# andreaskoepf/faster-rcnn.torch

Hardware: AMD Instinct MI355X
Metric: images/sec (vgg_small 800x450 fwd+bwd) (higher is better)
Workload: dtype f32 (conv / Linear(13824,1024) operands as 2 x fp16 split planes: 22 significand bits, 3 MFMA partial products; fp32 accumulate)

## Files before the change

faster-rcnn.torch_amd/_lib.py:

```python
import ctypes as C
import os

_HERE = os.path.dirname(os.path.abspath(__file__))
SO_PATH = os.environ.get("FRCNN_LIB_PATH") or os.path.join(_HERE, "libfrcnn_hip.so")

KC_NAMES = ["conv_igemm_k3", "conv_igemm_other", "conv_wgrad_k3", "conv_wgrad_other", "gemm", "elemwise",
            "roi", "rpn", "nms", "optim", "image", "conv_x3", "conv_wgradx", "topk"]


class FrcnnError(RuntimeError):
    pass


class ModelDesc(C.Structure):
    _fields_ = [
        ("nblocks", C.c_int),
        ("filters", C.c_int * 8), ("ksize", C.c_int * 8), ("pad", C.c_int * 8), ("conv_steps", C.c_int * 8),
        ("dropout", C.c_float * 8),
        ("nheads", C.c_int),
        ("head_k", C.c_int * 8), ("head_n", C.c_int * 8), ("head_input", C.c_int * 8),
        ("ncls", C.c_int),
        ("cls_n", C.c_int * 8), ("cls_bn", C.c_int * 8),
        ("cls_dropout", C.c_float * 8),
        ("class_count", C.c_int),
        ("kh", C.c_int), ("kw", C.c_int),
    ]


vp = C.c_void_p
_SIGS = {
    "frcnn_version": ([], C.c_int),
    "frcnn_set_option": ([C.c_char_p, C.c_int], C.c_int),
    "frcnn_get_option": ([C.c_char_p, C.POINTER(C.c_int)], C.c_int),
    "frcnn_last_error": ([], C.c_char_p),
    "frcnn_device_count": ([C.POINTER(C.c_int)], C.c_int),
    "frcnn_set_device": ([C.c_int], C.c_int),
    "frcnn_device_name": ([C.c_char_p, C.c_int], C.c_int),
    "frcnn_malloc": ([C.POINTER(vp), C.c_size_t], C.c_int),
    "frcnn_free": ([vp], C.c_int),
    "frcnn_host_alloc": ([C.POINTER(vp), C.c_size_t], C.c_int),
    "frcnn_host_free": ([vp], C.c_int),
    "frcnn_memcpy_h2d": ([vp, vp, C.c_size_t, vp], C.c_int),
    "frcnn_memcpy_d2h": ([vp, vp, C.c_size_t, vp], C.c_int),
    "frcnn_memcpy_d2d": ([vp, vp, C.c_size_t, vp], C.c_int),
    "frcnn_stream_sync": ([vp], C.c_int),
    "frcnn_zero": ([vp, C.c_size_t, vp], C.c_int),
    "frcnn_scale": ([vp, C.c_longlong, C.c_float, vp], C.c_int),
    "frcnn_add": ([vp, vp, C.c_longlong, vp], C.c_int),
    "frcnn_prof_enable": ([C.c_int], C.c_int),
    "frcnn_prof_collect": ([vp, vp, vp, vp], C.c_int),
    "frcnn_nms_workspace_bytes": ([C.c_int], C.c_size_t),
    "frcnn_nms_device": ([vp, C.c_int, C.c_int, C.c_float, C.c_int, C.c_int, vp, vp, vp, C.c_size_t, vp], C.c_int),
    "frcnn_nms_device_classes": ([vp, C.c_int, C.c_int, C.c_float, C.c_int, C.c_int, vp, vp, vp, vp, C.c_size_t, vp], C.c_int),
    "frcnn_nms_device_n": ([vp, C.c_int, vp, C.c_int, C.c_float, C.c_int, C.c_int, vp, vp, vp, vp, C.c_size_t, vp], C.c_int),
    "frcnn_nms_batch_workspace_bytes": ([C.c_int, C.c_int], C.c_size_t),
    "frcnn_nms_device_batch": ([vp, C.c_int, C.c_longlong, C.c_int, vp, C.c_int, C.c_float, C.c_int, C.c_int, vp, vp, vp, vp, C.c_size_t,
                               vp], C.c_int),
    "frcnn_topk_select_workspace_bytes": ([C.c_int, C.c_int], C.c_size_t),
    "frcnn_topk_select": ([vp, C.c_int, C.c_longlong, C.c_int, vp, C.c_int, vp, C.c_longlong, vp, vp, C.c_size_t, vp], C.c_int),
    "frcnn_rpn_gather_rows": ([vp, vp, vp, vp, C.c_int, C.c_longlong, C.c_int, vp, C.c_longlong, vp, C.c_int, vp, vp, vp, vp, vp, vp,
                              C.c_longlong, vp], C.c_int),
    "frcnn_detect_gather_batch": ([vp, vp, C.c_int, C.c_int, vp, vp, vp, vp, vp, C.c_longlong, vp, vp, vp, vp, vp], C.c_int),
    "frcnn_roi_windows": ([vp, vp, C.c_int, vp, C.c_int, C.c_int, C.c_int, vp, vp], C.c_int),
    "frcnn_detect_post": ([vp, vp, vp, vp, vp, C.c_int, C.c_int, C.c_double, vp, vp, vp, vp, vp, vp], C.c_int),
    "frcnn_detect_gather": ([vp, vp, C.c_int, vp, vp, vp, vp, vp, vp, vp, vp, vp, vp], C.c_int),
    "frcnn_nms_host": ([vp, C.c_int, C.c_int, C.c_float, C.c_int, C.c_int, vp, vp], C.c_int),
    "frcnn_conv2d_forward": ([vp, C.c_int, C.c_int, C.c_int, vp, vp, vp, vp, C.c_int, C.c_int, C.c_int, vp, vp], C.c_int),
    "frcnn_conv2d_backward_input": ([vp, C.c_int, C.c_int, C.c_int, vp, C.c_int, C.c_int, C.c_int, vp, C.c_int, vp], C.c_int),
    "frcnn_conv2d_backward_weight": ([vp, C.c_int, C.c_int, C.c_int, vp, vp, vp, C.c_int, C.c_int, C.c_int, vp, vp, vp], C.c_int),
    "frcnn_maxpool_act_forward": ([vp, C.c_int, C.c_int, C.c_int, vp, vp, vp, vp, vp], C.c_int),
    "frcnn_maxpool_act_backward": ([vp, vp, vp, C.c_int, C.c_int, C.c_int, vp, vp, vp, vp, vp, vp], C.c_int),
    "frcnn_act_forward": ([vp, C.c_int, C.c_longlong, vp, vp, vp, vp], C.c_int),
    "frcnn_act_backward": ([vp, vp, C.c_int, C.c_longlong, vp, vp, vp, vp, vp, vp], C.c_int),
    "frcnn_roi_pool_forward": ([vp, C.c_int, C.c_int, C.c_int, vp, C.c_int, C.c_int, C.c_int, vp, vp, vp], C.c_int),
    "frcnn_roi_pool_backward": ([vp, C.c_int, C.c_int, C.c_int, vp, vp, C.c_int, C.c_int, C.c_int, vp], C.c_int),
    "frcnn_roi_align_forward": ([vp, C.c_int, C.c_int, C.c_int, vp, vp, C.c_int, C.c_double, C.c_double, C.c_int, C.c_int, C.c_int, vp,
                                 vp], C.c_int),
    "frcnn_roi_align_backward": ([vp, C.c_int, C.c_int, C.c_int, vp, vp, vp, C.c_int, C.c_double, C.c_double, C.c_int, C.c_int, C.c_int,
                                  vp], C.c_int),
    "frcnn_rpn_scan_workspace_bytes": ([vp, vp], C.c_size_t),
    "frcnn_rpn_scan": ([vp, vp, vp, vp, vp, C.c_double, C.c_double, C.c_double, C.c_int, vp, vp, vp, vp, vp, vp, C.c_size_t, vp], C.c_int),
    "frcnn_rpn_scan_batch_workspace_bytes": ([vp, vp, C.c_int], C.c_size_t),
    "frcnn_rpn_scan_batch": ([vp, vp, vp, C.c_int, C.c_longlong, vp, vp, C.c_double, C.c_double, C.c_double, C.c_int, vp, vp, vp, vp, vp,
                             vp, C.c_size_t, vp], C.c_int),
    "frcnn_rpn_loss": ([vp, vp, vp, vp, vp, vp, vp, vp, C.c_int, C.c_int, C.c_int, vp, vp, vp, vp], C.c_int),
    "frcnn_loss_accumulate": ([vp, C.c_int, vp, vp], C.c_int),
    "frcnn_linear_forward": ([vp, C.c_int, C.c_int, vp, vp, C.c_int, vp, vp], C.c_int),
    "frcnn_linear_backward": ([vp, vp, C.c_int, C.c_int, vp, C.c_int, vp, vp, vp, vp], C.c_int),
    "frcnn_rmsprop": ([vp, vp, vp, C.c_longlong, C.c_float, C.c_float, C.c_float, vp], C.c_int),
    "frcnn_scale_rmsprop": ([vp, vp, C.c_float, vp, C.c_longlong, C.c_float, C.c_float, C.c_float, vp], C.c_int),
    "frcnn_scale_rmsprop_dev": ([vp, vp, vp, vp, C.c_longlong, C.c_float, C.c_float, C.c_float, vp], C.c_int),
    "frcnn_scale_rmsprop_slice": ([vp, vp, C.c_float, vp, C.c_longlong, C.c_longlong, C.c_float, C.c_float, C.c_float, vp], C.c_int),
    "frcnn_sgd": ([vp, vp, vp, C.c_longlong, C.c_float, vp, C.c_float, C.c_float, C.c_float, C.c_float, C.c_int, C.c_int, vp], C.c_int),
    "frcnn_sgd_slice": ([vp, vp, vp, C.c_longlong, C.c_longlong, C.c_float, C.c_float, C.c_float, C.c_float, C.c_float, C.c_int, C.c_int,
                         vp], C.c_int),
    "frcnn_nag": ([vp, vp, vp, C.c_longlong, C.c_float, vp, C.c_float, C.c_float, C.c_float, C.c_int, vp], C.c_int),
    "frcnn_nag_slice": ([vp, vp, vp, C.c_longlong, C.c_longlong, C.c_float, C.c_float, C.c_float, C.c_float, C.c_int, vp], C.c_int),
    "frcnn_scale_rmsprop_slice_dev": ([vp, vp, vp, vp, C.c_longlong, C.c_longlong, C.c_float, C.c_float, C.c_float, vp], C.c_int),
    "frcnn_sgd_slice_dev": ([vp, vp, vp, C.c_longlong, C.c_longlong, vp, C.c_float, C.c_float, C.c_float, C.c_float, C.c_int, C.c_int,
                            vp], C.c_int),
    "frcnn_nag_slice_dev": ([vp, vp, vp, C.c_longlong, C.c_longlong, vp, C.c_float, C.c_float, C.c_float, C.c_int, vp], C.c_int),
    "frcnn_grad_clip_workspace_bytes": ([C.c_longlong], C.c_size_t),
    "frcnn_grad_clip": ([vp, C.c_longlong, vp, C.c_int, C.c_double, vp, C.c_double, vp, vp, C.c_size_t, vp], C.c_int),
    "frcnn_nag_lookahead": ([vp, vp, C.c_longlong, C.c_float, vp], C.c_int),
    "frcnn_nag_lookahead_slice": ([vp, vp, C.c_longlong, C.c_longlong, C.c_float, vp], C.c_int),
    "frcnn_model_update_stream": ([vp, C.POINTER(vp)], C.c_int),
    "frcnn_model_update_fork": ([vp, vp], C.c_int),
    "frcnn_model_update_join": ([vp, vp], C.c_int),
    "frcnn_pnet_wait_backward_begun": ([vp, vp], C.c_int),
    "frcnn_pnet_wait_heads_done": ([vp, vp], C.c_int),
    "frcnn_pnet_wait_block_done": ([vp, C.c_int, vp], C.c_int),
    "frcnn_pnet_refresh_packs": ([vp, vp, C.c_int, vp], C.c_int),
    "frcnn_pnet_invalidate_packs": ([vp], C.c_int),
    "frcnn_model_create": ([C.POINTER(ModelDesc), C.POINTER(vp)], C.c_int),
    "frcnn_model_destroy": ([vp], C.c_int),
    "frcnn_model_param_count": ([vp, C.POINTER(C.c_longlong), C.POINTER(C.c_longlong)], C.c_int),
    "frcnn_model_param_table": ([vp, vp, C.c_int, C.POINTER(C.c_int)], C.c_int),
    "frcnn_model_localizer_layers": ([vp, C.c_int, vp, C.c_int, C.POINTER(C.c_int)], C.c_int),
    "frcnn_model_set_trainable": ([vp, C.c_int, C.c_int, C.c_int], C.c_int),
    "frcnn_model_get_trainable": ([vp, C.POINTER(C.c_int), C.POINTER(C.c_int), C.POINTER(C.c_int)], C.c_int),
    "frcnn_model_debug_buffer": ([vp, C.c_int, C.c_int, C.POINTER(vp), C.POINTER(C.c_longlong)], C.c_int),
    "frcnn_pnet_forward": ([vp, vp, vp, C.c_int, C.c_int, C.c_int, vp, C.c_ulonglong, vp], C.c_int),
    "frcnn_pnet_forward_async_heads": ([vp, vp, vp, C.c_int, C.c_int, vp, C.c_ulonglong, vp], C.c_int),
    "frcnn_pnet_output": ([vp, C.c_int, C.POINTER(vp), C.POINTER(C.c_int), C.POINTER(C.c_int), C.POINTER(C.c_int)], C.c_int),
    "frcnn_pnet_delta": ([vp, C.c_int, C.POINTER(vp)], C.c_int),
    "frcnn_pnet_set_sparse_deltas": ([vp, C.c_int, vp, C.c_int], C.c_int),
    "frcnn_pnet_zero_deltas": ([vp, vp], C.c_int),
    "frcnn_pnet_backward_heads_begin": ([vp, vp, vp, vp], C.c_int),
    "frcnn_pnet_anchor_loss_begin": ([vp, vp, vp, vp, vp, vp, vp, C.c_int, C.c_int, C.c_int, vp, vp, vp, vp, vp], C.c_int),
    "frcnn_pnet_anchor_loss_wait": ([vp, vp], C.c_int),
    "frcnn_pnet_backward_heads_join": ([vp, vp, C.POINTER(C.c_int)], C.c_int),
    "frcnn_pnet_backward": ([vp, vp, vp, vp], C.c_int),
    "frcnn_pnet_wait_block_gradients": ([vp, C.c_int, vp], C.c_int),
    "frcnn_cnet_forward": ([vp, vp, vp, C.c_int, C.c_int, vp, C.c_ulonglong, vp, vp, vp, vp], C.c_int),
    "frcnn_cnet_backward": ([vp, vp, vp, vp, vp, vp, vp], C.c_int),
    "frcnn_cnet_backward_join": ([vp, vp], C.c_int),
    "frcnn_cnet_losses": ([vp, vp, vp, vp, C.c_int, C.c_int, C.c_int, vp, vp, vp, vp], C.c_int),
    "frcnn_cnet_decode": ([vp, C.c_int, C.c_int, vp, vp, vp], C.c_int),
    "frcnn_anchors_create": ([vp, vp, vp, vp, C.c_int, C.c_int, C.POINTER(vp)], C.c_int),
    "frcnn_anchors_destroy": ([vp], C.c_int),
    "frcnn_anchors_assemble": ([vp, vp, C.c_int, C.c_double, C.c_double, C.c_double, C.c_double, C.c_int, C.c_int, C.c_int, vp,
                               C.POINTER(C.c_int), vp, vp, C.c_int, C.POINTER(C.c_int), C.POINTER(C.c_int)], C.c_int),
    "frcnn_comm_get_unique_id": ([vp], C.c_int),
    "frcnn_comm_exchange_id_file": ([C.c_char_p, C.c_int, vp, C.c_int], C.c_int),
    "frcnn_comm_init_rank": ([C.POINTER(vp), C.c_int, C.c_int, vp], C.c_int),
    "frcnn_comm_init_rank_timeout": ([C.POINTER(vp), C.c_int, C.c_int, vp, C.c_int], C.c_int),
    "frcnn_comm_init_rank_file": ([C.POINTER(vp), C.c_int, C.c_int, C.c_char_p, C.c_int], C.c_int),
    "frcnn_comm_destroy": ([vp], C.c_int),
    "frcnn_comm_info": ([vp, C.POINTER(C.c_int), C.POINTER(C.c_int)], C.c_int),
    "frcnn_comm_query": ([vp, C.POINTER(C.c_int), C.POINTER(C.c_int), C.POINTER(C.c_int)], C.c_int),
    "frcnn_allreduce_f32": ([vp, vp, C.c_longlong, vp], C.c_int),
    "frcnn_allreduce_f64": ([vp, vp, C.c_longlong, vp], C.c_int),
    "frcnn_broadcast_f32": ([vp, vp, C.c_longlong, C.c_int, vp], C.c_int),
    "frcnn_image_rgb2yuv": ([vp, vp, C.c_int, C.c_int, vp], C.c_int),
    "frcnn_image_rgb2hsv": ([vp, vp, C.c_int, C.c_int, vp], C.c_int),
    "frcnn_image_rgb2lab": ([vp, vp, C.c_int, C.c_int, vp], C.c_int),
    "frcnn_image_scale": ([vp, C.c_int, C.c_int, C.c_int, vp, C.c_int, C.c_int, vp, C.c_int, vp], C.c_int),
    "frcnn_image_scale_u8": ([vp, C.c_int, C.c_int, vp, C.c_int, C.c_int, vp, C.c_int, vp], C.c_int),
    "frcnn_image_crop_flip": ([vp, C.c_int, C.c_int, C.c_int, C.c_int, C.c_int, C.c_int, C.c_int, C.c_int, C.c_int, vp, vp], C.c_int),
    "frcnn_image_normalize_workspace_bytes": ([C.c_int], C.c_size_t),
    "frcnn_image_normalize": ([vp, C.c_int, C.c_int, C.c_int, C.c_int, C.c_int, vp, C.c_size_t, vp], C.c_int),
    "frcnn_image_contrastive_norm": ([vp, C.c_int, C.c_int, vp, C.c_int, C.c_float, vp, vp, vp], C.c_int),
}

_lib = None


def exported_symbols():
    return sorted(_SIGS.keys())


def load():
    global _lib
    if _lib is not None:
        return _lib
    if not os.path.exists(SO_PATH):
        raise FrcnnError(
            "libfrcnn_hip.so not found at %s -- build it with `python -c 'import __graft_entry__ as g; g.build()'` "
            "(there is no CPU fallback for the product path)" % SO_PATH)
    try:
        import torch
    except ImportError:
        pass
    L = C.CDLL(SO_PATH)
    for name, (args, res) in _SIGS.items():
        fn = getattr(L, name)
        fn.argtypes = args
        fn.restype = res
    _lib = L
    return L


def check(rc):
    if rc != 0:
        raise FrcnnError("libfrcnn_hip: %s (code %d)" % (load().frcnn_last_error().decode("utf-8", "replace"), rc))


def call(name, *args):
    check(getattr(load(), name)(*args))
```

faster-rcnn.torch_amd/csrc/amax.h:

```cpp
#pragma once
#include <hip/hip_runtime.h>

#include "kernels.h"

namespace frcnn {

__device__ __forceinline__ void amax_store_block(float m, float* rec) {
  __shared__ float amax_part[16];
#pragma unroll
  for (int o = 32; o > 0; o >>= 1) m = fmaxf(m, __shfl_xor(m, o));
  if ((threadIdx.x & 63) == 0) amax_part[threadIdx.x >> 6] = m;
  __syncthreads();
  if (threadIdx.x == 0) {
    const int nw = (blockDim.x + 63) >> 6;
    for (int i = 1; i < nw; ++i) m = fmaxf(m, amax_part[i]);
    rec[1 + blockIdx.x] = m;
    if (blockIdx.x == 0) rec[0] = __builtin_bit_cast(float, (int)gridDim.x);
  }
}

__device__ __forceinline__ float amax_load_block(const float* __restrict__ rec) {
  __shared__ float amax_all[16];
  const int n = __builtin_bit_cast(int, rec[0]);
  float m = 0.f;
  for (int i = threadIdx.x; i < n; i += blockDim.x) m = fmaxf(m, rec[1 + i]);
#pragma unroll
  for (int o = 32; o > 0; o >>= 1) m = fmaxf(m, __shfl_xor(m, o));
  if ((threadIdx.x & 63) == 0) amax_all[threadIdx.x >> 6] = m;
  __syncthreads();
  const int nw = (blockDim.x + 63) >> 6;
  m = amax_all[0];
  for (int i = 1; i < nw; ++i) m = fmaxf(m, amax_all[i]);
  __syncthreads();
  return m;
}

}
```

faster-rcnn.torch_amd/csrc/cnet.hip:

```cpp
#include "kernels.h"

namespace frcnn {

#define BN_EPS 1e-5
#define BN_MOM 0.1

#define BN_CB 16
#define BN_RG 64
template <int CB = BN_CB, int RG = BN_RG>
__device__ __forceinline__ double bn_reduce(double v, double* sh, int tx, int ty) {
  sh[ty * CB + tx] = v;
  __syncthreads();
  for (int stride = RG / 2; stride > 0; stride >>= 1) {
    if (ty < stride) sh[ty * CB + tx] += sh[(ty + stride) * CB + tx];
    __syncthreads();
  }
  const double s = sh[tx];
  __syncthreads();
  return s;
}
template <int NV>
__device__ __forceinline__ void fb_reduce(double (&v)[NV], double* sh, int tx, int ty) {
  const int tid = ty * 4 + tx, lane = tid & 63, wave = tid >> 6;
#pragma unroll
  for (int k = 0; k < NV; ++k) {
#pragma unroll
    for (int o = 4; o < 64; o <<= 1) v[k] += __shfl_xor(v[k], o, 64);
    if (lane < 4) sh[(k * 16 + wave) * 4 + lane] = v[k];
  }
  __syncthreads();
#pragma unroll
  for (int k = 0; k < NV; ++k) {
    double t = 0.0;
#pragma unroll
    for (int w = 0; w < 16; ++w) t += sh[(k * 16 + w) * 4 + tx];
    v[k] = t;
  }
  __syncthreads();
}
#define FB_CB 4
#define FB_RG 256
#define FB_KEEP 4

__global__ __launch_bounds__(1024) void bn_forward_kernel(const float* __restrict__ x, int R, int n,
                                                          const float* __restrict__ gamma, const float* __restrict__ beta,
                                                          float* running, int training, float* __restrict__ xhat,
                                                          float* __restrict__ invstd, float* __restrict__ y) {
  __shared__ double sh[BN_RG * BN_CB];
  const int tx = threadIdx.x, ty = threadIdx.y;
  const int j = blockIdx.x * BN_CB + tx;
  const bool ok = j < n;
  double mean, var;
  if (training) {
    double s = 0.0;
    if (ok) for (int r = ty; r < R; r += BN_RG) s += x[(size_t)r * n + j];
    mean = bn_reduce(s, sh, tx, ty) / R;
    double q = 0.0;
    if (ok) for (int r = ty; r < R; r += BN_RG) { double d = x[(size_t)r * n + j] - mean; q += d * d; }
    var = bn_reduce(q, sh, tx, ty);
    const double unb = R > 1 ? var / (R - 1) : var / R;
    var /= R;
    if (running && ok && ty == 0) {
      running[j] = (float)((1.0 - BN_MOM) * running[j] + BN_MOM * mean);
      running[n + j] = (float)((1.0 - BN_MOM) * running[n + j] + BN_MOM * unb);
    }
  } else {
    mean = ok ? running[j] : 0.0;
    var = ok ? running[n + j] : 1.0;
  }
  if (!ok) return;
  const double is = 1.0 / sqrt(var + BN_EPS);
  if (ty == 0) invstd[j] = (float)is;
  const double g = gamma[j], b = beta[j];
  for (int r = ty; r < R; r += BN_RG) {
    const double xh = (x[(size_t)r * n + j] - mean) * is;
    xhat[(size_t)r * n + j] = (float)xh;
    y[(size_t)r * n + j] = (float)(xh * g + b);
  }
}
int bn_forward(const float* x, int R, int n, const float* gamma, const float* beta, float* running,
               int training, float* xhat, float* invstd, float* y, hipStream_t s) {
  FR_CHECK(training || running, "bn_forward: evaluate mode needs running statistics");
  FR_LAUNCH(KC_ELEMWISE, 0, (double)R * n * 16.0, s, bn_forward_kernel, dim3(cdiv(n, BN_CB)), dim3(BN_CB, BN_RG), 0, x, R, n,
            gamma, beta, running, training, xhat, invstd, y);
  FR_LAUNCH_CHECK();
  return FRCNN_OK;
}

__global__ __launch_bounds__(1024) void bn_backward_kernel(const float* __restrict__ gy, const float* __restrict__ xhat,
                                                           const float* __restrict__ invstd, const float* __restrict__ gamma,
                                                           int R, int n, int training, float* __restrict__ gx, float* ggamma,
                                                           float* gbeta) {
  __shared__ double sh[BN_RG * BN_CB];
  const int tx = threadIdx.x, ty = threadIdx.y;
  const int j = blockIdx.x * BN_CB + tx;
  const bool ok = j < n;
  double sg = 0.0, sgx = 0.0;
  if (ok)
    for (int r = ty; r < R; r += BN_RG) {
      const double g = gy[(size_t)r * n + j];
      sg += g;
      sgx += g * xhat[(size_t)r * n + j];
    }
  sg = bn_reduce(sg, sh, tx, ty);
  sgx = bn_reduce(sgx, sh, tx, ty);
  if (!ok) return;
  if (ty == 0) {
    ggamma[j] = (float)((double)ggamma[j] + sgx);
    gbeta[j] = (float)((double)gbeta[j] + sg);
  }
  const double is = invstd[j], gm = gamma[j];
  for (int r = ty; r < R; r += BN_RG) {
    const double g = gy[(size_t)r * n + j];
    const double xh = xhat[(size_t)r * n + j];
    const double v = training ? (g - sg / R - xh * sgx / R) * gm * is : g * gm * is;
    gx[(size_t)r * n + j] = (float)v;
  }
}
int bn_backward(const float* gy, const float* xhat, const float* invstd, const float* gamma, int R,
                int n, int training, float* gx, float* ggamma, float* gbeta, hipStream_t s) {
  FR_LAUNCH(KC_ELEMWISE, 0, (double)R * n * 16.0, s, bn_backward_kernel, dim3(cdiv(n, BN_CB)), dim3(BN_CB, BN_RG), 0, gy,
            xhat, invstd, gamma, R, n, training, gx, ggamma, gbeta);
  FR_LAUNCH_CHECK();
  return FRCNN_OK;
}

__device__ __forceinline__ float fold_value(const float* __restrict__ x, const GemmFold& src, size_t total, size_t idx, int j) {
  if (src.nSplit == 0) return x[idx];
  float v = src.bias ? src.bias[j] : 0.f;
  for (int sI = 0; sI < src.nSplit; ++sI) v += src.slab[(size_t)sI * total + idx];
  return v;
}

template <bool GEN>
__global__ __launch_bounds__(1024) void cnet_act_forward_kernel(const float* __restrict__ x, GemmFold src, int R, int n,
                                                                const float* __restrict__ gamma, const float* __restrict__ beta,
                                                                float* running, int training, float* __restrict__ lin,
                                                                float* __restrict__ xhat, float* __restrict__ invstd,
                                                                float* __restrict__ pre, const float* slope, float* __restrict__ mask,
                                                                float inv_keep, float p, unsigned long long seed,
                                                                float* __restrict__ post) {
  __shared__ double sh[FB_RG * FB_CB];
  const int tx = threadIdx.x, ty = threadIdx.y;
  const int j = blockIdx.x * FB_CB + tx;
  const bool ok = j < n;
  const size_t total = (size_t)R * n;
  const bool bn = gamma != nullptr;
  const float* v = src.nSplit ? lin : x;
  const bool keep = R <= FB_RG * FB_KEEP;
  float xv[FB_KEEP];
  double s0 = 0.0;
  if (ok) {
#pragma unroll
    for (int i = 0; i < FB_KEEP; ++i) {
      const int r = ty + i * FB_RG;
      xv[i] = 0.f;
      if (keep && r < R) {
        const size_t idx = (size_t)r * n + j;
        xv[i] = fold_value(x, src, total, idx, j);
        if (src.nSplit) lin[idx] = xv[i];
        s0 += xv[i];
      }
    }
    if (!keep && (src.nSplit || (bn && training)))
      for (int r = ty; r < R; r += FB_RG) {
        const size_t idx = (size_t)r * n + j;
        const float t = fold_value(x, src, total, idx, j);
        if (src.nSplit) lin[idx] = t;
        s0 += t;
      }
  }
  double mean = 0.0, is = 1.0, g = 1.0, b = 0.0;
  if (bn) {
    double var;
    if (training) {
      { double t[1] = {s0}; fb_reduce(t, sh, tx, ty); mean = t[0] / R; }
      double q = 0.0;
      if (ok && keep) {
#pragma unroll
        for (int i = 0; i < FB_KEEP; ++i)
          if (ty + i * FB_RG < R) { double d = xv[i] - mean; q += d * d; }
      } else if (ok) {
        for (int r = ty; r < R; r += FB_RG) { double d = v[(size_t)r * n + j] - mean; q += d * d; }
      }
      { double t[1] = {q}; fb_reduce(t, sh, tx, ty); var = t[0]; }
      const double unb = R > 1 ? var / (R - 1) : var / R;
      var /= R;
      if (running && ok && ty == 0) {
        running[j] = (float)((1.0 - BN_MOM) * running[j] + BN_MOM * mean);
        running[n + j] = (float)((1.0 - BN_MOM) * running[n + j] + BN_MOM * unb);
      }
    } else {
      mean = ok ? running[j] : 0.0;
      var = ok ? running[n + j] : 1.0;
    }
    if (!ok) return;
    is = 1.0 / sqrt(var + BN_EPS);
    if (ty == 0) invstd[j] = (float)is;
    g = gamma[j]; b = beta[j];
  }
  if (!ok) return;
  const float a = *slope;
  auto emit = [&](size_t idx, float y) {
    if (bn) {
      const double xh = ((double)y - mean) * is;
      xhat[idx] = (float)xh;
      y = (float)(xh * g + b);
      pre[idx] = y;
    }
    y = y > 0.f ? y : a * y;
    if (GEN) {
      const float mk = frcnn_keep_mask(seed, (unsigned long long)idx, p);
      mask[idx] = mk;
      y = y * (mk * inv_keep);
    } else if (mask) {
      y = y * (mask[idx] * inv_keep);
    }
    post[idx] = y;
  };
  if (keep) {
#pragma unroll
    for (int i = 0; i < FB_KEEP; ++i)
      if (ty + i * FB_RG < R) emit((size_t)(ty + i * FB_RG) * n + j, xv[i]);
  } else {
    for (int r = ty; r < R; r += FB_RG) emit((size_t)r * n + j, v[(size_t)r * n + j]);
  }
}
template <bool GEN>
__global__ void cnet_act_forward_flat_kernel(const float* __restrict__ x, GemmFold src, long total, int n, float* __restrict__ lin,
                                             const float* slope, float* __restrict__ mask, float inv_keep, float p,
                                             unsigned long long seed, float* __restrict__ post) {
  const float a = *slope;
  for (long i = (long)blockIdx.x * blockDim.x + threadIdx.x; i < total; i += (long)gridDim.x * blockDim.x) {
    float y = fold_value(x, src, (size_t)total, (size_t)i, (int)(i % n));
    if (src.nSplit) lin[i] = y;
    y = y > 0.f ? y : a * y;
    if (GEN) {
      const float mk = frcnn_keep_mask(seed, (unsigned long long)i, p);
      mask[i] = mk;
      y = y * (mk * inv_keep);
    } else if (mask) {
      y = y * (mask[i] * inv_keep);
    }
    post[i] = y;
  }
}
int cnet_act_forward(const float* x, GemmFold src, int R, int n, const float* gamma, const float* beta, float* running,
                     int training, float* lin, float* xhat, float* invstd, float* pre, const float* slope, float* mask, bool gen,
                     float inv_keep, float p, unsigned long long seed, float* post, hipStream_t s) {
  FR_CHECK(!gamma || training || running, "cnet_act_forward: evaluate mode needs running statistics");
  if (!gamma) {
    const long total = (long)R * n;
    const int grid = (int)std::min<long>(std::max<long>(1, cdivl(total, 256)), 2048);
    if (gen)
      FR_LAUNCH(KC_ELEMWISE, 0, total * 16.0, s, cnet_act_forward_flat_kernel<true>, dim3(grid), dim3(256), 0, x, src, total, n, lin, slope,
                mask, inv_keep, p, seed, post);
    else
      FR_LAUNCH(KC_ELEMWISE, 0, total * 16.0, s, cnet_act_forward_flat_kernel<false>, dim3(grid), dim3(256), 0, x, src, total, n, lin, slope,
                mask, inv_keep, p, seed, post);
    FR_LAUNCH_CHECK();
    return FRCNN_OK;
  }
  if (gen)
    FR_LAUNCH(KC_ELEMWISE, 0, (double)R * n * 20.0, s, cnet_act_forward_kernel<true>, dim3(cdiv(n, FB_CB)), dim3(FB_CB, FB_RG), 0, x,
              src, R, n, gamma, beta, running, training, lin, xhat, invstd, pre, slope, mask, inv_keep, p, seed, post);
  else
    FR_LAUNCH(KC_ELEMWISE, 0, (double)R * n * 20.0, s, cnet_act_forward_kernel<false>, dim3(cdiv(n, FB_CB)), dim3(FB_CB, FB_RG), 0, x,
              src, R, n, gamma, beta, running, training, lin, xhat, invstd, pre, slope, mask, inv_keep, p, seed, post);
  FR_LAUNCH_CHECK();
  return FRCNN_OK;
}

__global__ __launch_bounds__(1024) void cnet_act_bn_backward_kernel(const float* __restrict__ gy, GemmFold src,
                                                                    const float* __restrict__ pre, const float* __restrict__ xhat,
                                                                    const float* __restrict__ invstd, const float* __restrict__ gamma,
                                                                    const float* slope, const float* __restrict__ mask, float inv_keep,
                                                                    int R, int n, int training, float* __restrict__ gx, float* ggamma,
                                                                    float* gbeta, float* gslope, float* part) {
  __shared__ double sh[FB_RG * FB_CB];
  __shared__ float shs[16];
  const int tx = threadIdx.x, ty = threadIdx.y;
  const int j = blockIdx.x * FB_CB + tx;
  const bool ok = j < n;
  const size_t total = (size_t)R * n;
  const float a = *slope;
  double sg = 0.0, sgx = 0.0;
  float sa = 0.f;
  const bool keep = R <= FB_RG * FB_KEEP;
  float tv[FB_KEEP], xh[FB_KEEP];
  auto first = [&](size_t idx, float& t, float& xhv) {
    float g = fold_value(gy, src, total, idx, j);
    if (mask) g = g * (mask[idx] * inv_keep);
    const float xv = pre[idx];
    t = g;
    if (!(xv > 0.f)) { t = a * g; sa += xv * g; }
    xhv = xhat[idx];
    sg += t;
    sgx += (double)t * xhv;
  };
  if (ok && keep) {
#pragma unroll
    for (int i = 0; i < FB_KEEP; ++i) {
      tv[i] = 0.f; xh[i] = 0.f;
      if (ty + i * FB_RG < R) first((size_t)(ty + i * FB_RG) * n + j, tv[i], xh[i]);
    }
  } else if (ok) {
    for (int r = ty; r < R; r += FB_RG) {
      const size_t idx = (size_t)r * n + j;
      float t, xhv;
      first(idx, t, xhv);
      gx[idx] = t;
    }
  }
  { double t[2] = {sg, sgx}; fb_reduce(t, sh, tx, ty); sg = t[0]; sgx = t[1]; }
  {
    const int tid = ty * FB_CB + tx;
#pragma unroll
    for (int o = 32; o > 0; o >>= 1) sa += __shfl_down(sa, o, 64);
    if ((tid & 63) == 0) shs[tid >> 6] = sa;
    __syncthreads();
    if (tid == 0) {
      float t = 0.f;
      for (int i = 0; i < 16; ++i) t += shs[i];
      if (part) part[blockIdx.x] = t; else unsafeAtomicAdd(gslope, t);
    }
  }
  if (!ok) return;
  if (ty == 0) {
    ggamma[j] = (float)((double)ggamma[j] + sgx);
    gbeta[j] = (float)((double)gbeta[j] + sg);
  }
  const double is = invstd[j], gm = gamma[j];
  auto second = [&](size_t idx, double g, double xhv) {
    const double v = training ? (g - sg / R - xhv * sgx / R) * gm * is : g * gm * is;
    gx[idx] = (float)v;
  };
  if (keep) {
#pragma unroll
    for (int i = 0; i < FB_KEEP; ++i)
      if (ty + i * FB_RG < R) second((size_t)(ty + i * FB_RG) * n + j, tv[i], xh[i]);
  } else {
    for (int r = ty; r < R; r += FB_RG) {
      const size_t idx = (size_t)r * n + j;
      second(idx, gx[idx], xhat[idx]);
    }
  }
}
__global__ void slope_fold_kernel(const float* __restrict__ part, int n, float* gslope);
int cnet_act_bn_backward(const float* gy, GemmFold src, const float* pre, const float* xhat, const float* invstd,
                         const float* gamma, const float* slope, const float* mask, float inv_keep, int R, int n, int training,
                         float* gx, float* ggamma, float* gbeta, float* gslope, hipStream_t s) {
  const int grid = cdiv(n, FB_CB);
  float* part = nullptr;
  if (deterministic()) FR_TRY(det_workspace(s, (size_t)grid, &part));
  FR_LAUNCH(KC_ELEMWISE, 0, (double)R * n * 28.0, s, cnet_act_bn_backward_kernel, dim3(grid), dim3(FB_CB, FB_RG), 0, gy, src, pre, xhat,
            invstd, gamma, slope, mask, inv_keep, R, n, training, gx, ggamma, gbeta, gslope, part);
  if (part) FR_LAUNCH(KC_ELEMWISE, 0, grid * 4.0, s, slope_fold_kernel, dim3(1), dim3(1), 0, (const float*)part, grid, gslope);
  FR_LAUNCH_CHECK();
  return FRCNN_OK;
}

template <bool GEN>
__global__ void prelu_dropout_forward_kernel(const float* __restrict__ x, long n, const float* slope,
                                             float* __restrict__ mask, float inv_keep, float p,
                                             unsigned long long seed, float* __restrict__ y) {
  const float a = *slope;
  for (long i = (long)blockIdx.x * blockDim.x + threadIdx.x; i < n; i += (long)gridDim.x * blockDim.x) {
    float v = x[i];
    v = v > 0.f ? v : a * v;
    if (GEN) {
      const float mk = frcnn_keep_mask(seed, (unsigned long long)i, p);
      mask[i] = mk;
      v = v * (mk * inv_keep);
    } else if (mask) {
      v = v * (mask[i] * inv_keep);
    }
    y[i] = v;
  }
}
int prelu_dropout_forward(const float* x, long n, const float* slope, const float* mask, float inv_keep,
                          float* y, hipStream_t s) {
  int grid = (int)std::min<long>(std::max<long>(1, cdivl(n, 256)), 1024);
  FR_LAUNCH(KC_ELEMWISE, 0, n * 12.0, s, prelu_dropout_forward_kernel<false>, dim3(grid), dim3(256), 0, x, n, slope,
            const_cast<float*>(mask), inv_keep, 0.f, 0ull, y);
  FR_LAUNCH_CHECK();
  return FRCNN_OK;
}
int prelu_dropout_forward_gen(const float* x, long n, const float* slope, float* mask_out, float p,
                              unsigned long long seed, float* y, hipStream_t s) {
  int grid = (int)std::min<long>(std::max<long>(1, cdivl(n, 256)), 1024);
  FR_LAUNCH(KC_ELEMWISE, 0, n * 12.0, s, prelu_dropout_forward_kernel<true>, dim3(grid), dim3(256), 0, x, n, slope,
            mask_out, 1.0f / (1.0f - p), p, seed, y);
  FR_LAUNCH_CHECK();
  return FRCNN_OK;
}

__global__ void prelu_dropout_backward_kernel(const float* __restrict__ gy, const float* __restrict__ x, long n,
                                              const float* slope, const float* __restrict__ mask,
                                              float inv_keep, float* __restrict__ gx, float* gslope, float* part) {
  __shared__ float sh[4];
  const float a = *slope;
  float sa = 0.f;
  for (long i = (long)blockIdx.x * blockDim.x + threadIdx.x; i < n; i += (long)gridDim.x * blockDim.x) {
    float g = gy[i];
    if (mask) g = g * (mask[i] * inv_keep);
    const float xv = x[i];
    float r = g;
    if (!(xv > 0.f)) { r = a * g; sa += xv * g; }
    gx[i] = r;
  }
#pragma unroll
  for (int o = 32; o > 0; o >>= 1) sa += __shfl_down(sa, o, 64);
  if ((threadIdx.x & 63) == 0) sh[threadIdx.x >> 6] = sa;
  __syncthreads();
  if (threadIdx.x == 0) {
    const float t = sh[0] + sh[1] + sh[2] + sh[3];
    if (part) part[blockIdx.x] = t;
    else unsafeAtomicAdd(gslope, t);
  }
}
__global__ void slope_fold_kernel(const float* __restrict__ part, int n, float* gslope) {
  float v = 0.f;
  for (int i = 0; i < n; ++i) v += part[i];
  *gslope += v;
}
int prelu_dropout_backward(const float* gy, const float* x, long n, const float* slope,
                           const float* mask, float inv_keep, float* gx, float* gslope, hipStream_t s) {
  int grid = (int)std::min<long>(std::max<long>(1, cdivl(n, 256)), 256);
  float* part = nullptr;
  if (deterministic()) FR_TRY(det_workspace(s, (size_t)grid, &part));
  FR_LAUNCH(KC_ELEMWISE, 0, n * 16.0, s, prelu_dropout_backward_kernel, dim3(grid), dim3(256), 0, gy, x, n,
            slope, mask, inv_keep, gx, gslope, part);
  if (part) FR_LAUNCH(KC_ELEMWISE, 0, grid * 4.0, s, slope_fold_kernel, dim3(1), dim3(1), 0, (const float*)part, grid, gslope);
  FR_LAUNCH_CHECK();
  return FRCNN_OK;
}

__device__ __forceinline__ double wave_sum_f64(double v) {
#pragma unroll
  for (int o = 32; o > 0; o >>= 1) v += __shfl_xor(v, o, 64);
  return v;
}
__device__ __forceinline__ double wave_max_f64(double v) {
#pragma unroll
  for (int o = 32; o > 0; o >>= 1) { const double w = __shfl_xor(v, o, 64); v = w > v ? w : v; }
  return v;
}
__global__ void log_softmax_rows_fold_kernel(float* __restrict__ x, GemmFold src, int R, int n, float* __restrict__ y,
                                             float* __restrict__ y2) {
  const int r = blockIdx.x * (blockDim.x >> 6) + (threadIdx.x >> 6), lane = threadIdx.x & 63;
  if (r >= R) return;
  float* xr = x + (size_t)r * n;
  const size_t total = (size_t)R * n;
  if (src.nSplit)
    for (int i = lane; i < n; i += 64) xr[i] = fold_value(x, src, total, (size_t)r * n + i, i);
  double m = -1.0e300;
  for (int i = lane; i < n; i += 64) m = xr[i] > m ? (double)xr[i] : m;
  m = wave_max_f64(m);
  double s = 0.0;
  for (int i = lane; i < n; i += 64) s += exp((double)xr[i] - m);
  s = wave_sum_f64(s);
  const double lse = m + log(s);
  for (int i = lane; i < n; i += 64) {
    const float v = (float)((double)xr[i] - lse);
    y[(size_t)r * n + i] = v;
    if (y2) y2[(size_t)r * n + i] = v;
  }
}
int log_softmax_rows_fold(const float* x, GemmFold src, int R, int n, float* y, float* y2, hipStream_t s) {
  if (R <= 0) return FRCNN_OK;
  FR_LAUNCH(KC_ELEMWISE, 0, (double)R * n * 8.0, s, log_softmax_rows_fold_kernel, dim3(cdiv(R, 4)), dim3(256), 0, const_cast<float*>(x),
            src, R, n, y, y2);
  FR_LAUNCH_CHECK();
  return FRCNN_OK;
}

__global__ void log_softmax_rows_kernel(const float* __restrict__ x, int R, int n, float* __restrict__ y) {
  const int r = blockIdx.x * (blockDim.x >> 6) + (threadIdx.x >> 6), lane = threadIdx.x & 63;
  if (r >= R) return;
  const float* xr = x + (size_t)r * n;
  double m = -1.0e300;
  for (int i = lane; i < n; i += 64) m = xr[i] > m ? (double)xr[i] : m;
  m = wave_max_f64(m);
  double s = 0.0;
  for (int i = lane; i < n; i += 64) s += exp((double)xr[i] - m);
  s = wave_sum_f64(s);
  const double lse = m + log(s);
  for (int i = lane; i < n; i += 64) y[(size_t)r * n + i] = (float)((double)xr[i] - lse);
}
int log_softmax_rows(const float* x, int R, int n, float* y, hipStream_t s) {
  if (R <= 0) return FRCNN_OK;
  FR_LAUNCH(KC_ELEMWISE, 0, (double)R * n * 8.0, s, log_softmax_rows_kernel, dim3(cdiv(R, 4)), dim3(256), 0, x, R,
            n, y);
  FR_LAUNCH_CHECK();
  return FRCNN_OK;
}

#define HEADS_PITCH 33
__global__ __launch_bounds__(256) void cnet_heads_forward_kernel(const float* __restrict__ x, int R, int nf, const float* __restrict__ Wb,
                                                                 const float* __restrict__ bb, const float* __restrict__ Wc,
                                                                 const float* __restrict__ bc, int nc, float* __restrict__ bbox_out,
                                                                 float* __restrict__ logits, float* __restrict__ lsm,
                                                                 float* __restrict__ cls_out) {
  extern __shared__ float wt[];
  float* xs = wt + (size_t)nf * HEADS_PITCH + (threadIdx.x >> 6) * nf;
  const int no = 4 + nc;
  for (int k = threadIdx.x; k < nf; k += 256) {
    float* d = wt + k * HEADS_PITCH;
#pragma unroll
    for (int n = 0; n < 4; ++n) d[n] = Wb[(size_t)n * nf + k];
#pragma unroll 8
// ... 208 lines not shown
```

faster-rcnn.torch_amd/csrc/kernels.h:

```cpp
#pragma once
#include <algorithm>

#include "common.h"

namespace frcnn {

int conv_cc(int k);
int conv_mpad(int M);
size_t conv_pack_floats(int Kchan, int M, int k);
int conv_pack_weights(const float* w, int O, int C, int k, float* wf, float* wd, hipStream_t s);
struct PackJob { long w_off; long total; float* dst; int O, C, k, mode, Mpad, blk_begin, nblk; };
PackJob conv_pack_job(long w_off, int O, int C, int k, int mode, float* dst);
int conv_pack_assign_blocks(PackJob* jobs, int njobs, int total_blocks);
int conv_pack_weights_multi(const float* weights, const PackJob* jobs_dev, int njobs, int grid, hipStream_t s);

enum { OUT_STORE = 0, OUT_ADD = 1 };
struct IgemmPool { float* out; unsigned char* idx; const float* slope; const float* scale; float* amax = nullptr; };
int conv_igemm(const float* in, int Cin, int H, int W, const float* in_slope, const float* in_scale,
               const float* wp, const float* bias, int M, int k, int pad, float* out, int out_mode,
               double algo_flops, hipStream_t s, int ws_slot = 0,
               const IgemmPool* pool = nullptr, bool* pool_fused = nullptr);

void set_split_bf16(int on);
int get_split_bf16();
bool conv_x3_eligible(int Cin, int M, int k);
size_t conv_x3_pack_bytes(int Kchan, int M, int k);
struct PackXJob {
  long w_off; long total; void* dst; const float* amax; float* amax_w; int O, C, k, mode, bm, blk_begin, nblk;
  const int* oidx = nullptr; const int* cidx = nullptr; int Cs = 0; long bias_off = 0; float* bias_dst = nullptr;
};
PackXJob conv_x3_pack_job(long w_off, int O, int C, int k, int mode, void* dst, int Ho, int Wo);
int conv_x3_pack_assign_blocks(PackXJob* jobs, int njobs);
int conv_x3_pack_multi(const float* weights, const PackXJob* jobs_dev, int njobs, int grid, hipStream_t s);
int conv_x3_pack(const float* w, int O, int C, int k, int mode, void* dst, hipStream_t s, int Ho, int Wo,
                 const float* amax_rec_w = nullptr, float* amax_w = nullptr);
#define AMAX_REC 16400
#define AMAX_MAX_BLOCKS 16384
int tensor_absmax(const float* x, long n, float* rec, hipStream_t s);
struct AmaxJob { long off; long n; float* out; int blk_begin; };
int tensor_absmax_assign_blocks(AmaxJob* jobs, int njobs);
long tensor_absmax_record_floats(long n);
int tensor_absmax_multi(const float* w, const AmaxJob* jobs_dev, int njobs, int grid, hipStream_t s);
void set_x3_f16(int on);
int get_x3_f16();
int conv_x3(const float* in, int Cin, int H, int W, const float* in_slope, const float* in_scale, const void* wp,
            const float* bias, int M, int k, int pad, float* out, int out_mode, double algo_flops, hipStream_t s, int ws_slot = 0,
            const struct X3PostAct* post = nullptr, const float* amax_in = nullptr, const float* amax_w = nullptr,
            float* amax_out = nullptr);
struct X3PostAct {
  const float* x;
  const float* slope;
  const float* scale;
  float* gslope;
};

bool conv_wgradx_eligible(int Cin, int O, int k);
size_t conv_wgradx_workspace_bytes(int Cin, int H, int W, int O, int pad);
struct WgradMap { const int* omap = nullptr; const int* cmap = nullptr; int Cfull = 0; };
int conv_wgradx(const float* in, int Cin, int H, int W, const float* in_slope, const float* in_scale, const float* g, int O,
                int pad, float* gw, void* ws, size_t ws_bytes, hipStream_t s, float* gbias = nullptr,
                const float* amax_in = nullptr, const float* amax_g = nullptr,
                const WgradMap* map = nullptr);
int wgrad_reduce(const float* slab, int nSplit, int taps, int OC, float* gw, hipStream_t s);
int wgrad_reduce_map(const float* slab, int nSplit, int taps, int O, int C, float* gw, const WgradMap& map, hipStream_t s);
bool conv_wgrad_first_pooled_eligible(int Cin, int O, int k, int Wo);
int conv_wgrad_first_pooled(const float* in, int Cin, int H, int W, const float* gpool, const unsigned char* pidx, const float* x,
                            const float* slope, int O, int pad, float* gw, float* gbias, float* gslope, void* ws, size_t ws_bytes,
                            hipStream_t s);

size_t conv_wgrad_workspace_bytes(int Cin, int H, int W, int O, int k, int pad);
int conv_wgrad(const float* in, int Cin, int H, int W, const float* in_slope, const float* in_scale,
               const float* g, int O, int k, int pad, float* gw, void* ws, size_t ws_bytes, hipStream_t s,
               float* gbias = nullptr,
               const float* amax_in = nullptr, const float* amax_g = nullptr,
               const WgradMap* map = nullptr);

bool deterministic();
void set_deterministic(bool on);
int det_workspace(hipStream_t s, size_t floats, float** out);

int fill_zero(void* p, size_t bytes, hipStream_t s);
int scale_inplace(float* x, long n, float sc, hipStream_t s);
int add_inplace(float* y, const float* x, long n, hipStream_t s);
int act_forward(const float* x, int C, long hw, const float* slope, const float* scale, float* y,
                hipStream_t s);
int maxpool_act_forward(const float* x, int C, int H, int W, const float* slope, const float* scale,
                        float* out, unsigned char* idx, hipStream_t s, float* amax = nullptr);
int maxpool_act_backward(const float* gpool, const unsigned char* idx, const float* x, int C, int H,
                         int W, const float* slope, const float* scale, float* gx, float* gbias,
                         float* gslope, hipStream_t s, float* amax = nullptr);
int act_backward(const float* gy, const float* x, int C, long hw, const float* slope,
                 const float* scale, float* gx, float* gbias, float* gslope, hipStream_t s, float* amax = nullptr);
int channel_sum(const float* g, int C, long hw, float* gbias, hipStream_t s);
int channel_sum_cols(const float* g, int R, int O, float* gb, hipStream_t s);
int gather_positions(const float* src, int C, long hw, const int* pos, int P, float* dst, const float* slope,
                     float* dst_act, hipStream_t s);
int im2col_positions(const float* X, int C, int H, int W, int k, int Wo, const int* pos, int P, float* col, hipStream_t s);
int col2im_positions_add(const float* col, int C, int H, int W, int k, int Wo, const int* pos, int P, float* gX,
                         hipStream_t s);
int dropout_channel_mask(float* scale, int C, float p, unsigned long long seed, hipStream_t s);
int fill_value(float* x, long n, float v, hipStream_t s);
int rmsprop_step(float* x, float* g, float* m, long n, float lr, float alpha, float eps, float gscale,
                 bool scale_first, hipStream_t s, const double* gcount_dev = nullptr);
int rmsprop_slice(float* x, float* g, float* m, long lo, long hi, float lr, float alpha, float eps, float gscale, bool scale_first,
                  hipStream_t s, const double* gcount_dev = nullptr);
int sgd_update(float* x, float* g, float* v, long lo, long hi, bool slice, float gscale, const double* gcount_dev, float clr,
               float wd, float mom, float one_minus_damp, bool nesterov, bool first, hipStream_t s);
int nag_update(float* x, float* g, float* v, long lo, long hi, bool slice, float gscale, const double* gcount_dev, float clr,
               float wd, float mom, bool first, hipStream_t s);
int nag_lookahead(float* x, const float* v, long n, float mom, hipStream_t s);
constexpr int GRAD_CLIP_MAX_RANGES = 16;
size_t grad_clip_workspace_bytes(long n);
int grad_clip(float* g, long n, const long long* ranges_host, int nranges, double divisor, const double* divisor_dev, double clip_norm,
              double* record, void* workspace, size_t workspace_bytes, hipStream_t s);
int nag_lookahead_slice(float* x, const float* v, long lo, long hi, float mom, hipStream_t s);

#define FRCNN_HEAD_OUT 18
struct HeadJob {
  int Cin, H, W, k, Ho, Wo, n;
  int P; const int* pos;
  const float* in; float* gin;
  const float *bias3, *slope, *bias1;
  float *gbias3, *gslope, *gbias1;
  float* out; const float* delta;
  float *COL, *HX, *HY, *OUT, *D, *GH, *DX;
  const float* hx_slab; int hx_splits;
};
struct HeadJobs { HeadJob j[4]; int n; };
int heads_im2col(const HeadJobs& g, hipStream_t s);
int heads_bias_act(const HeadJobs& g, hipStream_t s);
int heads_scatter(const HeadJobs& g, hipStream_t s);
int heads_gather_delta(const HeadJobs& g, hipStream_t s);
int heads_act_backward(const HeadJobs& g, hipStream_t s);
int heads_col2im(const HeadJobs& g, hipStream_t s);

struct GemmFold;
#define GEMM_GROUP_MAX 4
struct GemmJob {
  const float* A; long sAm, sAk; const float* B; long sBk, sBn; float* C; long ldc;
  int M, N, K, out_mode;
  int splits = 1;
  int kPerSplit = 0;
};
int gemm_f32_group(GemmJob* jobs, int n, hipStream_t s);
int gemm_f32(const float* A, long sAm, long sAk, const float* B, long sBk, long sBn, float* C,
             long ldc, int M, int N, int K, int out_mode, const float* bias_n, hipStream_t s, int ws_slot = 0,
             GemmFold* defer = nullptr);
int gemm_workspace_get(size_t need, float** out, int slot);
struct GemmFold {
  const float* slab = nullptr;
  int nSplit = 0;
  const float* bias = nullptr;
};
int gemm_reduce_slabs(const float* slab, int nSplit, int M, int N, const float* bias, float* C, long ldc, bool accumulate,
                      hipStream_t s);
void set_gemm_x_roles(int mask);
int get_gemm_x_roles();
bool linear_x_eligible(int role, int R, int I, int O);
int linear_x_rows_padded(int R);
int split_planes(const float* src, int R, int C, void* P , void* PT ,
                 hipStream_t s, const float* amax = nullptr);
int linear_x_forward(const void* Xp, int R, int I, const float* W, const float* bias, int O, float* y, hipStream_t s, int ws_slot = 0,
                     GemmFold* defer = nullptr, const float* amax_x = nullptr, const float* amax_w = nullptr);
int linear_x_dgrad(const void* Gp, int R, int O, const float* W, int I, float* gx, int out_mode, hipStream_t s, int ws_slot = 0,
                   GemmFold* defer = nullptr, const float* amax_g = nullptr, const float* amax_w = nullptr);
int linear_x_wgrad(const void* GpT, const void* XpT, int R, int O, int I, float* gw, hipStream_t s, int ws_slot = 0,
                   const float* amax_g = nullptr, const float* amax_x = nullptr);


int roi_pool_forward(const float* fmap, int C, int H, int W, const int* wins, int R, int kh, int kw,
                     float* out, int* idx, hipStream_t s);
int roi_pool_backward(float* gmap, int C, int H, int W, const float* gout, const int* idx, int R,
                      int kh, int kw, hipStream_t s);

int roi_align_forward(const float* fmap, int C, int H, int W, const double* rect, const long long* pick, int R, double inv_sx,
                      double inv_sy, int kh, int kw, int g, float* out, hipStream_t s);
int roi_align_backward(float* gmap, int C, int H, int W, const float* gout, const double* rect, const long long* pick, int R,
                       double inv_sx, double inv_sy, int kh, int kw, int g, hipStream_t s);

struct RpnLayers {
  const float* map[4];
  int H[4], W[4];
};
int rpn_scan(const RpnLayers& L, const float* anchor_w, const float* anchor_h, double img_w,
             double img_h, double p_threshold, int cap, float* match_p, int* match_idx,
             double* match_rect, float* match_box, int* count, void* ws, size_t ws_bytes,
             hipStream_t s);
size_t rpn_scan_workspace_bytes(const RpnLayers& L);
int rpn_scan_batch(const RpnLayers& L, int B, long slot_stride, const float* anchor_w, const float* anchor_h, double img_w,
                   double img_h, double p_threshold, int cap, float* match_p, int* match_idx, double* match_rect,
                   float* match_box, int* count, void* ws, size_t ws_bytes, hipStream_t s);
size_t rpn_scan_batch_workspace_bytes(const RpnLayers& L, int B);
int rpn_loss(const RpnLayers& L, float* const* delta, const int* ex_idx, const double* ex_anchor,
             const double* ex_roi, const int* ex_class, int npos, int nneg, int bgclass,
             double* ex_loss, float* crtarget, float* cctarget, hipStream_t s);

int loss_accumulate(const double* ex_loss, int E, double* acc, hipStream_t s);

size_t nms_workspace_bytes(int n);
int nms_device(const float* boxes, int n, int ncols, float overlap, int key_mode, int key_col,
               long long* pick, int* count, void* ws, size_t ws_bytes, hipStream_t s, const int* cls = nullptr,
               const int* n_dev = nullptr);
size_t nms_batch_workspace_bytes(int B, int n);
int nms_device_batch(const float* boxes, int B, long row_stride, int n, const int* n_dev, int ncols, float overlap, int key_mode,
                     int key_col, const int* cls, long long* pick, int* count, void* ws, size_t ws_bytes, hipStream_t s);
size_t topk_select_workspace_bytes(int B, int n_cap);
int topk_select(const float* score, int B, long stride, int n_cap, const int* n_dev, int K, int* sel_row, long sel_stride,
                int* k_dev, void* ws, size_t ws_bytes, hipStream_t s);
int rpn_gather_rows(const float* p, const int* idx, const double* rect, const float* box, int B, long src_stride, int src_rows,
                    const int* sel_row, long sel_stride, const int* k_dev, int k_cap, float* dst_p, int* dst_idx,
                    double* dst_rect, float* dst_box, float* box5, int* row, long dst_stride, hipStream_t s);
int roi_windows(const double* rect, const long long* pick, int k, const int* layers, int nlayers, int fmH, int fmW, int* wins,
                hipStream_t s);
int detect_post(const int* cls, const float* conf, const float* bbox, const double* rect, const long long* pick, int R,
                int bgclass, double min_conf, float* bb, int* kc, int* keep_row, double* r2, int* K_dev, hipStream_t s);
int detect_gather(const long long* wpick, const int* nwin_dev, int cap, const int* keep_row, const int* kc, const float* bb,
                  const double* r2, const long long* pick, const float* mp, const double* rect, const int* midx, double* rec,
                  hipStream_t s);
int detect_gather_batch(const long long* wpick, const int* counts, int B, int row_stride, const int* keep_row, const int* kc,
                        const float* bb, const double* r2, const long long* pick, long match_stride, const float* mp,
                        const double* rect, const int* midx, double* rec, hipStream_t s);

int bn_forward(const float* x, int R, int n, const float* gamma, const float* beta, float* running,
               int training, float* xhat, float* invstd, float* y, hipStream_t s);
int bn_backward(const float* gy, const float* xhat, const float* invstd, const float* gamma, int R,
                int n, int training, float* gx, float* ggamma, float* gbeta, hipStream_t s);
int prelu_dropout_forward(const float* x, long n, const float* slope, const float* mask, float inv_keep,
                          float* y, hipStream_t s);
int prelu_dropout_forward_gen(const float* x, long n, const float* slope, float* mask_out, float p,
                              unsigned long long seed, float* y, hipStream_t s);
int prelu_dropout_backward(const float* gy, const float* x, long n, const float* slope,
                           const float* mask, float inv_keep, float* gx, float* gslope, hipStream_t s);
int cnet_act_forward(const float* x, GemmFold src, int R, int n, const float* gamma, const float* beta, float* running,
                     int training, float* lin, float* xhat, float* invstd, float* pre, const float* slope, float* mask, bool gen,
                     float inv_keep, float p, unsigned long long seed, float* post, hipStream_t s);
int cnet_act_bn_backward(const float* gy, GemmFold src, const float* pre, const float* xhat, const float* invstd,
                         const float* gamma, const float* slope, const float* mask, float inv_keep, int R, int n, int training,
                         float* gx, float* ggamma, float* gbeta, float* gslope, hipStream_t s);
bool cnet_heads_fused_eligible(int nf, int nc);
int cnet_heads_forward(const float* x, int R, int nf, const float* Wb, const float* bb, const float* Wc, const float* bc, int nc,
                       float* bbox_out, float* logits, float* lsm, float* cls_out, hipStream_t s);
struct HeadsPostAct {
  const float* pre = nullptr;
  const float* mask = nullptr;
  float inv_keep = 1.f;
  const float* slope = nullptr;
  float* gslope = nullptr;
};
int cnet_heads_backward(const float* g_bbox, const float* g_cls, const float* lsm, int R, int nf, const float* Wb, const float* Wc,
                        int nc, float* glog, float* gfeat, hipStream_t s, const HeadsPostAct* post = nullptr);
int log_softmax_rows_fold(const float* x, GemmFold src, int R, int n, float* y, float* y2, hipStream_t s);
int dropout_mask(float* mask, long n, float p, unsigned long long seed, hipStream_t s);
struct DropoutJobs { float* ptr[8]; int C[8]; float p[8]; unsigned long long seed[8]; int n; };
int dropout_channel_masks(const DropoutJobs& j, hipStream_t s);
int log_softmax_rows(const float* x, int R, int n, float* y, hipStream_t s);
int cnet_losses(float* crout, const float* crtarget, const float* ccout, const float* cctarget, int R,
                int npos, int ncls, float* crdelta, float* ccdelta, double* loss2, hipStream_t s);
int log_softmax_backward(const float* gy, const float* lsm, int R, int n, float* gx, hipStream_t s);
int cnet_decode(const float* cls_lsm, int R, int ncls, int* cls_out, float* conf_out, hipStream_t s);

int image_rgb2yuv(const float* rgb, float* yuv, int H, int W, hipStream_t s);
int image_rgb2hsv(const float* rgb, float* hsv, int H, int W, hipStream_t s);
int image_rgb2lab(const float* rgb, float* lab, int H, int W, hipStream_t s);
int image_scale(const float* src, int C, int H, int W, float* dst, int dH, int dW, float* tmp, int rgb2yuv,
                hipStream_t s);
int image_scale_u8(const unsigned char* src_hwc, int H, int W, float* dst, int dH, int dW, float* tmp, int rgb2yuv,
                   hipStream_t s);
int image_crop_flip(const float* src, int C, int H, int W, int x0, int y0, int w, int h, int hflip, int vflip,
                    float* dst, hipStream_t s);
size_t image_normalize_workspace_bytes(int C);
int image_normalize(float* img, int C, int H, int W, int centering, int scaling, void* ws, size_t ws_bytes,
                    hipStream_t s);
int image_contrastive_norm(const float* in, int H, int W, const float* kernel_host, int K, float threshold, float* out,
                           float* tmp, hipStream_t s);

}
```

faster-rcnn.torch_amd/csrc/net.cpp:

```cpp
#include <array>
#include <vector>
#include <cmath>
#include <cstring>

#include "kernels.h"

namespace frcnn {

static const int HEAD_OUT = 18;
static const int SPARSE_MAX_POS = 512;

struct DevBuf {
  void* p = nullptr;
  size_t bytes = 0;
  bool owned = true;
  void view(void* ptr, size_t n) { p = ptr; bytes = n; owned = false; }
  int ensure(size_t need) {
    if (need <= bytes) return FRCNN_OK;
    if (p && owned) (void)hipFree(p);
    owned = true;
    p = nullptr; bytes = 0;
    FR_HIP(hipMalloc(&p, need + 64));
    bytes = need;
    return FRCNN_OK;
  }
  void release() { if (p && owned) (void)hipFree(p); p = nullptr; bytes = 0; owned = true; }
  float* f() const { return (float*)p; }
};

struct Conv {
  int Cin, Cout, k, pad;
  int H, W, Ho, Wo;
  long w_off, b_off, a_off;
  int block, step;
  DevBuf wf, wd;
  DevBuf wx, wxd;
  bool x_f = false, x_d = false;
  DevBuf x, gx;
  int am = -1;
};

struct Block {
  int first_conv, nconv;
  bool has_drop;
  float p_drop;
  DevBuf scale;
  DevBuf pooled, gpooled;
  DevBuf pidx;
  int Hp, Wp;
  int am = -1;
  bool dc_on = false;
  int nk = 0, nkM = 0, nkK = 0;
  const int* dc_idx = nullptr;
  DevBuf dc_bias;
};

struct Head {
  Conv c3;
  Conv c1;
  int input;
  DevBuf delta;
  const int* sp_pos = nullptr;
  int sp_count = -1;
  DevBuf spD, spHX, spHY, spGH, spCol, spDX;
  DevBuf spOut, spSlab;
  hipStream_t stream = nullptr;
  hipEvent_t done = nullptr;
  hipEvent_t gin_done = nullptr;
  bool gin_recorded = false;
};

struct ClsLayer {
  int in, n;
  bool bn;
  float p_drop;
  long w_off, b_off, bnw_off, bnb_off, a_off;
  DevBuf lin, pre, post, xhat, invstd, mask, g;
  DevBuf gin;
  DevBuf xp, xpT, gp, gpT;
  int x_form = 0;
  DevBuf am;
  const float* am_w_of = nullptr;
  long am_w_gen = -1;
};

}

using namespace frcnn;

static int g_drop_compact = -1;
static int drop_compact_on() {
  if (g_drop_compact < 0) g_drop_compact = getenv("FRCNN_DROP_COMPACT") ? (atoi(getenv("FRCNN_DROP_COMPACT")) != 0) : 1;
  return g_drop_compact;
}
static int pool_stream(int slot, hipStream_t* out) {
  static hipStream_t pool[8] = {};
  if (!pool[slot]) FR_HIP(hipStreamCreateWithFlags(&pool[slot], hipStreamNonBlocking));
  *out = pool[slot];
  return FRCNN_OK;
}

static int g_sparse_heads = -1;
static int sparse_heads_on() {
  if (g_sparse_heads < 0) g_sparse_heads = getenv("FRCNN_SPARSE_HEADS") ? (atoi(getenv("FRCNN_SPARSE_HEADS")) != 0) : 1;
  return g_sparse_heads;
}
static int g_static_weights = 0;
static long g_static_gen = 0;

struct frcnn_model {
  frcnn_model_desc d;
  std::vector<Conv> convs;
  std::vector<Block> blocks;
  std::vector<Head> heads;
  std::vector<ClsLayer> cls;
  long pnet_params = 0, total_params = 0;
  long bbox_w_off = 0, bbox_b_off = 0, clsw_off = 0, clsb_off = 0;
  int H = 0, W = 0;
  int training = 0;
  DevBuf delta_last;
  DevBuf zero_arena;
  size_t delta_bytes = 0, gpool_bytes = 0;
  DevBuf pack_jobs;
  DevBuf x3_jobs;
  DevBuf amax, amax_ws, amax_jobs;
  int n_amax = 0, n_amax_jobs = 0, amax_grid = 0;
  float* rec(int id) const { return (float*)amax.p + (size_t)id * AMAX_REC; }
  bool f16_packed = false;
  long eval_packs_gen = -1;
  const float* eval_packs_w = nullptr;
  int n_x3_all = 0, n_x3_fwd = 0, x3_grid_all = 0, x3_grid_fwd = 0;
  int n_pack_fwd = 0, n_pack_all = 0, n_pack_heads = 0, pack_grid_fwd = 0, pack_grid_all = 0, pack_grid_heads = 0;
  bool head_packs_fresh = false;
  struct PackGroup { int pk_off = 0, pk_n = 0, pk_grid = 0, am_off = 0, am_n = 0, am_grid = 0, x3_off = 0, x3_off16 = 0, x3_n = 0, x3_grid = 0; };
  std::vector<PackGroup> groups;
  unsigned fresh_mask = 0;
  const float* fresh_w = nullptr;
  bool fresh_f16 = false;
  static const int DC_RING = 4;
  char* dc_pin = nullptr; DevBuf dc_dev; size_t dc_slot_bytes = 0, dc_idx_off = 0; unsigned dc_step = 0;
  hipEvent_t dc_ev[DC_RING] = {};
  std::vector<PackXJob> x3_host, x3_host16;
  std::vector<int> x3_conv;
  DevBuf dbg_expand;
  std::vector<hipEvent_t> block_rd_ev;
  hipStream_t side = nullptr;
  hipStream_t cw = nullptr;
  hipEvent_t cw_fork = nullptr, cw_done = nullptr;
  bool cw_pending = false;
  std::vector<hipEvent_t> cw_ev;
  std::vector<hipEvent_t> fork_ev;
  hipEvent_t join_ev = nullptr;
  bool update_armed = false;
  hipEvent_t bwd_ev = nullptr;
  hipEvent_t upd_ev = nullptr, upd_join_ev = nullptr;
  bool head_x3_fresh = true;
  int am_bb_off = 0, am_bb_n = 0, am_bb_grid = 0;
  int pk_bb_off = 0, pk_bb_n = 0, pk_bb_grid = 0;
  bool heads_deferred = false;
  bool heads_sparse_fwd = false;
  const float* last_w = nullptr;
  hipEvent_t heads_gin_ev = nullptr;
  bool heads_gin = false;
  bool heads_begun = false;
  bool heads_joined = false;
  bool side_busy = false;
  hipEvent_t loss_ev = nullptr;
  hipEvent_t chain_ev = nullptr;
  std::vector<hipEvent_t> block_ev;
  bool block_ev_valid = false;
  bool loss_pending = false;
  DevBuf wg_ws;
  DevBuf wg_ws_first;
  DevBuf img;
  int frozen_blocks = 0;
  int train_heads = 1, train_cnet = 1;
  int R = 0, D = 0;
  const float* cnet_x = nullptr;
  DevBuf feat_g, logits, lsm, glog, gtmp;
  std::vector<std::array<long long, 4>> table;
};

static int pool_out(int n) { return (n - 2 + 1) / 2 + 1; }
static int refresh_group(frcnn_model* m, const float* w, int group, hipStream_t s);

static void build_layout(frcnn_model* m) {
  const frcnn_model_desc& d = m->d;
  long off = 0;
  int cin = 3;
  for (int b = 0; b < d.nblocks; ++b) {
    Block blk;
    blk.first_conv = (int)m->convs.size();
    blk.nconv = d.conv_steps[b];
    blk.has_drop = d.dropout[b] > 0.f;
    blk.p_drop = d.dropout[b];
    for (int s = 0; s < d.conv_steps[b]; ++s) {
      Conv c;
      c.Cin = cin; c.Cout = d.filters[b]; c.k = d.ksize[b]; c.pad = d.pad[b];
      c.block = b; c.step = s;
      long wsz = (long)c.Cout * c.Cin * c.k * c.k;
      c.w_off = off; c.b_off = off + wsz; c.a_off = off + wsz + c.Cout;
      m->table.push_back({c.w_off, wsz, 0, (long long)c.k * c.k * c.Cout});
      m->table.push_back({c.b_off, c.Cout, 1, 0});
      m->table.push_back({c.a_off, 1, 2, 0});
      off += wsz + c.Cout + 1;
      cin = c.Cout;
      m->convs.push_back(std::move(c));
    }
    m->blocks.push_back(std::move(blk));
  }
  for (int h = 0; h < d.nheads; ++h) {
    Head hd;
    hd.input = d.head_input[h] - 1;
    Conv& a = hd.c3;
    a.Cin = d.filters[hd.input]; a.Cout = d.head_n[h]; a.k = d.head_k[h]; a.pad = 0;
    a.block = -1; a.step = 0;
    long wsz = (long)a.Cout * a.Cin * a.k * a.k;
    a.w_off = off; a.b_off = off + wsz; a.a_off = off + wsz + a.Cout;
    m->table.push_back({a.w_off, wsz, 0, (long long)a.k * a.k * a.Cout});
    m->table.push_back({a.b_off, a.Cout, 1, 0});
    m->table.push_back({a.a_off, 1, 2, 0});
    off += wsz + a.Cout + 1;
    Conv& c = hd.c1;
    c.Cin = a.Cout; c.Cout = HEAD_OUT; c.k = 1; c.pad = 0; c.block = -1; c.step = 1;
    long w1 = (long)HEAD_OUT * c.Cin;
    c.w_off = off; c.b_off = off + w1; c.a_off = -1;
    m->table.push_back({c.w_off, w1, 0, (long long)HEAD_OUT});
    m->table.push_back({c.b_off, HEAD_OUT, 1, 0});
    off += w1 + HEAD_OUT;
    m->heads.push_back(std::move(hd));
  }
  m->pnet_params = off;
  int in = d.kh * d.kw * d.filters[d.nblocks - 1];
  m->D = in;
  for (int l = 0; l < d.ncls; ++l) {
    ClsLayer L;
    L.in = in; L.n = d.cls_n[l]; L.bn = d.cls_bn[l] != 0; L.p_drop = d.cls_dropout[l];
    L.w_off = off; L.b_off = off + (long)in * L.n;
    m->table.push_back({L.w_off, (long long)in * L.n, 3, in});
    m->table.push_back({L.b_off, L.n, 4, in});
    off += (long)in * L.n + L.n;
    L.bnw_off = L.bnb_off = -1;
    if (L.bn) {
      L.bnw_off = off; L.bnb_off = off + L.n;
      m->table.push_back({L.bnw_off, L.n, 5, 0});
      m->table.push_back({L.bnb_off, L.n, 6, 0});
      off += 2L * L.n;
    }
    L.a_off = off;
    m->table.push_back({L.a_off, 1, 2, 0});
    off += 1;
    in = L.n;
    m->cls.push_back(std::move(L));
  }
  m->bbox_w_off = off; m->bbox_b_off = off + (long)in * 4;
  m->table.push_back({m->bbox_w_off, (long long)in * 4, 3, in});
  m->table.push_back({m->bbox_b_off, 4, 4, in});
  off += (long)in * 4 + 4;
  int nc = d.class_count + 1;
  m->clsw_off = off; m->clsb_off = off + (long)in * nc;
  m->table.push_back({m->clsw_off, (long long)in * nc, 3, in});
  m->table.push_back({m->clsb_off, nc, 4, in});
  off += (long)in * nc + nc;
  m->total_params = off;
}

static int ensure_conv(Conv& c, int H, int W, bool need_dgrad) {
  c.H = H; c.W = W;
  c.Ho = H + 2 * c.pad - c.k + 1; c.Wo = W + 2 * c.pad - c.k + 1;
  FR_CHECK(c.Ho > 0 && c.Wo > 0, "image too small: a %dx%d map reaches a %dx%d convolution", H, W, c.k, c.k);
  size_t n = (size_t)c.Cout * c.Ho * c.Wo * 4;
  FR_TRY(c.x.ensure(n));
  FR_TRY(c.gx.ensure(n));
  if (c.wf.bytes < conv_pack_floats(c.Cin, c.Cout, c.k) * 4) {
    FR_TRY(c.wf.ensure(conv_pack_floats(c.Cin, c.Cout, c.k) * 4));
    FR_HIP(hipMemset(c.wf.p, 0, c.wf.bytes));
  }
  if (need_dgrad && c.wd.bytes < conv_pack_floats(c.Cout, c.Cin, c.k) * 4) {
    FR_TRY(c.wd.ensure(conv_pack_floats(c.Cout, c.Cin, c.k) * 4));
    FR_HIP(hipMemset(c.wd.p, 0, c.wd.bytes));
  }
  c.x_f = (c.k == 3 || c.block < 0) && conv_x3_eligible(c.Cin, c.Cout, c.k);
  c.x_d = c.block >= 0 && need_dgrad && conv_x3_eligible(c.Cout, c.Cin, c.k);
  if (c.x_f) FR_TRY(c.wx.ensure(conv_x3_pack_bytes(c.Cin, c.Cout, c.k)));
  if (c.x_d) FR_TRY(c.wxd.ensure(conv_x3_pack_bytes(c.Cout, c.Cin, c.k)));
  return FRCNN_OK;
}

static int ensure_shapes(frcnn_model* m, int H, int W) {
  int h = H, w = W;
  for (size_t b = 0; b < m->blocks.size(); ++b) {
    Block& blk = m->blocks[b];
    for (int s = 0; s < blk.nconv; ++s) {
      Conv& c = m->convs[blk.first_conv + s];
      FR_TRY(ensure_conv(c, h, w, !(b == 0 && s == 0)));
      h = c.Ho; w = c.Wo;
    }
    FR_CHECK(h >= 2 && w >= 2, "image too small for block %zu pooling", b + 1);
    blk.Hp = pool_out(h); blk.Wp = pool_out(w);
    int C = m->d.filters[b];
    FR_TRY(blk.pooled.ensure((size_t)C * blk.Hp * blk.Wp * 4));
    FR_TRY(blk.pidx.ensure((size_t)C * blk.Hp * blk.Wp));
    if (blk.has_drop) FR_TRY(blk.scale.ensure((size_t)C * 4));
    h = blk.Hp; w = blk.Wp;
  }
  for (auto& hd : m->heads) {
    const Block& in = m->blocks[hd.input];
    FR_TRY(ensure_conv(hd.c3, in.Hp, in.Wp, true));
    FR_TRY(ensure_conv(hd.c1, hd.c3.Ho, hd.c3.Wo, true));
  }
  const Block& last = m->blocks.back();
  {
    auto al = [](size_t b) { return (b + 255) / 256 * 256; };
    size_t db = 0, gb = 0;
    for (auto& hd : m->heads) db += al((size_t)HEAD_OUT * hd.c1.Ho * hd.c1.Wo * 4);
    db += al((size_t)m->d.filters[m->d.nblocks - 1] * last.Hp * last.Wp * 4);
    for (size_t b = 0; b < m->blocks.size(); ++b) gb += al((size_t)m->d.filters[b] * m->blocks[b].Hp * m->blocks[b].Wp * 4);
    m->zero_arena.release();
    FR_TRY(m->zero_arena.ensure(db + gb));
    char* q = (char*)m->zero_arena.p;
    for (auto& hd : m->heads) { size_t n = (size_t)HEAD_OUT * hd.c1.Ho * hd.c1.Wo * 4; hd.delta.view(q, n); q += al(n); }
    { size_t n = (size_t)m->d.filters[m->d.nblocks - 1] * last.Hp * last.Wp * 4; m->delta_last.view(q, n); q += al(n); }
    for (size_t b = 0; b < m->blocks.size(); ++b) {
      size_t n = (size_t)m->d.filters[b] * m->blocks[b].Hp * m->blocks[b].Wp * 4;
      m->blocks[b].gpooled.view(q, n); q += al(n);
    }
    m->delta_bytes = db; m->gpool_bytes = gb;
  }
  size_t wsb = 0;
  for (auto& c : m->convs) wsb = std::max(wsb, conv_wgrad_workspace_bytes(c.Cin, c.H, c.W, c.Cout, c.k, c.pad));
  for (auto& hd : m->heads) {
// ... 606 lines not shown
    else
      FR_TRY(conv_pack_weights_multi(w, (const PackJob*)m->pack_jobs.p + m->n_pack_all, m->n_pack_fwd, m->pack_grid_fwd, s));
    const PackXJob* xjobs = (const PackXJob*)m->x3_jobs.p + (f16 ? m->n_x3_all + m->n_x3_fwd : 0);
    if (f16 && skip_heads)
      FR_TRY(tensor_absmax_multi(w, (const AmaxJob*)m->amax_jobs.p + m->am_bb_off, m->am_bb_n, m->am_bb_grid, s));
    else if (f16)
      FR_TRY(tensor_absmax_multi(w, (const AmaxJob*)m->amax_jobs.p, m->n_amax_jobs, m->amax_grid, s));
    if (training && any_compact(m))
      FR_TRY(pack_compact(m, w, f16, s));
    else if (training)
      FR_TRY(conv_x3_pack_multi(w, xjobs, m->n_x3_all, m->x3_grid_all, s));
    else
      FR_TRY(conv_x3_pack_multi(w, xjobs + m->n_x3_all, m->n_x3_fwd, m->x3_grid_fwd, s));
  }
  m->eval_packs_gen = training ? -1 : g_static_gen;
  m->eval_packs_w = w;
  FR_TRY(m->img.ensure((size_t)3 * H * W * 4));
  FR_HIP(hipMemcpyAsync(m->img.p, img, (size_t)3 * H * W * 4, hipMemcpyDeviceToDevice, s));
  const float* cur = m->img.f();
  const float* cur_slope = nullptr;
  const float* cur_scale = nullptr;
  const float* cur_am = nullptr;
  for (size_t b = 0; b < m->blocks.size(); ++b) {
    Block& blk = m->blocks[b];
    bool pooled_in_conv = false;
    for (int st = 0; st < blk.nconv; ++st) {
      Conv& c = m->convs[blk.first_conv + st];
      const bool last = st == blk.nconv - 1;
      IgemmPool pl = {blk.pooled.f(), (unsigned char*)blk.pidx.p, w + c.a_off,
                      (st == 0 && blk.has_drop) ? blk.scale.f() : nullptr, f16 ? m->rec(blk.am) : nullptr};
      const bool want_am = f16 && !last && m->convs[blk.first_conv + st + 1].x_f;
      if (c.x_f && blk.dc_on && st <= 1) {
        const int cin = st == 0 ? c.Cin : blk.nkK, mo = st == 0 ? blk.nkM : c.Cout;
        FR_TRY(conv_x3(cur, cin, c.H, c.W, cur_slope, nullptr, c.wx.p, st == 0 ? blk.dc_bias.f() : w + c.b_off, mo, c.k, c.pad, c.x.f(),
                       OUT_STORE, 0, s, 0, nullptr, f16 ? cur_am : nullptr, f16 ? m->amax_ws.f() + c.am : nullptr,
                       want_am ? m->rec(c.am) : nullptr));
      } else if (c.x_f)
        FR_TRY(conv_x3(cur, c.Cin, c.H, c.W, cur_slope, cur_scale, c.wx.p, w + c.b_off, c.Cout, c.k, c.pad, c.x.f(), OUT_STORE, 0, s, 0,
                       nullptr, f16 ? cur_am : nullptr, f16 ? m->amax_ws.f() + c.am : nullptr, want_am ? m->rec(c.am) : nullptr));
      else
        FR_TRY(conv_igemm(cur, c.Cin, c.H, c.W, cur_slope, cur_scale, c.wf.f(), w + c.b_off, c.Cout, c.k, c.pad,
                          c.x.f(), OUT_STORE, 0, s, 0, last ? &pl : nullptr, last ? &pooled_in_conv : nullptr));
      if (want_am) {
        if (!c.x_f) FR_TRY(tensor_absmax(c.x.f(), (long)c.Cout * c.Ho * c.Wo, m->rec(c.am), s));
        cur_am = m->rec(c.am);
      }
      cur = c.x.f();
      cur_slope = w + c.a_off;
      cur_scale = (st == 0 && blk.has_drop) ? blk.scale.f() : nullptr;
    }
    const Conv& lc = m->convs[blk.first_conv + blk.nconv - 1];
    if (!pooled_in_conv)
      FR_TRY(maxpool_act_forward(cur, lc.Cout, lc.Ho, lc.Wo, cur_slope, cur_scale, blk.pooled.f(),
                                 (unsigned char*)blk.pidx.p, s, f16 ? m->rec(blk.am) : nullptr));
    cur = blk.pooled.f();
    cur_slope = nullptr;
    cur_scale = nullptr;
    cur_am = f16 ? m->rec(blk.am) : nullptr;
    if (use_side && b + 1 < m->blocks.size() && !m->heads_deferred) {
      FR_TRY(ensure_side(m));
      for (size_t i = 0; i < m->heads.size(); ++i) {
        Head& h = m->heads[i];
        if (h.input != (int)b) continue;
        FR_TRY(fork_to(m, s, head_stream(m, i), 16 + i));
        FR_TRY(head_forward(m, h, w, head_stream(m, i), head_slot(m, i)));
      }
    }
  }
  if (!m->heads_deferred) {
    const int last = (int)m->blocks.size() - 1;
    int heavy = -1;
    for (size_t i = 0; i < m->heads.size(); ++i)
      if ((!use_side || m->heads[i].input == last) && (heavy < 0 || m->heads[i].c3.k > m->heads[heavy].c3.k)) heavy = (int)i;
    if (async_heads) heavy = -1;
    if (use_side) FR_TRY(ensure_side(m));
    for (size_t i = 0; use_side && i < m->heads.size(); ++i) {
      if (m->heads[i].input != last || (int)i == heavy) continue;
      FR_TRY(fork_to(m, s, head_stream(m, i), 16 + i));
      FR_TRY(head_forward(m, m->heads[i], w, head_stream(m, i), head_slot(m, i)));
    }
    for (size_t i = 0; i < m->heads.size(); ++i)
      if ((int)i == heavy || (!use_side)) FR_TRY(head_forward(m, m->heads[i], w, s, 0));
  }
  if (use_side && !async_heads) FR_TRY(join_side(m, s));
  return FRCNN_OK;
}

int frcnn_pnet_forward(frcnn_model* m, const float* w, const float* img, int H, int W, int training,
                       const float* const* drop_masks, unsigned long long seed, void* stream) {
  return pnet_forward_impl(m, w, img, H, W, training, drop_masks, seed, stream, false);
}

int frcnn_pnet_forward_async_heads(frcnn_model* m, const float* w, const float* img, int H, int W,
                                   const float* const* drop_masks, unsigned long long seed, void* stream) {
  return pnet_forward_impl(m, w, img, H, W, 1, drop_masks, seed, stream, true);
}

int frcnn_pnet_output(frcnn_model* m, int i, float** ptr, int* C, int* H, int* W) {
  FR_CHECK(m->H > 0, "pnet_output: call frcnn_pnet_forward first");
  FR_CHECK(i >= 1 && i <= (int)m->heads.size() + 1, "pnet_output: index %d out of range", i);
  if (i <= (int)m->heads.size()) {
    Head& h = m->heads[i - 1];
    *ptr = h.c1.x.f(); *C = HEAD_OUT; *H = h.c1.Ho; *W = h.c1.Wo;
  } else {
    Block& b = m->blocks.back();
    *ptr = b.pooled.f(); *C = m->d.filters[m->d.nblocks - 1]; *H = b.Hp; *W = b.Wp;
  }
  return FRCNN_OK;
}

int frcnn_model_debug_buffer(frcnn_model* m, int kind, int index, void** ptr, long long* bytes) {
  FR_CHECK(m && ptr && bytes, "frcnn_model_debug_buffer: NULL argument");
  const DevBuf* b = nullptr;
  size_t n = 0;
  switch (kind) {
    case 0: {
      FR_CHECK(index >= 0 && index < (int)m->convs.size() && m->H > 0, "debug_buffer: backbone convolution %d (after a forward pass)", index);
      const Conv& c = m->convs[index]; b = &c.x; n = (size_t)c.Cout * c.Ho * c.Wo * 4;
      const Block& k = m->blocks[c.block];
      if (k.dc_on && c.step == 0) {
        FR_HIP(hipDeviceSynchronize());
        FR_TRY(m->dbg_expand.ensure(n));
        FR_HIP(hipMemset(m->dbg_expand.p, 0, n));
        std::vector<int> idx(c.Cout);
        FR_HIP(hipMemcpy(idx.data(), k.dc_idx, (size_t)c.Cout * 4, hipMemcpyDeviceToHost));
        const size_t row = (size_t)c.Ho * c.Wo * 4;
        for (int i = 0; i < k.nk; ++i)
          FR_HIP(hipMemcpy((char*)m->dbg_expand.p + (size_t)idx[i] * row, (const char*)c.x.p + (size_t)i * row, row, hipMemcpyDeviceToDevice));
        b = &m->dbg_expand;
      }
    } break;
    case 4: {
      FR_CHECK(index >= 0 && index < (int)m->blocks.size() && m->H > 0 && m->blocks[index].has_drop, "debug_buffer: block %d has no dropout", index);
      const Block& k = m->blocks[index]; b = &k.scale; n = (size_t)m->d.filters[index] * 4;
    } break;
    case 1: {
      FR_CHECK(index >= 0 && index < (int)m->blocks.size() && m->H > 0, "debug_buffer: block %d (after a forward pass)", index);
      const Block& k = m->blocks[index]; b = &k.pidx; n = (size_t)m->d.filters[index] * k.Hp * k.Wp;
    } break;
    case 2: {
      FR_CHECK(index >= 0 && index < (int)m->heads.size() && m->H > 0, "debug_buffer: anchor net %d (after a forward pass)", index);
      const Conv& c = m->heads[index].c3; b = &c.x; n = (size_t)c.Cout * c.Ho * c.Wo * 4;
      if ((m->heads_sparse_fwd || m->heads_deferred) && m->last_w) {
        FR_HIP(hipDeviceSynchronize());
        if (!m->head_x3_fresh) { FR_TRY(refresh_group(m, m->last_w, (int)m->blocks.size(), nullptr)); m->head_x3_fresh = true; }
        FR_TRY(head_forward(m, m->heads[index], m->last_w, nullptr, 0));
        FR_HIP(hipDeviceSynchronize());
      }
    } break;
    case 3: {
      FR_CHECK(index >= 0 && index < (int)m->cls.size() && m->R > 0, "debug_buffer: classification layer %d (after frcnn_cnet_forward)", index);
      const ClsLayer& L = m->cls[index]; b = L.bn ? &L.pre : &L.lin; n = (size_t)m->R * L.n * 4;
    } break;
    default: FR_CHECK(false, "debug_buffer: unknown kind %d", kind);
  }
  FR_CHECK(b->p && b->bytes >= n, "debug_buffer: buffer not allocated yet");
  *ptr = b->p; *bytes = (long long)n;
  return FRCNN_OK;
}

int frcnn_pnet_delta(frcnn_model* m, int i, float** ptr) {
  FR_CHECK(m->H > 0, "pnet_delta: call frcnn_pnet_forward first");
  FR_CHECK(i >= 1 && i <= (int)m->heads.size() + 1, "pnet_delta: index %d out of range", i);
  *ptr = i <= (int)m->heads.size() ? m->heads[i - 1].delta.f() : m->delta_last.f();
  return FRCNN_OK;
}

int frcnn_pnet_set_sparse_deltas(frcnn_model* m, int head, const int* positions, int count) {
  FR_CHECK(head >= 1 && head <= (int)m->heads.size(), "pnet_set_sparse_deltas: head %d out of range", head);
  m->heads[head - 1].sp_pos = positions;
  m->heads[head - 1].sp_count = count;
  return FRCNN_OK;
}

int frcnn_pnet_zero_deltas(frcnn_model* m, void* stream) {
  FR_CHECK(m->H > 0, "pnet_zero_deltas: call frcnn_pnet_forward first");
  FR_TRY(fill_zero(m->zero_arena.p, m->delta_bytes, S(stream)));
  return FRCNN_OK;
}

static bool head_is_sparse(const Head& h) { return h.sp_count >= 0 && h.sp_count <= SPARSE_MAX_POS; }
static bool head_needs_gin(const frcnn_model* m, const Head& h) { return h.input >= m->frozen_blocks; }
static bool backbone_trained(const frcnn_model* m) { return m->frozen_blocks < (int)m->blocks.size(); }

static int backward_head(frcnn_model* m, Head& h, const float* w, float* grad, hipStream_t s, int ws_slot) {
  Block& in = m->blocks[h.input];
  Conv &a = h.c3, &c = h.c1;
  const long hw1 = (long)c.Ho * c.Wo;
  if (head_is_sparse(h)) {
    const int P = h.sp_count;
    const int* pos = h.sp_pos;
    h.sp_count = -1; h.sp_pos = nullptr;
    if (P == 0) return FRCNN_OK;
    const int n = a.Cout, ckk = a.Cin * a.k * a.k;
    FR_TRY(h.spD.ensure((size_t)HEAD_OUT * SPARSE_MAX_POS * 4));
    FR_TRY(h.spHX.ensure((size_t)n * SPARSE_MAX_POS * 4));
    FR_TRY(h.spHY.ensure((size_t)n * SPARSE_MAX_POS * 4));
    FR_TRY(h.spGH.ensure((size_t)n * SPARSE_MAX_POS * 4));
    FR_TRY(h.spCol.ensure((size_t)ckk * SPARSE_MAX_POS * 4));
    FR_TRY(h.spDX.ensure((size_t)ckk * SPARSE_MAX_POS * 4));
    float *D = h.spD.f(), *HX = h.spHX.f(), *HY = h.spHY.f(), *GH = h.spGH.f(), *COL = h.spCol.f(), *DX = h.spDX.f();
    FR_TRY(gather_positions(h.delta.f(), HEAD_OUT, hw1, pos, P, D, nullptr, nullptr, s));
    FR_TRY(gather_positions(a.x.f(), n, hw1, pos, P, HX, w + a.a_off, HY, s));
    FR_TRY(gemm_f32(w + c.w_off, 1, n, D, P, 1, GH, P, n, P, HEAD_OUT, OUT_STORE, nullptr, s, ws_slot));
    FR_TRY(act_backward(GH, HX, n, P, w + a.a_off, nullptr, GH, grad + a.b_off, grad + a.a_off, s));
    if (head_needs_gin(m, h)) {
      FR_TRY(gemm_f32(GH, 1, P, w + a.w_off, ckk, 1, DX, ckk, P, ckk, n, OUT_STORE, nullptr, s, ws_slot));
      FR_TRY(col2im_positions_add(DX, a.Cin, a.H, a.W, a.k, a.Wo, pos, P, in.gpooled.f(), s));
    }
    if (h.stream && s == h.stream) {
      if (!h.gin_done) FR_HIP(hipEventCreateWithFlags(&h.gin_done, hipEventDisableTiming));
      FR_HIP(hipEventRecord(h.gin_done, s));
      h.gin_recorded = true;
    }
    FR_TRY(gemm_f32(D, P, 1, HY, 1, P, grad + c.w_off, n, HEAD_OUT, n, P, OUT_ADD, nullptr, s, ws_slot));
    FR_TRY(channel_sum(D, HEAD_OUT, P, grad + c.b_off, s));
    FR_TRY(im2col_positions(in.pooled.f(), a.Cin, a.H, a.W, a.k, a.Wo, pos, P, COL, s));
    FR_TRY(gemm_f32(GH, P, 1, COL, ckk, 1, grad + a.w_off, ckk, n, ckk, P, OUT_ADD, nullptr, s, ws_slot));
    return FRCNN_OK;
  }
  h.sp_count = -1; h.sp_pos = nullptr;
  if (!m->head_packs_fresh) {
    FR_TRY(conv_pack_weights_multi(w, (const PackJob*)m->pack_jobs.p + m->n_pack_all + m->n_pack_fwd, m->n_pack_heads,
                                   m->pack_grid_heads, s));
    m->head_packs_fresh = true;
  }
  FR_TRY(conv_wgrad(a.x.f(), c.Cin, c.H, c.W, w + a.a_off, nullptr, h.delta.f(), HEAD_OUT, 1, 0, grad + c.w_off, m->wg_ws.p, m->wg_ws.bytes, s));
  FR_TRY(channel_sum(h.delta.f(), HEAD_OUT, hw1, grad + c.b_off, s));
  double f1 = 2.0 * HEAD_OUT * c.Cin * (double)hw1;
  FR_TRY(conv_igemm(h.delta.f(), HEAD_OUT, c.Ho, c.Wo, nullptr, nullptr, c.wd.f(), nullptr, c.Cin, 1, 0, a.gx.f(),
                    OUT_STORE, f1, s, ws_slot));
  FR_TRY(act_backward(a.gx.f(), a.x.f(), a.Cout, (long)a.Ho * a.Wo, w + a.a_off, nullptr, a.gx.f(),
                      grad + a.b_off, grad + a.a_off, s));
  FR_TRY(conv_wgrad(in.pooled.f(), a.Cin, a.H, a.W, nullptr, nullptr, a.gx.f(), a.Cout, a.k, 0, grad + a.w_off, m->wg_ws.p, m->wg_ws.bytes, s));
  if (!head_needs_gin(m, h)) return FRCNN_OK;
  double f3 = 2.0 * a.Cout * a.Cin * a.k * a.k * (double)a.Ho * a.Wo;
  FR_TRY(conv_igemm(a.gx.f(), a.Cout, a.Ho, a.Wo, nullptr, nullptr, a.wd.f(), nullptr, a.Cin, a.k, a.k - 1,
                    in.gpooled.f(), OUT_ADD, f3, s, ws_slot));
  return FRCNN_OK;
}

static int backward_heads(frcnn_model* m, const float* w, float* grad, hipStream_t s, int ws_slot) {
  for (auto& h : m->heads) FR_TRY(backward_head(m, h, w, grad, s, ws_slot));
  return FRCNN_OK;
}

static int backward_heads_fanout(frcnn_model* m, const float* w, float* grad) {
  FR_TRY(ensure_head_streams(m));
  if (backbone_trained(m)) FR_TRY(fill_zero((char*)m->zero_arena.p + m->delta_bytes, m->gpool_bytes, m->side));
  FR_HIP(hipEventRecord(m->chain_ev, m->side));
  for (auto& h : m->heads) h.gin_recorded = false;
  std::vector<char> own(m->heads.size(), 0);
  for (size_t i = 0; i < m->heads.size(); ++i) own[i] = m->heads[i].stream && head_is_sparse(m->heads[i]);
  bool any_dense = false;
  for (size_t i = 0; i < m->heads.size(); ++i) any_dense = any_dense || !head_is_sparse(m->heads[i]);
  if (any_dense || deterministic()) std::fill(own.begin(), own.end(), 0);
  for (size_t i = 0; i < m->heads.size(); ++i) {
    Head& h = m->heads[i];
    if (!own[i]) continue;
    FR_HIP(hipStreamWaitEvent(h.stream, m->chain_ev, 0));
    FR_TRY(backward_head(m, h, w, grad, h.stream, head_slot(m, i)));
  }
  for (size_t i = 0; i < m->heads.size(); ++i)
    if (!own[i]) FR_TRY(backward_head(m, m->heads[i], w, grad, m->side, 1));
  return FRCNN_OK;
}

static int heads_forward_dense(frcnn_model* m, const float* w, hipStream_t s) {
  FR_TRY(ensure_side(m));
  FR_TRY(ensure_head_streams(m));
  if (!m->head_x3_fresh) {
    FR_TRY(refresh_group(m, w, (int)m->blocks.size(), s));
    m->head_x3_fresh = true;
  }
  for (size_t i = 0; i < m->heads.size(); ++i) {
    FR_TRY(fork_to(m, s, head_stream(m, i), 16 + i));
    FR_TRY(head_forward(m, m->heads[i], w, head_stream(m, i), head_slot(m, i)));
  }
  m->heads_deferred = false;
  return FRCNN_OK;
}

static bool heads_all_sparse(const frcnn_model* m) {
  for (auto& h : m->heads) if (!head_is_sparse(h)) return false;
  return !m->heads.empty() && m->heads.size() <= 4;
}

static int heads_jobs(frcnn_model* m, const float* w, float* grad, HeadJobs& g) {
  g.n = 0;
  for (auto& h : m->heads) {
    const int P = h.sp_count;
    if (P <= 0) continue;
    Block& in = m->blocks[h.input];
    Conv &a = h.c3, &c = h.c1;
    const size_t n = (size_t)a.Cout, ckk = (size_t)a.Cin * a.k * a.k, cap = SPARSE_MAX_POS;
    FR_TRY(h.spD.ensure((size_t)HEAD_OUT * cap * 4)); FR_TRY(h.spOut.ensure((size_t)HEAD_OUT * cap * 4));
    FR_TRY(h.spHX.ensure(n * cap * 4)); FR_TRY(h.spHY.ensure(n * cap * 4)); FR_TRY(h.spGH.ensure(n * cap * 4));
    FR_TRY(h.spCol.ensure(ckk * cap * 4)); FR_TRY(h.spDX.ensure(ckk * cap * 4));
    HeadJob& j = g.j[g.n++];
    j.Cin = a.Cin; j.H = a.H; j.W = a.W; j.k = a.k; j.Ho = a.Ho; j.Wo = a.Wo; j.n = a.Cout;
    j.P = P; j.pos = h.sp_pos;
    j.in = in.pooled.f(); j.gin = in.gpooled.f();
    j.bias3 = w + a.b_off; j.slope = w + a.a_off; j.bias1 = w + c.b_off;
    j.gbias3 = grad ? grad + a.b_off : nullptr; j.gslope = grad ? grad + a.a_off : nullptr; j.gbias1 = grad ? grad + c.b_off : nullptr;
    j.out = c.x.f(); j.delta = h.delta.f();
    j.COL = h.spCol.f(); j.HX = h.spHX.f(); j.HY = h.spHY.f(); j.OUT = h.spOut.f(); j.D = h.spD.f(); j.GH = h.spGH.f(); j.DX = h.spDX.f();
// ... 269 lines not shown
    m->heads_begun = false; m->heads_joined = false; m->side_busy = false;
  } else if (!m->train_heads) {
    for (auto& h : m->heads) { h.sp_count = -1; h.sp_pos = nullptr; }
    m->heads_deferred = false;
    FR_TRY(join_side(m, s));
  } else {
    if (m->heads_deferred) {
      bool any = false;
      for (auto& h : m->heads) any = any || h.sp_count != 0;
      if (any) FR_TRY(heads_forward_dense(m, w, s));
      m->heads_deferred = false;
    }
    FR_TRY(join_side(m, s));
    if (backbone_trained(m)) FR_TRY(fill_zero((char*)m->zero_arena.p + m->delta_bytes, m->gpool_bytes, s));
    FR_TRY(backward_heads(m, w, grad, s, 0));
  }
  const int fb = m->frozen_blocks;
  if (fb < nb) {
    if (!m->train_heads) FR_TRY(fill_zero((char*)m->zero_arena.p + m->delta_bytes, m->gpool_bytes, s));
    Block& last = m->blocks.back();
    FR_TRY(add_inplace(last.gpooled.f(), m->delta_last.f(), (long)m->d.filters[nb - 1] * last.Hp * last.Wp, s));
  }
  if (m->update_armed) {
    if (!m->bwd_ev) FR_HIP(hipEventCreateWithFlags(&m->bwd_ev, hipEventDisableTiming));
    FR_HIP(hipEventRecord(m->bwd_ev, s));
  }
  for (int b = 0; b < fb; ++b) {
    while (m->block_ev.size() < (size_t)nb) {
      hipEvent_t e;
      FR_HIP(hipEventCreateWithFlags(&e, hipEventDisableTiming));
      m->block_ev.push_back(e);
    }
    FR_HIP(hipEventRecord(m->block_ev[b], s));
    FR_TRY(record_block_read(m, b, s));
  }
  const bool use_side = side_enabled();
  if (use_side) FR_TRY(ensure_side(m));
  hipStream_t ws = use_side ? m->side : s;
  size_t n_fork = 0;
  const bool fuse_act = !deterministic() && !(getenv("FRCNN_FUSE_ACT") && atoi(getenv("FRCNN_FUSE_ACT")) == 0);
  bool act_done = false;
  for (int b = nb - 1; b >= fb; --b) {
    Block& blk = m->blocks[b];
    for (int st = blk.nconv - 1; st >= 0; --st) {
      Conv& c = m->convs[blk.first_conv + st];
      const float* scale = (st == 0 && blk.has_drop) ? blk.scale.f() : nullptr;
      const bool fused_here = act_done;
      act_done = false;
      static const bool first_pooled_on = !(getenv("FRCNN_FIRST_POOLED") && atoi(getenv("FRCNN_FIRST_POOLED")) == 0);
      const bool first_pooled = fuse_act && first_pooled_on && b == 0 && st == 0 && blk.nconv == 1 && scale == nullptr &&
                                conv_wgrad_first_pooled_eligible(c.Cin, c.Cout, c.k, c.Wo);
      if (first_pooled) {
        FR_TRY(conv_wgrad_first_pooled(m->img.f(), c.Cin, c.H, c.W, blk.gpooled.f(), (const unsigned char*)blk.pidx.p, c.x.f(),
                                       w + c.a_off, c.Cout, c.pad, grad + c.w_off, grad + c.b_off, grad + c.a_off,
                                       m->wg_ws_first.p, m->wg_ws_first.bytes, s));
        while (m->block_ev.size() < (size_t)nb) {
          hipEvent_t e;
          FR_HIP(hipEventCreateWithFlags(&e, hipEventDisableTiming));
          m->block_ev.push_back(e);
        }
        FR_HIP(hipEventRecord(m->block_ev[b], s));
        FR_TRY(record_block_read(m, b, s));
        break;
      }
      if (fused_here) {
      } else if (st == blk.nconv - 1) {
        FR_TRY(maxpool_act_backward(blk.gpooled.f(), (const unsigned char*)blk.pidx.p, c.x.f(), c.Cout, c.Ho, c.Wo,
                                    w + c.a_off, scale, c.gx.f(), grad + c.b_off, grad + c.a_off, s,
                                    (c.x_d && m->f16_packed) ? m->rec(c.am + 1) : nullptr));
      } else {
        FR_TRY(act_backward(c.gx.f(), c.x.f(), c.Cout, (long)c.Ho * c.Wo, w + c.a_off, scale, c.gx.f(),
                            grad + c.b_off, grad + c.a_off, s, (c.x_d && m->f16_packed) ? m->rec(c.am + 1) : nullptr));
      }
      const float* in; const float* in_slope = nullptr; const float* in_scale = nullptr;
      if (st > 0) {
        Conv& pc = m->convs[blk.first_conv + st - 1];
        in = pc.x.f(); in_slope = w + pc.a_off;
        in_scale = (st - 1 == 0 && blk.has_drop) ? blk.scale.f() : nullptr;
      } else {
        in = b == 0 ? m->img.f() : m->blocks[b - 1].pooled.f();
      }
      const bool dc = blk.dc_on && st <= 1;
      int wg_cin = c.Cin, wg_o = c.Cout;
      WgradMap wmap;
      if (dc) {
        wmap.Cfull = c.Cin;
        if (st == 1) { wg_cin = blk.nkM; wmap.cmap = blk.dc_idx; in_scale = nullptr; }
        else { wg_o = blk.nkM; wmap.omap = blk.dc_idx; }
      }
      const float* wa_in = nullptr; const float* wa_g = nullptr;
      if (m->f16_packed && c.x_f && c.x_d && (st > 0 || b > 0)) {
        wa_in = st > 0 ? m->rec(m->convs[blk.first_conv + st - 1].am) : m->rec(m->blocks[b - 1].am);
        wa_g = m->rec(c.am + 1);
      }
      const bool on_caller = use_side && b == 0 && st == 0;
      if (use_side && !on_caller) FR_TRY(fork_side(m, s, n_fork++));
      if (on_caller) {
        FR_TRY(conv_wgrad(in, wg_cin, c.H, c.W, in_slope, in_scale, c.gx.f(), wg_o, c.k, c.pad, grad + c.w_off, m->wg_ws_first.p,
                          m->wg_ws_first.bytes, s, fused_here ? grad + c.b_off : nullptr, wa_in, wa_g, dc ? &wmap : nullptr));
        FR_HIP(hipEventRecord(m->join_ev, ws));
        FR_HIP(hipStreamWaitEvent(s, m->join_ev, 0));
      } else {
        FR_TRY(conv_wgrad(in, wg_cin, c.H, c.W, in_slope, in_scale, c.gx.f(), wg_o, c.k, c.pad, grad + c.w_off, m->wg_ws.p, m->wg_ws.bytes, ws,
                          fused_here ? grad + c.b_off : nullptr, wa_in, wa_g, dc ? &wmap : nullptr));
      }
      if (st == 0) {
        while (m->block_ev.size() < (size_t)nb) {
          hipEvent_t e;
          FR_HIP(hipEventCreateWithFlags(&e, hipEventDisableTiming));
          m->block_ev.push_back(e);
        }
        FR_HIP(hipEventRecord(m->block_ev[b], on_caller ? s : ws));
      }
      if (b == fb && st == 0) {
        FR_TRY(record_block_read(m, b, s));
        break;
      }
      float* gin = st > 0 ? m->convs[blk.first_conv + st - 1].gx.f() : m->blocks[b - 1].gpooled.f();
      const int gmode = st > 0 ? OUT_STORE : OUT_ADD;
      const float* ag = nullptr;
      const float* aw = nullptr;
      if (c.x_d && m->f16_packed) { ag = m->rec(c.am + 1); aw = m->amax_ws.f() + c.am; }
      const int dg_k = (dc && st == 0) ? blk.nkK : c.Cout, dg_m = (dc && st == 1) ? blk.nkM : c.Cin;
      const double fl = 2.0 * dg_k * dg_m * c.k * c.k * (double)c.Ho * c.Wo;
      if (c.x_d && st > 0 && fuse_act && c.k == 3) {
        Conv& pc = m->convs[blk.first_conv + st - 1];
        X3PostAct post{pc.x.f(), w + pc.a_off, (st - 1 == 0 && blk.has_drop && !dc) ? blk.scale.f() : nullptr, grad + pc.a_off};
        FR_TRY(conv_x3(c.gx.f(), dg_k, c.Ho, c.Wo, nullptr, nullptr, c.wxd.p, nullptr, dg_m, c.k, c.k - 1 - c.pad, gin, gmode, fl, s, 0, &post, ag, aw,
                       (pc.x_d && m->f16_packed) ? m->rec(pc.am + 1) : nullptr));
        act_done = true;
      } else if (c.x_d)
        FR_TRY(conv_x3(c.gx.f(), dg_k, c.Ho, c.Wo, nullptr, nullptr, c.wxd.p, nullptr, dg_m, c.k, c.k - 1 - c.pad, gin, gmode, fl, s, 0, nullptr, ag, aw));
      else
        FR_TRY(conv_igemm(c.gx.f(), c.Cout, c.Ho, c.Wo, nullptr, nullptr, c.wd.f(), nullptr, c.Cin, c.k,
                          c.k - 1 - c.pad, gin, gmode, fl, s));
      if (st == 0) FR_TRY(record_block_read(m, b, s));
    }
  }
  m->block_ev_valid = true;
  if (heads_tail && !m->heads_gin) FR_TRY(join_heads(m, s));
  FR_TRY(cw_join(m, s));
  if (use_side) {
    FR_HIP(hipEventRecord(m->join_ev, ws));
    FR_HIP(hipStreamWaitEvent(s, m->join_ev, 0));
    m->side_busy = false;
  }
  return FRCNN_OK;
}

static bool cnet_fuse() {
  const char* e = getenv("FRCNN_CNET_FUSE");
  return !(e && atoi(e) == 0);
}
static bool gemm_f16_on() {
  static const bool env_on = !(getenv("FRCNN_GEMM_F16") && atoi(getenv("FRCNN_GEMM_F16")) == 0);
  return env_on && get_x3_f16();
}
static int ensure_cnet(frcnn_model* m, int R) {
  for (auto& L : m->cls) {
    size_t n = (size_t)R * L.n * 4;
    FR_TRY(L.lin.ensure(n));
    if (L.bn) { FR_TRY(L.pre.ensure(n)); FR_TRY(L.xhat.ensure(n)); FR_TRY(L.invstd.ensure((size_t)L.n * 4)); }
    FR_TRY(L.post.ensure(n));
    FR_TRY(L.g.ensure(n));
    FR_TRY(L.gin.ensure((size_t)R * L.in * 4));
    if (L.p_drop > 0.f) FR_TRY(L.mask.ensure(n));
    L.x_form = 0;
    for (int role : {1, 2, 4}) if (linear_x_eligible(role, R, L.in, L.n)) L.x_form |= role;
    const size_t Rp = (size_t)linear_x_rows_padded(R);
    if (L.x_form & 1) FR_TRY(L.xp.ensure((size_t)3 * R * L.in * 2));
    if (L.x_form & 2) FR_TRY(L.gp.ensure((size_t)3 * R * L.n * 2));
    if (L.x_form & 4) { FR_TRY(L.xpT.ensure((size_t)3 * L.in * Rp * 2)); FR_TRY(L.gpT.ensure((size_t)3 * L.n * Rp * 2)); }
    if (L.x_form & 7) FR_TRY(L.am.ensure((size_t)5 * AMAX_REC * 4));
  }
  int nc = m->d.class_count + 1;
  int nf = m->cls.empty() ? m->D : m->cls.back().n;
  FR_TRY(m->feat_g.ensure((size_t)R * nf * 4));
  FR_TRY(m->logits.ensure((size_t)R * nc * 4));
  FR_TRY(m->lsm.ensure((size_t)R * nc * 4));
  FR_TRY(m->glog.ensure((size_t)R * nc * 4));
  return FRCNN_OK;
}

int frcnn_cnet_forward(frcnn_model* m, const float* weights, const float* x, int R, int training,
                       const float* const* drop_masks, unsigned long long seed, float* bn_running,
                       float* bbox_out, float* cls_out, void* stream) {
  hipStream_t s = S(stream);
  FR_CHECK(R > 0, "cnet_forward: empty batch");
  FR_TRY(cw_join(m, s));
  FR_TRY(ensure_cnet(m, R));
  m->R = R; m->cnet_x = x; m->training = training;
  const float* w = weights;
  const float* cur = x;
  float* bnr = bn_running;
  for (size_t l = 0; l < m->cls.size(); ++l) {
    ClsLayer& L = m->cls[l];
    GemmFold fold;
    GemmFold* defer = cnet_fuse() ? &fold : nullptr;
    if ((L.x_form & 3) && gemm_f16_on()) {
      float* rw = L.am.f() + 2 * AMAX_REC;
      const bool have = !training && g_static_weights && L.am_w_gen == g_static_gen && L.am_w_of == w;
      if (!have) FR_TRY(tensor_absmax(w + L.w_off, (long)L.n * L.in, rw, s));
      L.am_w_of = w; L.am_w_gen = training ? -1 : g_static_gen;
    } else {
      L.am_w_of = nullptr;
    }
    if ((L.x_form & 1) && gemm_f16_on()) {
      float* rx = L.am.f();
      FR_TRY(tensor_absmax(cur, (long)R * L.in, rx, s));
      FR_TRY(split_planes(cur, R, L.in, L.xp.p, nullptr, s, rx));
      FR_TRY(linear_x_forward(L.xp.p, R, L.in, w + L.w_off, w + L.b_off, L.n, L.lin.f(), s, 0, defer, rx, rx + 2 * AMAX_REC));
    } else if (L.x_form & 1) {
      FR_TRY(split_planes(cur, R, L.in, L.xp.p, nullptr, s));
      FR_TRY(linear_x_forward(L.xp.p, R, L.in, w + L.w_off, w + L.b_off, L.n, L.lin.f(), s, 0, defer));
    } else {
      FR_TRY(gemm_f32(cur, L.in, 1, w + L.w_off, 1, L.in, L.lin.f(), L.n, R, L.n, L.in, OUT_STORE, w + L.b_off, s, 0, defer));
    }
    if (L.bn) FR_CHECK(training || bnr, "cnet_forward: evaluate mode needs bn_running");
    const float* mask = nullptr;
    float inv_keep = 1.f;
    bool draw = false;
    if (training && L.p_drop > 0.f) {
      inv_keep = 1.0f / (1.0f - L.p_drop);
      if (drop_masks && drop_masks[l])
        FR_HIP(hipMemcpyAsync(L.mask.p, drop_masks[l], (size_t)R * L.n * 4, hipMemcpyDeviceToDevice, s));
      else
        draw = true;
      mask = L.mask.f();
    }
    if (defer) {
      FR_TRY(cnet_act_forward(L.lin.f(), fold, R, L.n, L.bn ? w + L.bnw_off : nullptr, L.bn ? w + L.bnb_off : nullptr, L.bn ? bnr : nullptr,
                              training, L.lin.f(), L.xhat.f(), L.invstd.f(), L.pre.f(), w + L.a_off, const_cast<float*>(mask), draw,
                              inv_keep, L.p_drop, seed * 977 + l + 17, L.post.f(), s));
      if (L.bn && bnr) bnr += 2 * L.n;
      cur = L.post.f();
      continue;
    }
    const float* pre = L.lin.f();
    if (L.bn) {
      FR_TRY(bn_forward(L.lin.f(), R, L.n, w + L.bnw_off, w + L.bnb_off, bnr, training, L.xhat.f(), L.invstd.f(),
                        L.pre.f(), s));
      if (bnr) bnr += 2 * L.n;
      pre = L.pre.f();
    }
    if (draw)
      FR_TRY(prelu_dropout_forward_gen(pre, (long)R * L.n, w + L.a_off, L.mask.f(), L.p_drop, seed * 977 + l + 17,
                                       L.post.f(), s));
    else
      FR_TRY(prelu_dropout_forward(pre, (long)R * L.n, w + L.a_off, mask, inv_keep, L.post.f(), s));
    cur = L.post.f();
  }
  const int nf = m->cls.empty() ? m->D : m->cls.back().n;
  const int nc = m->d.class_count + 1;
  if (cnet_fuse() && cnet_heads_fused_eligible(nf, nc)) {
    return cnet_heads_forward(cur, R, nf, w + m->bbox_w_off, w + m->bbox_b_off, w + m->clsw_off, w + m->clsb_off, nc, bbox_out,
                              m->logits.f(), m->lsm.f(), cls_out, s);
  }
  FR_TRY(gemm_f32(cur, nf, 1, w + m->bbox_w_off, 1, nf, bbox_out, 4, R, 4, nf, OUT_STORE, w + m->bbox_b_off, s));
  if (cnet_fuse()) {
    GemmFold fold;
    FR_TRY(gemm_f32(cur, nf, 1, w + m->clsw_off, 1, nf, m->logits.f(), nc, R, nc, nf, OUT_STORE, w + m->clsb_off, s, 0, &fold));
    FR_TRY(log_softmax_rows_fold(m->logits.f(), fold, R, nc, m->lsm.f(), cls_out, s));
    return FRCNN_OK;
  }
  FR_TRY(gemm_f32(cur, nf, 1, w + m->clsw_off, 1, nf, m->logits.f(), nc, R, nc, nf, OUT_STORE, w + m->clsb_off, s));
  FR_TRY(log_softmax_rows(m->logits.f(), R, nc, m->lsm.f(), s));
  FR_HIP(hipMemcpyAsync(cls_out, m->lsm.p, (size_t)R * nc * 4, hipMemcpyDeviceToDevice, s));
  return FRCNN_OK;
}

int frcnn_cnet_backward(frcnn_model* m, const float* weights, const float* g_bbox, const float* g_cls, float* gx,
                        float* grad, void* stream) {
  hipStream_t s = S(stream);
  FR_CHECK(m->R > 0, "cnet_backward: call frcnn_cnet_forward first");
  const int R = m->R;
  const float* w = weights;
  const int nf = m->cls.empty() ? m->D : m->cls.back().n;
  const int nc = m->d.class_count + 1;
  const float* feat = m->cls.empty() ? m->cnet_x : m->cls.back().post.f();
  if (m->frozen_blocks >= (int)m->blocks.size()) gx = nullptr;
  FR_TRY(cw_join(m, s));
  const bool async = g_cnet_wgrad_async && !deterministic();
  if (async && !m->cw) {
    FR_TRY(pool_stream(1, &m->cw));
    FR_HIP(hipEventCreateWithFlags(&m->cw_done, hipEventDisableTiming));
  }
  while (async && m->cw_ev.size() < m->cls.size() + 1) {
    hipEvent_t e;
    FR_HIP(hipEventCreateWithFlags(&e, hipEventDisableTiming));
    m->cw_ev.push_back(e);
  }
  hipStream_t ws = async ? m->cw : s;
  const int wslot = async ? 7 : 0;
  size_t nfork = 0;
  auto fork = [&]() -> int {
    if (!async) return FRCNN_OK;
    FR_HIP(hipEventRecord(m->cw_ev[nfork], s));
    FR_HIP(hipStreamWaitEvent(ws, m->cw_ev[nfork], 0));
    ++nfork;
    return FRCNN_OK;
  };
  bool top_act_done = false;
  if (cnet_fuse() && cnet_heads_fused_eligible(nf, nc)) {
    HeadsPostAct post;
    float* dst = m->feat_g.f();
    if (!m->cls.empty() && !m->cls.back().bn && !deterministic()) {
      ClsLayer& T = m->cls.back();
      const bool drop = m->training && T.p_drop > 0.f;
      post.pre = T.lin.f(); post.mask = drop ? T.mask.f() : nullptr; post.inv_keep = drop ? 1.0f / (1.0f - T.p_drop) : 1.f;
      post.slope = w + T.a_off; post.gslope = grad + T.a_off;
      dst = T.g.f();
      top_act_done = true;
    }
    FR_TRY(cnet_heads_backward(g_bbox, g_cls, m->lsm.f(), R, nf, w + m->bbox_w_off, w + m->clsw_off, nc, m->glog.f(), dst, s,
                               top_act_done ? &post : nullptr));
    FR_TRY(fork());
  } else {
    FR_TRY(log_softmax_backward(g_cls, m->lsm.f(), R, nc, m->glog.f(), s));
    FR_TRY(fork());
    FR_TRY(gemm_f32(g_bbox, 4, 1, w + m->bbox_w_off, nf, 1, m->feat_g.f(), nf, R, nf, 4, OUT_STORE, nullptr, s));
    FR_TRY(gemm_f32(m->glog.f(), nc, 1, w + m->clsw_off, nf, 1, m->feat_g.f(), nf, R, nf, nc, OUT_ADD, nullptr, s));
  }
  FR_TRY(gemm_f32(g_bbox, 1, 4, feat, nf, 1, grad + m->bbox_w_off, nf, 4, nf, R, OUT_ADD, nullptr, ws, wslot));
  FR_TRY(channel_sum_cols(g_bbox, R, 4, grad + m->bbox_b_off, ws));
  FR_TRY(gemm_f32(m->glog.f(), 1, nc, feat, nf, 1, grad + m->clsw_off, nf, nc, nf, R, OUT_ADD, nullptr, ws, wslot));
  FR_TRY(channel_sum_cols(m->glog.f(), R, nc, grad + m->clsb_off, ws));
  const float* g = m->feat_g.f();
  GemmFold gfold;
  for (int l = (int)m->cls.size() - 1; l >= 0; --l) {
    ClsLayer& L = m->cls[l];
    const float* pre = L.bn ? L.pre.f() : L.lin.f();
    const bool drop = m->training && L.p_drop > 0.f;
    if (top_act_done && l == (int)m->cls.size() - 1) {
    } else if (L.bn && cnet_fuse()) {
      FR_TRY(cnet_act_bn_backward(g, gfold, pre, L.xhat.f(), L.invstd.f(), w + L.bnw_off, w + L.a_off, drop ? L.mask.f() : nullptr,
                                  drop ? 1.0f / (1.0f - L.p_drop) : 1.f, R, L.n, m->training, L.g.f(), grad + L.bnw_off,
                                  grad + L.bnb_off, grad + L.a_off, s));
    } else {
      FR_TRY(prelu_dropout_backward(g, pre, (long)R * L.n, w + L.a_off, drop ? L.mask.f() : nullptr,
                                    drop ? 1.0f / (1.0f - L.p_drop) : 1.f, L.g.f(), grad + L.a_off, s));
      if (L.bn)
        FR_TRY(bn_backward(L.g.f(), L.xhat.f(), L.invstd.f(), w + L.bnw_off, R, L.n, m->training, L.g.f(),
                           grad + L.bnw_off, grad + L.bnb_off, s));
    }
    gfold = GemmFold{};
    GemmFold* gdefer = (cnet_fuse() && async && l > 0 && m->cls[l - 1].bn) ? &gfold : nullptr;
    FR_TRY(fork());
    const float* in = l == 0 ? m->cnet_x : m->cls[l - 1].post.f();
    float* gin = l == 0 ? gx : L.gin.f();
    const bool xw = (L.x_form & 4) != 0, xd = (L.x_form & 2) != 0 && gin;
    if (xd && gemm_f16_on() && L.am_w_of == w) {
      float* rg = L.am.f() + AMAX_REC;
      FR_TRY(tensor_absmax(L.g.f(), (long)R * L.n, rg, s));
      FR_TRY(split_planes(L.g.f(), R, L.n, L.gp.p, nullptr, s, rg));
      FR_TRY(linear_x_dgrad(L.gp.p, R, L.n, w + L.w_off, L.in, gin, OUT_STORE, s, 0, gdefer, rg, L.am.f() + 2 * AMAX_REC));
    } else if (xd) {
      FR_TRY(split_planes(L.g.f(), R, L.n, L.gp.p, nullptr, s));
      FR_TRY(linear_x_dgrad(L.gp.p, R, L.n, w + L.w_off, L.in, gin, OUT_STORE, s, 0, gdefer));
    } else if (gin) {
      FR_TRY(gemm_f32(L.g.f(), L.n, 1, w + L.w_off, L.in, 1, gin, L.in, R, L.in, L.n, OUT_STORE, nullptr, s, 0, gdefer));
    }
    static const bool wgrad_f16 = !(getenv("FRCNN_GEMM_WGRAD_F16") && atoi(getenv("FRCNN_GEMM_WGRAD_F16")) == 0);
    if (xw && wgrad_f16 && gemm_f16_on() && L.am.bytes >= (size_t)5 * AMAX_REC * 4) {
      float *rgT = L.am.f() + 3 * AMAX_REC, *rxT = L.am.f() + 4 * AMAX_REC;
      FR_TRY(tensor_absmax(L.g.f(), (long)R * L.n, rgT, ws));
      if ((L.x_form & 1) && L.am_w_of == w) rxT = L.am.f();
      else FR_TRY(tensor_absmax(in, (long)R * L.in, rxT, ws));
      FR_TRY(split_planes(L.g.f(), R, L.n, nullptr, L.gpT.p, ws, rgT));
      FR_TRY(split_planes(in, R, L.in, nullptr, L.xpT.p, ws, rxT));
      FR_TRY(linear_x_wgrad(L.gpT.p, L.xpT.p, R, L.n, L.in, grad + L.w_off, ws, wslot, rgT, rxT));
    } else if (xw) {
      FR_TRY(split_planes(L.g.f(), R, L.n, nullptr, L.gpT.p, ws));
      FR_TRY(split_planes(in, R, L.in, nullptr, L.xpT.p, ws));
      FR_TRY(linear_x_wgrad(L.gpT.p, L.xpT.p, R, L.n, L.in, grad + L.w_off, ws, wslot));
    } else {
      FR_TRY(gemm_f32(L.g.f(), 1, L.n, in, L.in, 1, grad + L.w_off, L.in, L.n, L.in, R, OUT_ADD, nullptr, ws, wslot));
    }
    FR_TRY(channel_sum_cols(L.g.f(), R, L.n, grad + L.b_off, ws));
    g = gin;
  }
  if (m->cls.empty() && gx) FR_HIP(hipMemcpyAsync(gx, g, (size_t)R * m->D * 4, hipMemcpyDeviceToDevice, s));
  if (async) {
    FR_HIP(hipEventRecord(m->cw_done, ws));
    m->cw_pending = true;
  }
  return FRCNN_OK;
}

}
```

faster-rcnn.torch_amd/csrc/roi.hip:

```cpp
#include "kernels.h"
#include "roi_fix.h"

namespace frcnn {

__global__ void roi_pool_forward_kernel(const float* __restrict__ fmap, int C, int H, int W,
                                        const int* __restrict__ wins, int R, int kh, int kw,
                                        float* __restrict__ out, int* __restrict__ idx) {
  const long total = (long)R * C * kh * kw;
  for (long t = (long)blockIdx.x * blockDim.x + threadIdx.x; t < total; t += (long)gridDim.x * blockDim.x) {
    int j = (int)(t % kw);
    long q = t / kw;
    int i = (int)(q % kh);
    q /= kh;
    int c = (int)(q % C);
    int r = (int)(q / C);
    const int* wn = wins + 4 * r;
    const int r0 = wn[0] - 1, c0 = wn[2] - 1;
    const int h = wn[1] - wn[0] + 1, w = wn[3] - wn[2] + 1;
    const int ys = (i * h) / kh, ye = ((i + 1) * h + kh - 1) / kh;
    const int xs = (j * w) / kw, xe = ((j + 1) * w + kw - 1) / kw;
    const float* ip = fmap + (size_t)c * H * W;
    float best = -3.402823466e+38f;
    int bi = -1;
    for (int y = ys; y < ye; ++y)
      for (int x = xs; x < xe; ++x) {
        float v = ip[(size_t)(r0 + y) * W + (c0 + x)];
        if (v > best) { best = v; bi = (r0 + y) * W + (c0 + x); }
      }
    out[t] = best;
    if (idx) idx[t] = bi;
  }
}

__global__ __launch_bounds__(256) void roi_pool_forward_cells_kernel(const float* __restrict__ fmap, int C, int H, int W,
                                                                     const int* __restrict__ wins, int kh, int kw,
                                                                     float* __restrict__ out, int* __restrict__ idx) {
  const int r = blockIdx.x, cells = kh * kw, groups = blockDim.x / cells;
  const int tid = threadIdx.x;
  if (tid >= groups * cells) return;
  const int cg = tid / cells, cell = tid - cg * cells;
  const int i = cell / kw, j = cell - i * kw;
  const int* wn = wins + 4 * r;
  const int r0 = wn[0] - 1, c0 = wn[2] - 1;
  const int h = wn[1] - wn[0] + 1, w = wn[3] - wn[2] + 1;
  const int ys = (i * h) / kh, ye = ((i + 1) * h + kh - 1) / kh;
  const int xs = (j * w) / kw, xe = ((j + 1) * w + kw - 1) / kw;
  const int HW = H * W;
  const int base = (r0 + ys) * W + c0 + xs, nx = xe - xs, ny = ye - ys;
  if (HW >= 4) {
    for (int c = blockIdx.y * groups + cg; c < C; c += gridDim.y * groups) {
      const float* ip = fmap + (size_t)c * HW;
      float best = -3.402823466e+38f;
      int bi = -1;
      for (int y = 0, o = base; y < ny; ++y, o += W)
        for (int x = 0; x < nx; x += 4) {
          const int q = min(o + x, HW - 4);
          float v[4];
          __builtin_memcpy(v, ip + q, 16);
#pragma unroll
          for (int e = 0; e < 4; ++e) {
            const int at = q + e;
            if (at >= o && at < o + nx && v[e] > best) { best = v[e]; bi = at; }
          }
        }
      const size_t t = ((size_t)r * C + c) * cells + cell;
      out[t] = best;
      if (idx) idx[t] = bi;
    }
    return;
  }
  for (int c = blockIdx.y * groups + cg; c < C; c += gridDim.y * groups) {
    const float* ip = fmap + (size_t)c * HW;
    float best = -3.402823466e+38f;
    int bi = -1;
    for (int y = 0, o = base; y < ny; ++y, o += W)
      for (int x = 0; x < nx; ++x) {
        const float v = ip[o + x];
        if (v > best) { best = v; bi = o + x; }
      }
    const size_t t = ((size_t)r * C + c) * cells + cell;
    out[t] = best;
    if (idx) idx[t] = bi;
  }
}

int roi_pool_forward(const float* fmap, int C, int H, int W, const int* wins, int R, int kh, int kw,
                     float* out, int* idx, hipStream_t s) {
  if (R <= 0) return FRCNN_OK;
  long total = (long)R * C * kh * kw;
  if (kh * kw <= 256) {
    const int groups = 256 / (kh * kw);
    const int slices = std::max(1, std::min(cdiv(C, groups), (int)cdivl(4096, R)));
    FR_LAUNCH(KC_ROI, 0, total * 8.0, s, roi_pool_forward_cells_kernel, dim3(R, slices), dim3(256), 0, fmap, C, H, W,
              wins, kh, kw, out, idx);
    FR_LAUNCH_CHECK();
    return FRCNN_OK;
  }
  int grid = (int)std::min<long>(cdivl(total, 256), 4096);
  FR_LAUNCH(KC_ROI, 0, total * 8.0, s, roi_pool_forward_kernel, dim3(grid), dim3(256), 0, fmap, C, H, W,
            wins, R, kh, kw, out, idx);
  FR_LAUNCH_CHECK();
  return FRCNN_OK;
}

__global__ void roi_pool_backward_lds_kernel(float* __restrict__ gmap, int C, int HW, const float* __restrict__ gout,
                                             const int* __restrict__ idx, int R, int cell) {
  extern __shared__ float plane[];
  const int c = blockIdx.x;
  for (int i = threadIdx.x; i < HW; i += blockDim.x) plane[i] = 0.f;
  __syncthreads();
  const long D = (long)C * cell;
  const int total = R * cell;
  for (int e = threadIdx.x; e < total; e += blockDim.x) {
    const int r = e / cell, j = e - r * cell;
    const long t = (long)r * D + (long)c * cell + j;
    const int bi = idx[t];
    const float g = gout[t];
    if (bi >= 0 && g != 0.f) atomicAdd(&plane[bi], g);
  }
  __syncthreads();
  float* gp = gmap + (size_t)c * HW;
  for (int i = threadIdx.x; i < HW; i += blockDim.x) {
    const float v = plane[i];
    if (v != 0.f) gp[i] += v;
  }
}

__global__ void roi_pool_backward_lds_det_kernel(float* __restrict__ gmap, int C, int HW, const float* __restrict__ gout,
                                                 const int* __restrict__ idx, int R, int cell) {
  extern __shared__ unsigned long long fplane[];
  const int c = blockIdx.x;
  for (int i = threadIdx.x; i < HW; i += blockDim.x) fplane[i] = 0ull;
  __syncthreads();
  const long D = (long)C * cell;
  const int total = R * cell;
  for (int e = threadIdx.x; e < total; e += blockDim.x) {
    const int r = e / cell, j = e - r * cell;
    const long t = (long)r * D + (long)c * cell + j;
    const int bi = idx[t];
    const float g = gout[t];
    if (bi >= 0 && g != 0.f) atomicAdd(&fplane[bi], (unsigned long long)roi_to_fix(g));
  }
  __syncthreads();
  float* gp = gmap + (size_t)c * HW;
  for (int i = threadIdx.x; i < HW; i += blockDim.x) {
    const long long v = (long long)fplane[i];
    if (v != 0) gp[i] += (float)((double)v / ROI_FIX_SCALE);
  }
}
__global__ void roi_pool_backward_det_kernel(unsigned long long* __restrict__ fix, int C, long HW,
                                             const float* __restrict__ gout, const int* __restrict__ idx,
                                             long total, int cell) {
  for (long t = (long)blockIdx.x * blockDim.x + threadIdx.x; t < total; t += (long)gridDim.x * blockDim.x) {
    int c = (int)((t / cell) % C);
    int bi = idx[t];
    float g = gout[t];
    if (bi >= 0 && g != 0.f) atomicAdd(fix + (size_t)c * HW + bi, (unsigned long long)roi_to_fix(g));
  }
}
__global__ void roi_fix_apply_kernel(const unsigned long long* __restrict__ fix, long n, float* __restrict__ gmap) {
  for (long t = (long)blockIdx.x * blockDim.x + threadIdx.x; t < n; t += (long)gridDim.x * blockDim.x) {
    const long long v = (long long)fix[t];
    if (v != 0) gmap[t] += (float)((double)v / ROI_FIX_SCALE);
  }
}

int roi_fix_apply(const unsigned long long* fix, long n, float* gmap, hipStream_t s) {
  FR_LAUNCH(KC_ROI, 0, n * 16.0, s, roi_fix_apply_kernel, dim3((int)std::min<long>(cdivl(n, 256), 4096)), dim3(256), 0, fix, n, gmap);
  FR_LAUNCH_CHECK();
  return FRCNN_OK;
}

__global__ void roi_pool_backward_kernel(float* __restrict__ gmap, int C, long HW,
                                         const float* __restrict__ gout, const int* __restrict__ idx,
                                         long total, int cell) {
  for (long t = (long)blockIdx.x * blockDim.x + threadIdx.x; t < total; t += (long)gridDim.x * blockDim.x) {
    int c = (int)((t / cell) % C);
    int bi = idx[t];
    float g = gout[t];
    if (bi >= 0 && g != 0.f) unsafeAtomicAdd(gmap + (size_t)c * HW + bi, g);
  }
}

int roi_pool_backward(float* gmap, int C, int H, int W, const float* gout, const int* idx, int R,
                      int kh, int kw, hipStream_t s) {
  if (R <= 0) return FRCNN_OK;
  long total = (long)R * C * kh * kw;
  if (deterministic()) {
    if ((size_t)H * W * 8 <= 64 * 1024) {
      FR_LAUNCH(KC_ROI, 0, total * 12.0, s, roi_pool_backward_lds_det_kernel, dim3(C), dim3(256), (size_t)H * W * 8, gmap, C,
                H * W, gout, idx, R, kh * kw);
    } else {
      float* ws = nullptr;
      const long n = (long)C * H * W;
      FR_TRY(det_workspace(s, (size_t)n * 2, &ws));
      FR_HIP(hipMemsetAsync(ws, 0, (size_t)n * 8, s));
      int grid = (int)std::min<long>(cdivl(total, 256), 4096);
      FR_LAUNCH(KC_ROI, 0, total * 12.0, s, roi_pool_backward_det_kernel, dim3(grid), dim3(256), 0, (unsigned long long*)ws, C,
                (long)H * W, gout, idx, total, kh * kw);
      FR_LAUNCH_CHECK();
      return roi_fix_apply((const unsigned long long*)ws, n, gmap, s);
    }
    FR_LAUNCH_CHECK();
    return FRCNN_OK;
  }
  if ((size_t)H * W * 4 <= 64 * 1024) {
    FR_LAUNCH(KC_ROI, 0, total * 12.0, s, roi_pool_backward_lds_kernel, dim3(C), dim3(1024), (size_t)H * W * 4, gmap, C,
              H * W, gout, idx, R, kh * kw);
    FR_LAUNCH_CHECK();
    return FRCNN_OK;
  }
  int grid = (int)std::min<long>(cdivl(total, 256), 4096);
  FR_LAUNCH(KC_ROI, 0, total * 12.0, s, roi_pool_backward_kernel, dim3(grid), dim3(256), 0, gmap, C,
            (long)H * W, gout, idx, total, kh * kw);
  FR_LAUNCH_CHECK();
  return FRCNN_OK;
}

}
```

faster-rcnn.torch_amd/model_utilities.py:

```python
import ctypes as C

import numpy as np

from . import _lib
from .tensor import DeviceTensor, ptr, stream_ptr, to_device


class _Node(object):

    def __init__(self, layers):
        self.layers = layers


class _OutNode(object):
    def __init__(self, children):
        self.children = children


class NativeModel(object):

    def __init__(self, cfg, layers, anchor_nets, class_layers):
        d = _lib.ModelDesc()
        d.nblocks = len(layers)
        for i, l in enumerate(layers):
# ... 68 lines not shown


class ProposalNet(object):

    def __init__(self, native):
        self.native = native
        self.train = True
        n_out = native.desc.nheads + 1
        self.outnode = _OutNode([_Node(native.localizer_layers(i + 1)) for i in range(n_out)])
        self.drop_masks = None
        self.output = None

    def cuda(self):
        return self

    def training(self):
        self.train = True

    def evaluate(self):
        self.train = False

    def forward(self, img, async_heads=False):
        nat = self.native
        if nat.weights is None:
            raise _lib.FrcnnError("pnet:forward before combine_and_flatten_parameters()")
        img = to_device(img)
        assert len(img.shape) == 3 and img.shape[0] == 3, "expected a 3xHxW image"
        _, H, W = img.shape
        arr, keep = _mask_ptrs(self.drop_masks, nat.desc.nblocks)
        nat.seed += 1
        if async_heads and self.train:
            _lib.call("frcnn_pnet_forward_async_heads", nat.h, ptr(nat.weights), ptr(img), H, W,
                      C.cast(arr, C.c_void_p) if arr is not None else None, nat.seed, stream_ptr())
        else:
            _lib.call("frcnn_pnet_forward", nat.h, ptr(nat.weights), ptr(img), H, W, 1 if self.train else 0,
                      C.cast(arr, C.c_void_p) if arr is not None else None, nat.seed, stream_ptr())
        outs = []
        for i in range(1, nat.desc.nheads + 2):
            p = C.c_void_p(); c = C.c_int(); h = C.c_int(); w = C.c_int()
            _lib.call("frcnn_pnet_output", nat.h, i, C.byref(p), C.byref(c), C.byref(h), C.byref(w))
            outs.append(DeviceTensor(p.value, (c.value, h.value, w.value), np.float32, owner=nat))
        self.output = outs
        return outs

    def delta_outputs(self, zero=True):
        nat = self.native
        if zero:
            _lib.call("frcnn_pnet_zero_deltas", nat.h, stream_ptr())
        res = []
        for i, o in enumerate(self.output):
            p = C.c_void_p()
            _lib.call("frcnn_pnet_delta", nat.h, i + 1, C.byref(p))
            res.append(DeviceTensor(p.value, o.shape, np.float32, owner=nat))
        return res

    def backward(self, img, delta_outputs):
        nat = self.native
        own = self.delta_outputs(zero=False)
        for mine, given in zip(own, delta_outputs):
            if ptr(given).value != mine.ptr:
                mine.copy_(given)
        _lib.call("frcnn_pnet_backward", nat.h, ptr(nat.weights), ptr(nat.gradient), stream_ptr())
        return None

    def backward_heads_begin(self):
        nat = self.native
        _lib.call("frcnn_pnet_backward_heads_begin", nat.h, ptr(nat.weights), ptr(nat.gradient), stream_ptr())

    def anchor_loss_begin(self, d_idx, d_anchor, d_roi, d_class, npos, nneg, bgclass, ex_loss, crtarget, cctarget, acc):
        nat = self.native
        _lib.call("frcnn_pnet_anchor_loss_begin", nat.h, ptr(nat.weights), ptr(nat.gradient), C.c_void_p(d_idx),
                  C.c_void_p(d_anchor), C.c_void_p(d_roi), C.c_void_p(d_class), npos, nneg, bgclass, ptr(ex_loss),
                  ptr(crtarget), ptr(cctarget), ptr(acc), stream_ptr())

    def anchor_loss_wait(self):
        _lib.call("frcnn_pnet_anchor_loss_wait", self.native.h, stream_ptr())

    def backward_heads_join(self):
        joined = C.c_int(0)
        _lib.call("frcnn_pnet_backward_heads_join", self.native.h, stream_ptr(), C.byref(joined))
        return bool(joined.value)

    def block_param_range(self, b):
        d = self.native.desc
        first = sum(int(d.conv_steps[i]) for i in range(b))
        n = int(d.conv_steps[b])
        t = self.native.param_table
        last = t[3 * (first + n) - 1]
        return int(t[3 * first][0]), int(last[0]) + int(last[1])

    def wait_block_gradients(self, b):
        _lib.call("frcnn_pnet_wait_block_gradients", self.native.h, b + 1, stream_ptr())

    def heads_param_range(self):
        d = self.native.desc
        nconv = sum(int(d.conv_steps[b]) for b in range(d.nblocks))
        return int(self.native.param_table[3 * nconv][0]), int(self.native.pnet_params)

    def parameters(self):
        return _param_views(self.native, 0, self.native.pnet_params)


class ClassificationNet(object):

    def __init__(self, native):
        self.native = native
        self.train = True
        self.drop_masks = None
        self.output = None
        self._bufs = {}
        self._pending = None

    def _buf(self, name, shape):
        need = int(np.prod(shape)) * 4
        b = self._bufs.get(name)
        if b is None or b.nbytes < need:
            b = DeviceTensor.empty((max(need, 256),), np.uint8)
            self._bufs[name] = b
        return DeviceTensor(b.ptr, shape, np.float32, owner=b)

    def cuda(self):
        return self

    def training(self):
        self.train = True

    def evaluate(self):
        self.train = False

    def forward(self, cinput, out=None):
        nat = self.native
        cinput = to_device(cinput)
        R, D = cinput.shape
        nc = nat.desc.class_count + 1
        bbox, cls = out if out is not None else (self._buf("bbox", (R, 4)), self._buf("cls", (R, nc)))
        arr, keep = _mask_ptrs(self.drop_masks, nat.desc.ncls)
        nat.seed += 1
        self._input = cinput
        _lib.call("frcnn_cnet_forward", nat.h, ptr(nat.weights), ptr(cinput), R, 1 if self.train else 0,
                  C.cast(arr, C.c_void_p) if arr is not None else None, nat.seed, ptr(nat.bn_running), ptr(bbox),
                  ptr(cls), stream_ptr())
        self.output = [bbox, cls]
        return self.output

    def backward(self, cinput, grad_outputs):
        nat = self.native
        R, D = self._input.shape
        gx = self._buf("gx", (R, D))
        _lib.call("frcnn_cnet_backward", nat.h, ptr(nat.weights), ptr(grad_outputs[0]), ptr(grad_outputs[1]), ptr(gx),
                  ptr(nat.gradient), stream_ptr())
        self._pending = (self._input, grad_outputs[0], grad_outputs[1])
        return gx

    def join_backward(self):
        _lib.call("frcnn_cnet_backward_join", self.native.h, stream_ptr())
        self._pending = None

    def parameters(self):
        return _param_views(self.native, self.native.pnet_params, self.native.total_params)


def _param_views(native, lo, hi):
    if native.weights is None:
        raise _lib.FrcnnError("parameters() before combine_and_flatten_parameters()")
    ws, gs = [], []
    for off, cnt, kind, aux in native.param_table:
        if lo <= off < hi:
            ws.append(native.weights[off:off + cnt])
            gs.append(native.gradient[off:off + cnt])
    return ws, gs


def create_model(cfg, layers, anchor_nets, class_layers):
    native = NativeModel(cfg, layers, anchor_nets, class_layers)
    return dict(cfg=cfg, layers=layers, anchor_nets=anchor_nets, class_layers=class_layers,
                pnet=ProposalNet(native), cnet=ClassificationNet(native), native=native)
```

faster-rcnn.torch_amd/objective.py:

```python
import ctypes as C
import os
import sys

import numpy as np

from . import _lib
from .Anchors import Anchors
from .Localizer import Localizer
from .Rect import Rect
from .tensor import DeviceTensor, ptr, stream_ptr, to_device


def roi_window(input_rect, localizer, fm_h, fm_w):
    r = localizer.inputToFeatureRect(input_rect)
    r = r.clip(Rect(0, 0, fm_w, fm_h))
    return (int(min(r.minY + 1, r.maxY)), int(r.maxY), int(min(r.minX + 1, r.maxX)), int(r.maxX))


def roi_windows(rects, localizer, fm_h, fm_w):
    r = localizer.inputToFeatureRectBatch(rects)
    minX = np.minimum(np.maximum(r[:, 0], 0), fm_w); minY = np.minimum(np.maximum(r[:, 1], 0), fm_h)
    maxX = np.maximum(np.minimum(r[:, 2], fm_w), 0); maxY = np.maximum(np.minimum(r[:, 3], fm_h), 0)
    return np.stack([np.minimum(minY + 1, maxY), maxY, np.minimum(minX + 1, maxX), maxX], 1).astype(np.int32)

# ... 272 lines not shown
        ex_idx = np.array([(a.layer, a.aspect, a.index[1], a.index[2]) for a in anch], dtype=np.int32)
        ex_anchor = np.array([(a.minX, a.minY, a.maxX, a.maxY) for a in anch], dtype=np.float64)
        ex_roi = np.zeros((max(npos, 1), 4), dtype=np.float64)
        ex_class = np.zeros(max(npos, 1), dtype=np.int32)
        if npos:
            ex_roi[:npos] = [(e[1].rect.minX, e[1].rect.minY, e[1].rect.maxX, e[1].rect.maxY) for e in p]
            ex_class[:npos] = [e[1].class_index for e in p]
            if ex_class[:npos].min() < 1 or ex_class[:npos].max() > cfg["class_count"]:
                raise _lib.FrcnnError("roi.class_index %d outside 1..%d (class_count)"
                                      % (int(ex_class[:npos].min() if ex_class[:npos].min() < 1 else ex_class[:npos].max()),
                                         cfg["class_count"]))
        pooled = np.concatenate([ex_roi[:npos], ex_anchor[npos:]], 0)
        wins = np.ascontiguousarray(pooled) if align else roi_windows(pooled, localizer, fmH, fmW)
        sp = []
        for l in range(4):
            sel = ex_idx[ex_idx[:, 0] == l + 1]
            sp.append(np.unique((sel[:, 2] - 1) * sizes[l][1] + (sel[:, 3] - 1)).astype(np.int32))
        sp_all = np.concatenate(sp)
        head = [ex_anchor.view(np.uint8).ravel(), ex_roi.view(np.uint8).ravel(), ex_idx.view(np.uint8).ravel(),
                ex_class.view(np.uint8).ravel()]
        if align:
            head.append(np.zeros(-sum(a.size for a in head) % 8, np.uint8))
        blob = np.concatenate(head + [wins.view(np.uint8).ravel(), sp_all.view(np.uint8).ravel()])
        prep.update(ex_anchor=ex_anchor, ex_roi=ex_roi, ex_idx=ex_idx, ex_class=ex_class, wins=wins, sp=sp, blob=blob)
        return prep

    nblk_all = int(native.desc.nblocks)

    def stage_ranges():
        fb, prop, clsf = train_settings(model["cfg"], nblk_all)
        ranges = trainable_ranges([pnet.block_param_range(b) for b in range(nblk_all)], pnet.heads_param_range(),
                                  (native.pnet_params, gradient.numel()), fb, prop, clsf)
        return fb, prop, clsf, (None if ranges == [(0, gradient.numel())] else ranges)

    def run(w, defer, eager=None):
        guarded, guard["armed"] = guard["armed"], False
        guard["deferred"] = False
        guard["divisor"] = None
        frozen_blocks, proposal, classification, ranges = stage_ranges()
        _lib.call("frcnn_model_set_trainable", native.h, frozen_blocks, int(proposal), int(classification))
        stage[0] = ranges
        trunk_frozen = frozen_blocks == nblk_all
        if w is not weights:
            weights.copy_(w)
        if packs_promise[0] is not None and packs_promise[0] != getattr(weights, "_version", None):
            _lib.call("frcnn_pnet_invalidate_packs", native.h)
        packs_promise[0] = None
        s = stream_ptr()
        probing = exchange_probe is not None and _dist() is None and getattr(gradient, "is_cuda", False)
        if probing:
            _probe_mark("step_begin", 0, 0, "")
        _lib.call("frcnn_zero", ptr(gradient), gradient.numel() * 4, s)
        cls_count = reg_count = creg_count = ccls_count = 0
        pnet.training()
        cnet.training()
        batch = next_batch[0] if next_batch[0] is not None else batch_iterator.nextTraining()
        next_batch[0] = None
        pending = []
        early_copy = False
        if eager is not None:
            side = C.c_int(0)
            _lib.call("frcnn_get_option", b"side_stream", C.byref(side))
            if not (defer == "fold" and _dist() is None and len(batch) == 1 and side.value and w is weights
                    and getattr(gradient, "is_cuda", False)):
                eager = None
        if eager is not None:
            from .synthetic import clean_examples, output_map_sizes
            x0 = batch[0]
            held0 = prepared.get(id(x0))
            if held0 is not None and held0[0] is x0:
                n_ex = len(held0[1]["p"]) + len(held0[1]["n"])
            else:
                sizes0 = output_map_sizes(model, x0["img"].shape[1], x0["img"].shape[2])
                n_ex = len(clean_examples(x0["positive"], sizes0)) + len(clean_examples(x0["negative"], sizes0))
            eager["gscale"] = (1.0 / n_ex) if n_ex > 0 else 1.0
            eager["done"] = []
            eager["ranges"] = ranges
            us = C.c_void_p()
            _lib.call("frcnn_model_update_stream", native.h, C.byref(us))
            nblk = int(native.desc.nblocks)

            def eager_slice(lo, hi, on, group=None):
                eager["update"](weights, gradient, lo, hi, eager["gscale"], on)
                eager["done"].append((int(lo), int(hi)))
                if group is not None:
                    _lib.call("frcnn_pnet_refresh_packs", native.h, ptr(weights), group, on)
                    eager["groups"].add(group)
            eager["groups"] = set()
            eager["slice"] = eager_slice
        dev_tail = (dev_tail_ok and defer == "fold" and _dist() is not None and getattr(gradient, "is_cuda", False)
                    and ranges is None)
        c4 = None
        if dev_tail:
            from .synthetic import clean_examples, output_map_sizes
            c4 = [0.0, 0.0, 0.0, 0.0]
            for x in batch:
                shp = x["img"].shape
                sizes = output_map_sizes(model, shp[1], shp[2])
                np_, nn_ = len(clean_examples(x["positive"], sizes)), len(clean_examples(x["negative"], sizes))
                c4[0] += np_ + nn_; c4[1] += np_; c4[2] += np_; c4[3] += 1
            init = np.array([0.0, 0.0, c4[0], c4[1], 0.0, 0.0, c4[2], c4[3]], dtype=np.float64)
            hinit, staged = pinned.stage(init.view(np.uint8))
            _lib.call("frcnn_memcpy_h2d", ptr(acc_dev), C.c_void_p(hinit), 64, s)
            staged()
        else:
            acc_dev.zero_()
        for bi, x in enumerate(batch):
            last = bi == len(batch) - 1
            held = prepared.pop(id(x), None)
            prep = held[1] if held is not None and held[0] is x else prepare_examples(x)
            img = to_device(x["img"])
            outputs = pnet.forward(img, async_heads=True)
            if prep["sizes"] != [tuple(o.shape[1:]) for o in outputs[:len(prep["sizes"])]] or prep["fm"] != tuple(outputs[-1].shape[1:]):
                raise _lib.FrcnnError("lossAndGradient: the example tables were packed for other map sizes than this image's")
            p, n = prep["p"], prep["n"]
            delta_outputs = pnet.delta_outputs(zero=True)
            npos, nneg = len(p), len(n)
            E = npos + nneg
            fm = outputs[-1]
            fmC, fmH, fmW = fm.shape
            if E > 0:
                ex_anchor, ex_roi, ex_idx, ex_class, wins, sp, blob = (prep[k] for k in ("ex_anchor", "ex_roi", "ex_idx", "ex_class", "wins", "sp", "blob"))
                dblob = scratch.get("blob", (blob.size,), np.uint8)
                hblob, staged = pinned.stage(blob)
                _lib.call("frcnn_memcpy_h2d", ptr(dblob), C.c_void_p(hblob), blob.nbytes, s)
                staged()
                o = 0
                d_anchor = dblob.ptr + o; o += ex_anchor.nbytes
                d_roi = dblob.ptr + o; o += ex_roi.nbytes
                d_idx = dblob.ptr + o; o += ex_idx.nbytes
                d_class = dblob.ptr + o; o += ex_class.nbytes
                if align:
                    o += -o % 8
                d_wins = dblob.ptr + o; o += wins.nbytes
                for l in range(4):
                    _lib.call("frcnn_pnet_set_sparse_deltas", native.h, l + 1, C.c_void_p(dblob.ptr + o), len(sp[l]))
                    o += sp[l].nbytes
                ex_loss = scratch.get("ex_loss", (E, 2), np.float64)
                crtarget = scratch.get("crtarget", (E, 4))
                cctarget = scratch.get("cctarget", (E,))
                pnet.anchor_loss_begin(d_idx, d_anchor, d_roi, d_class, npos, nneg, bgclass, ex_loss, crtarget,
                                       cctarget, acc_dev)
            if E > 0 and not classification:
                native.seed += 1
                pnet.anchor_loss_wait()
            elif E > 0:
                cinput = scratch.get("cinput", (E, D))
                if align:
                    debug["rects"] = wins
                    _lib.call("frcnn_roi_align_forward", ptr(fm), fmC, fmH, fmW, C.c_void_p(d_wins), None, E, inv_sx, inv_sy,
                              kh, kw, sampling, ptr(cinput), s)
                else:
                    pidx = scratch.get("pidx", (E, D), np.int32)
                    _lib.call("frcnn_roi_pool_forward", ptr(fm), fmC, fmH, fmW, C.c_void_p(d_wins), E, kh, kw,
                              ptr(cinput), ptr(pidx), s)
                coutputs = cnet.forward(cinput)
                crout, ccout = coutputs
                crdelta = scratch.get("crdelta", (E, 4))
                ccdelta = scratch.get("ccdelta", (E, ncls))
                pnet.anchor_loss_wait()
                _lib.call("frcnn_cnet_losses", ptr(crout), ptr(crtarget), ptr(ccout), ptr(cctarget), E, npos, ncls,
                          ptr(crdelta), ptr(ccdelta), C.c_void_p(acc_dev.ptr + 4 * 8), s)
                post_roi_delta = cnet.backward(cinput, [crdelta, ccdelta])
                if not trunk_frozen and align:
                    _lib.call("frcnn_roi_align_backward", ptr(delta_outputs[4]), fmC, fmH, fmW, ptr(post_roi_delta),
                              C.c_void_p(d_wins), None, E, inv_sx, inv_sy, kh, kw, sampling, s)
                elif not trunk_frozen:
                    _lib.call("frcnn_roi_pool_backward", ptr(delta_outputs[4]), fmC, fmH, fmW, ptr(post_roi_delta),
                              ptr(pidx), E, kh, kw, s)
            if E == 0:
                for l in range(4):
                    _lib.call("frcnn_pnet_set_sparse_deltas", native.h, l + 1, None, 0)
            if last and _dist() is not None:
                _lib.call("frcnn_cnet_backward_join", native.h, stream_ptr())
                if classification:
                    pending.append(allreduce_begin(gradient, native.pnet_params, gradient.numel()))
                side = C.c_int(0)
                _lib.call("frcnn_get_option", b"side_stream", C.byref(side))
                if len(batch) == 1 and side.value and proposal:
                    pnet.backward_heads_join()
                    lo, hi = pnet.heads_param_range()
                    pending.append(allreduce_begin(gradient, lo, hi))
            if last and probing:
                _lib.call("frcnn_cnet_backward_join", native.h, stream_ptr())
                _probe_mark("classification net", native.pnet_params, gradient.numel(), "frcnn_cnet_backward_join (its weight-gradient stream)")
                side = C.c_int(0)
                _lib.call("frcnn_get_option", b"side_stream", C.byref(side))
                if len(batch) == 1 and side.value:
                    pnet.backward_heads_join()
                    lo, hi = pnet.heads_param_range()
                    _probe_mark("anchor nets", lo, hi, "frcnn_pnet_backward_heads_join (the anchor nets' streams)")
            if last and defer and _dist() is None and not guarded:
                acc_pin.copy_(acc_t, non_blocking=True)
                acc_event.record()
                early_copy = True
            debug["E"] = E
            pnet.backward(img, delta_outputs)
            if eager is not None:
                _lib.call("frcnn_pnet_wait_backward_begun", native.h, us)
                if classification:
                    eager_slice(native.pnet_params, gradient.numel(), us)
                _lib.call("frcnn_pnet_wait_heads_done", native.h, us)
                lo, hi = pnet.heads_param_range()
                if proposal:
                    eager_slice(lo, hi, us, nblk)
                for b in range(nblk, max(frozen_blocks, 1), -1):
                    _lib.call("frcnn_pnet_wait_block_done", native.h, b, us)
                    lo, hi = pnet.block_param_range(b - 1)
                    eager_slice(lo, hi, us, b - 1)
                _lib.call("frcnn_model_update_join", native.h, stream_ptr())
            if last and _dist() is not None and early_blocks and getattr(gradient, "is_cuda", False):
                if aux_stream[0] is None:
                    aux_stream[0] = torch.cuda.Stream()
                for b in [b for b in early_blocks if b >= frozen_blocks]:
                    lo, hi = pnet.block_param_range(b)
                    with torch.cuda.stream(aux_stream[0]):
                        pnet.wait_block_gradients(b)
                        pending.append(allreduce_begin(gradient, lo, hi))
            if last and probing:
                covered = []
                if early_blocks:
                    if aux_stream[0] is None:
                        aux_stream[0] = torch.cuda.Stream()
                    for b in early_blocks:
                        lo, hi = pnet.block_param_range(b)
                        with torch.cuda.stream(aux_stream[0]):
                            pnet.wait_block_gradients(b)
                            _probe_mark("backbone block %d" % (b + 1), lo, hi, "frcnn_pnet_wait_block_gradients(%d) on an auxiliary stream" % (b + 1))
                        covered.append((lo, hi))
                _probe_mark("backward_end", 0, 0, "")
                lo_rest = 0
                hi_rest = min([c[0] for c in covered] + [pnet.heads_param_range()[0]])
                _probe_mark("rest of the backbone", lo_rest, hi_rest, "end of frcnn_pnet_backward on the caller's stream")
            reg_count += npos
            cls_count += npos + nneg
            creg_count += npos
            ccls_count += 1

        single = _dist() is None
        fold = single and defer == "fold" and cls_count > 0
        if single and cls_count > 0 and not fold:
            _lib.call("frcnn_scale", ptr(gradient), gradient.numel(), 1.0 / cls_count, stream_ptr())
        counts = (cls_count, reg_count, creg_count, ccls_count)
        if not single:
            pending[:] = allreduce_begin_rest(gradient, pending, ranges)
        if dev_tail:
            assert [float(v) for v in (cls_count, reg_count, creg_count, ccls_count)] == c4, "count bookkeeping diverged"
            acc_work = _dist().all_reduce(acc_t, async_op=True)
            for pnd in pending:
                pnd[2].wait()
            acc_work.wait()
            if not guarded:
                acc_pin.copy_(acc_t, non_blocking=True)
                acc_event.record()
            fin = lambda: finish(None, None, (), True, reduced=True)
            guard["deferred"] = guarded
            guard["divisor"] = DeviceDivisor(acc_dev.ptr + 2 * 8, acc_all)
            return (fin, DeviceDivisor(acc_dev.ptr + 2 * 8, acc_t))
        if single and defer:
            if not early_copy and not guarded:
                acc_pin.copy_(acc_t, non_blocking=True)
                acc_event.record()
            guard["deferred"] = guarded
            guard["divisor"] = float(cls_count) if cls_count > 0 else None
            fin = lambda: finish(None, counts, pending, single, staged=(classification, ranges))
            if eager is not None:
                assert cls_count == 0 or eager["gscale"] == 1.0 / cls_count, "example count bookkeeping diverged"
                return (fin, eager["gscale"] if cls_count > 0 else None)
            return (fin, 1.0 / cls_count) if fold else fin
        if defer == "fold" and not single:
            res = finish(acc_dev.numpy(), counts, pending, single, fold=True, staged=(classification, ranges))
            gs = dp_gscale[0]
            guard["divisor"] = dp_count[0]
            fin = (lambda: (guard_stats(acc_all[8:12].cpu().numpy()), res)[1]) if guarded else (lambda: res)
            return (fin, gs) if gs is not None else fin
        return (lambda r: (lambda: r))(finish(acc_dev.numpy(), counts, pending, single, staged=(classification, ranges)))

    dp_gscale = [None]
    dp_count = [None]
    packs_promise = [None]
    debug = dict(scratch=scratch, E=0)
    next_batch = [None]
    prefetch_batches = os.environ.get("FRCNN_PREFETCH_BATCH", "1") != "0"

    stage = [None]

    def finish(a, counts, pending, single, fold=False, reduced=False, staged=(True, None)):
        if a is None:
            if next_batch[0] is None and prefetch_batches:
                next_batch[0] = batch_iterator.nextTraining()
                prepared.clear()
                for xb in next_batch[0]:
                    prepared[id(xb)] = (xb, prepare_examples(xb))
            acc_event.synchronize()
            a = (guard["pin"] if guard["deferred"] else acc_pin).numpy().copy()
        if counts is None:
            counts = (a[2], a[3], a[6], a[7])
        cls_count, reg_count, creg_count, ccls_count = counts
        tot = np.array([a[0], a[1], cls_count, reg_count, a[4], creg_count, a[5], ccls_count], dtype=np.float64)
        if not reduced:
            tot = allreduce_gradient_and_stats(gradient, tot, pending, staged[1])
        cls_loss, reg_loss, cls_count, reg_count, creg_loss, creg_count, ccls_loss, ccls_count = tot
        dp_gscale[0] = dp_count[0] = None
        if not single and cls_count > 0:
            if fold:
                dp_gscale[0] = 1.0 / cls_count
                dp_count[0] = float(cls_count)
            else:
                _lib.call("frcnn_scale", ptr(gradient), gradient.numel(), 1.0 / cls_count, stream_ptr())
        with np.errstate(divide="ignore", invalid="ignore"):
            pcls = float(np.float64(cls_loss) / cls_count)
            preg = float(np.float64(reg_loss) / reg_count)
            dcls = float(np.float64(ccls_loss) / ccls_count)
            dreg = float(np.float64(creg_loss) / creg_count)
        if not staged[0]:
            dcls = dreg = float("nan")
        if stats.get("verbose"):
            print("prop: cls: %f (%d), reg: %f (%d); det: cls: %f, reg: %f" % (pcls, cls_count, preg, reg_count, dcls, dreg))
        stats["pcls"].append(pcls); stats["preg"].append(preg)
        stats["dcls"].append(dcls); stats["dreg"].append(dreg)
        if guard["deferred"]:
            guard_stats(a[8:12])
# ... 54 lines not shown
```

include/frcnn_hip.h:

```cpp
#ifndef FRCNN_HIP_H
#define FRCNN_HIP_H

#include <stddef.h>

#ifdef __cplusplus
extern "C" {
#endif

#define FRCNN_OK 0
#define FRCNN_ERR_ARG 1
#define FRCNN_ERR_HIP 2
#define FRCNN_ERR_STATE 3

int frcnn_version(void);
const char *frcnn_last_error(void);
int frcnn_device_count(int *n);
int frcnn_set_device(int device);
int frcnn_device_name(char *buf_host, int len);
int frcnn_set_option(const char *name, int value);
int frcnn_get_option(const char *name, int *value_host);

int frcnn_malloc(void **ptr_out_host, size_t bytes);
int frcnn_free(void *ptr);
int frcnn_host_alloc(void **ptr_out_host, size_t bytes);
// ... 56 lines not shown
                         int k, int pad, float *out, void *stream);
int frcnn_conv2d_backward_input(const float *gout, int O, int Ho, int Wo, const float *weight,
                                int C, int k, int pad, float *gin, int accumulate, void *stream);
int frcnn_conv2d_backward_weight(const float *in, int C, int H, int W, const float *in_slope,
                                 const float *in_scale, const float *gout, int O, int k, int pad,
                                 float *gweight, float *gbias, void *stream);

int frcnn_maxpool_act_forward(const float *x, int C, int H, int W, const float *slope,
                              const float *scale, float *out, unsigned char *idx, void *stream);
int frcnn_maxpool_act_backward(const float *gpool, const unsigned char *idx, const float *x, int C,
                               int H, int W, const float *slope, const float *scale, float *gx,
                               float *gbias, float *gslope, void *stream);
int frcnn_act_forward(const float *x, int C, long long hw, const float *slope, const float *scale,
                      float *y, void *stream);
int frcnn_act_backward(const float *gy, const float *x, int C, long long hw, const float *slope,
                       const float *scale, float *gx, float *gbias, float *gslope, void *stream);

int frcnn_roi_pool_forward(const float *fmap, int C, int H, int W, const int *wins, int R, int kh,
                           int kw, float *out, int *idx, void *stream);
int frcnn_roi_pool_backward(float *gmap, int C, int H, int W, const float *gout, const int *idx,
                            int R, int kh, int kw, void *stream);

int frcnn_roi_align_forward(const float *fmap, int C, int H, int W, const double *rect, const long long *pick, int R,
                            double inv_sx, double inv_sy, int kh, int kw, int g, float *out, void *stream);
int frcnn_roi_align_backward(float *gmap, int C, int H, int W, const float *gout, const double *rect, const long long *pick,
                             int R, double inv_sx, double inv_sy, int kh, int kw, int g, void *stream);

size_t frcnn_rpn_scan_workspace_bytes(const int *H_host, const int *W_host);
int frcnn_rpn_scan(const float *const *maps_host, const int *H_host, const int *W_host,
                   const float *anchor_w, const float *anchor_h, double img_w, double img_h,
                   double p_threshold, int cap, float *match_p, int *match_idx,
                   double *match_rect, float *match_box, int *count, void *workspace,
                   size_t workspace_bytes, void *stream);
size_t frcnn_rpn_scan_batch_workspace_bytes(const int *H_host, const int *W_host, int B);
int frcnn_rpn_scan_batch(const float *const *maps_host, const int *H_host, const int *W_host, int B, long long slot_stride,
                         const float *anchor_w, const float *anchor_h, double img_w, double img_h, double p_threshold,
                         int cap, float *match_p, int *match_idx, double *match_rect, float *match_box, int *count,
                         void *workspace, size_t workspace_bytes, void *stream);

size_t frcnn_topk_select_workspace_bytes(int B, int n_cap);
int frcnn_topk_select(const float *score, int B, long long stride, int n_cap, const int *n_dev, int K, int *sel_row,
                      long long sel_stride, int *k_dev, void *workspace, size_t workspace_bytes, void *stream);
int frcnn_rpn_gather_rows(const float *match_p, const int *match_idx, const double *match_rect, const float *match_box, int B,
                          long long src_stride, int src_rows, const int *sel_row, long long sel_stride, const int *k_dev,
                          int k_cap, float *dst_p, int *dst_idx, double *dst_rect, float *dst_box, float *box5, int *row,
                          long long dst_stride, void *stream);

int frcnn_rpn_loss(const float *const *maps_host, float *const *deltas_host, const int *H_host,
                   const int *W_host, const int *ex_idx, const double *ex_anchor,
                   const double *ex_roi, const int *ex_class, int npos, int nneg, int bgclass,
                   double *ex_loss, float *crtarget, float *cctarget, void *stream);

int frcnn_loss_accumulate(const double *ex_loss, int E, double *acc, void *stream);

int frcnn_linear_forward(const float *x, int R, int I, const float *weight, const float *bias,
                         int O, float *y, void *stream);
int frcnn_linear_backward(const float *x, const float *gy, int R, int I, const float *weight,
                          int O, float *gx, float *gweight, float *gbias, void *stream);

int frcnn_rmsprop(float *x, const float *g, float *m, long long n, float lr, float alpha,
                  float eps, void *stream);
int frcnn_scale_rmsprop(float *x, float *g, float gscale, float *m, long long n, float lr, float alpha,
                        float eps, void *stream);
int frcnn_scale_rmsprop_dev(float *x, float *g, const double *gcount_dev, float *m, long long n, float lr,
                            float alpha, float eps, void *stream);
int frcnn_scale_rmsprop_slice(float *x, float *g, float gscale, float *m, long long lo, long long hi, float lr,
                              float alpha, float eps, void *stream);

int frcnn_sgd(float *x, float *g, float *v, long long n, float gscale, const double *gcount_dev, float clr, float wd,
              float mom, float one_minus_damp, int nesterov, int first, void *stream);
int frcnn_sgd_slice(float *x, float *g, float *v, long long lo, long long hi, float gscale, float clr, float wd, float mom,
                    float one_minus_damp, int nesterov, int first, void *stream);
int frcnn_nag(float *x, float *g, float *v, long long n, float gscale, const double *gcount_dev, float clr, float wd,
              float mom, int first, void *stream);
int frcnn_nag_slice(float *x, float *g, float *v, long long lo, long long hi, float gscale, float clr, float wd, float mom,
                    int first, void *stream);
int frcnn_scale_rmsprop_slice_dev(float *x, float *g, const double *gcount_dev, float *m, long long lo, long long hi,
                                  float lr, float alpha, float eps, void *stream);
int frcnn_sgd_slice_dev(float *x, float *g, float *v, long long lo, long long hi, const double *gcount_dev, float clr,
                        float wd, float mom, float one_minus_damp, int nesterov, int first, void *stream);
int frcnn_nag_slice_dev(float *x, float *g, float *v, long long lo, long long hi, const double *gcount_dev, float clr,
                        float wd, float mom, int first, void *stream);

size_t frcnn_grad_clip_workspace_bytes(long long n);
int frcnn_grad_clip(float *g, long long n, const long long *ranges_host, int nranges, double divisor,
                    const double *divisor_dev, double clip_norm, double *record_dev, void *workspace,
                    size_t workspace_bytes, void *stream);

int frcnn_nag_lookahead(float *x, const float *v, long long n, float mom, void *stream);
int frcnn_nag_lookahead_slice(float *x, const float *v, long long lo, long long hi, float mom, void *stream);

typedef struct {
  int nblocks;
  int filters[8], ksize[8], pad[8], conv_steps[8];
  float dropout[8];
  int nheads;
  int head_k[8], head_n[8], head_input[8];
  int ncls;
  int cls_n[8], cls_bn[8];
  float cls_dropout[8];
  int class_count;
  int kh, kw;
} frcnn_model_desc;

typedef struct frcnn_model frcnn_model;

int frcnn_model_create(const frcnn_model_desc *desc_host, frcnn_model **out_host);
int frcnn_model_destroy(frcnn_model *);
int frcnn_model_param_count(const frcnn_model *, long long *total_host, long long *pnet_host);
int frcnn_model_param_table(const frcnn_model *, long long *table_host, int cap, int *n_host);
int frcnn_model_localizer_layers(const frcnn_model *, int output_index, int *layers_host, int cap,
                                 int *n_host);
int frcnn_model_set_trainable(frcnn_model *, int frozen_blocks, int heads, int cnet);
int frcnn_model_get_trainable(const frcnn_model *, int *frozen_blocks_host, int *heads_host, int *cnet_host);

int frcnn_pnet_forward(frcnn_model *, const float *weights, const float *img, int H, int W,
                       int training, const float *const *drop_masks_host, unsigned long long seed,
                       void *stream);
int frcnn_pnet_forward_async_heads(frcnn_model *, const float *weights, const float *img, int H, int W,
                                   const float *const *drop_masks_host, unsigned long long seed,
                                   void *stream);
int frcnn_pnet_output(frcnn_model *, int i, float **ptr_host, int *C_host, int *H_host,
                      int *W_host);
int frcnn_model_debug_buffer(frcnn_model *, int kind, int index, void **ptr_host, long long *bytes_host);
int frcnn_pnet_delta(frcnn_model *, int i, float **ptr_host);
int frcnn_pnet_zero_deltas(frcnn_model *, void *stream);
int frcnn_pnet_set_sparse_deltas(frcnn_model *, int head, const int *positions, int count);
int frcnn_pnet_backward_heads_begin(frcnn_model *, const float *weights, float *grad, void *stream);
int frcnn_pnet_anchor_loss_begin(frcnn_model *, const float *weights, float *grad, const int *ex_idx,
                                 const double *ex_anchor, const double *ex_roi, const int *ex_class,
                                 int npos, int nneg, int bgclass, double *ex_loss, float *crtarget,
                                 float *cctarget, double *acc, void *stream);
int frcnn_pnet_anchor_loss_wait(frcnn_model *, void *stream);
int frcnn_pnet_backward_heads_join(frcnn_model *, void *stream, int *joined_host);
int frcnn_pnet_backward(frcnn_model *, const float *weights, float *grad, void *stream);

int frcnn_pnet_wait_block_gradients(frcnn_model *, int block, void *stream);

int frcnn_model_update_stream(frcnn_model *, void **stream_host);
int frcnn_model_update_fork(frcnn_model *, void *stream);
int frcnn_model_update_join(frcnn_model *, void *stream);
int frcnn_pnet_wait_backward_begun(frcnn_model *, void *stream);
int frcnn_pnet_wait_heads_done(frcnn_model *, void *stream);
int frcnn_pnet_wait_block_done(frcnn_model *, int block, void *stream);
int frcnn_pnet_refresh_packs(frcnn_model *, const float *weights, int group, void *stream);
int frcnn_pnet_invalidate_packs(frcnn_model *);

int frcnn_cnet_forward(frcnn_model *, const float *weights, const float *x, int R, int training,
                       const float *const *drop_masks_host, unsigned long long seed,
                       float *bn_running, float *bbox_out, float *cls_out, void *stream);
int frcnn_cnet_backward_join(frcnn_model *, void *stream);
int frcnn_cnet_backward(frcnn_model *, const float *weights, const float *g_bbox,
                        const float *g_cls, float *gx, float *grad, void *stream);
int frcnn_cnet_losses(float *crout, const float *crtarget, const float *ccout,
                      const float *cctarget, int R, int npos, int ncls, float *crdelta,
                      float *ccdelta, double *loss2, void *stream);
int frcnn_cnet_decode(const float *cls_out, int R, int ncls, int *cls, float *conf, void *stream);

int frcnn_image_rgb2yuv(const float *rgb, float *yuv, int H, int W, void *stream);
int frcnn_image_rgb2hsv(const float *rgb, float *hsv, int H, int W, void *stream);
int frcnn_image_rgb2lab(const float *rgb, float *lab, int H, int W, void *stream);
int frcnn_image_scale(const float *src, int C, int H, int W, float *dst, int dH, int dW, float *tmp,
                      int rgb2yuv, void *stream);
int frcnn_image_scale_u8(const unsigned char *src_hwc, int H, int W, float *dst, int dH, int dW,
                         float *tmp, int rgb2yuv, void *stream);
int frcnn_image_crop_flip(const float *src, int C, int H, int W, int x0, int y0, int w, int h, int hflip,
                          int vflip, float *dst, void *stream);
size_t frcnn_image_normalize_workspace_bytes(int C);
int frcnn_image_normalize(float *img, int C, int H, int W, int centering, int scaling, void *workspace,
                          size_t workspace_bytes, void *stream);
int frcnn_image_contrastive_norm(const float *in, int H, int W, const float *kernel_host, int K,
                                 float threshold, float *out, float *tmp, void *stream);

typedef struct frcnn_anchors frcnn_anchors;
int frcnn_anchors_create(const float *w_tab_host, const float *h_tab_host, const double *cx_host,
                         const double *cy_host, int nscales, int width, frcnn_anchors **out_host);
int frcnn_anchors_destroy(frcnn_anchors *);
int frcnn_anchors_assemble(frcnn_anchors *, const double *rois_host, int nroi, double img_w, double img_h,
                           double pos_thr, double neg_thr, int best_match, int nearby_aversion,
                           int negatives, unsigned int *mt_state_host, int *mt_index_host, int *ex_host,
                           double *ex_rect_host, int cap, int *npos_host, int *nneg_host);

#define FRCNN_COMM_ID_BYTES 128
typedef struct frcnn_comm frcnn_comm;
int frcnn_comm_get_unique_id(void *id_host);
int frcnn_comm_exchange_id_file(const char *path, int rank, void *id_host, int timeout_ms);
int frcnn_comm_init_rank(frcnn_comm **out_host, int nranks, int rank, const void *id_host);
int frcnn_comm_init_rank_timeout(frcnn_comm **out_host, int nranks, int rank, const void *id_host, int timeout_ms);
int frcnn_comm_init_rank_file(frcnn_comm **out_host, int nranks, int rank, const char *path, int timeout_ms);
int frcnn_comm_destroy(frcnn_comm *);
int frcnn_comm_info(const frcnn_comm *, int *nranks_host, int *rank_host);
int frcnn_comm_query(const frcnn_comm *, int *count_host, int *user_rank_host, int *device_host);
int frcnn_allreduce_f32(frcnn_comm *, float *buf, long long n, void *stream);
int frcnn_allreduce_f64(frcnn_comm *, double *buf, long long n, void *stream);
int frcnn_broadcast_f32(frcnn_comm *, float *buf, long long n, int root, void *stream);

#ifdef __cplusplus
}
#endif
#endif
```

Before: 517.4.

## Fuse absmax records into ROI pool and BN backward, fold split-K slabs into ROI backward

The ROI-pool forward kernel now writes per-block absmax records, so the first classification layer's f16 split does not need a separate absmax pass over its input. The BN+activation backward kernel also emits absmax of its gradient output, which removes the separate absmax launches for dgrad and wgrad. The first layer's split-K dgrad slabs are no longer reduced into gx; a new ROI-pool backward kernel sums them directly in LDS while scattering. These steps remove several full-tensor passes and kernel launches. In exchange there is stamp/pointer bookkeeping that can go stale, plus a double-buffered record and a new native entry point.

```diff
diff --git a/faster-rcnn.torch_amd/_lib.py b/faster-rcnn.torch_amd/_lib.py
--- a/faster-rcnn.torch_amd/_lib.py
+++ b/faster-rcnn.torch_amd/_lib.py
@@ -135,6 +135,8 @@
     "frcnn_cnet_forward": ([vp, vp, vp, C.c_int, C.c_int, vp, C.c_ulonglong, vp, vp, vp, vp], C.c_int),
     "frcnn_cnet_backward": ([vp, vp, vp, vp, vp, vp, vp], C.c_int),
     "frcnn_cnet_backward_join": ([vp, vp], C.c_int),
+    "frcnn_cnet_roi_pool_forward": ([vp, vp, C.c_int, C.c_int, C.c_int, vp, C.c_int, C.c_int, C.c_int, vp, vp, vp], C.c_int),
+    "frcnn_cnet_backward_roi_pool": ([vp, vp, vp, vp, vp, vp, vp, C.c_int, C.c_int, C.c_int, vp, C.c_int, C.c_int, vp], C.c_int),
     "frcnn_cnet_losses": ([vp, vp, vp, vp, C.c_int, C.c_int, C.c_int, vp, vp, vp, vp], C.c_int),
     "frcnn_cnet_decode": ([vp, C.c_int, C.c_int, vp, vp, vp], C.c_int),
     "frcnn_anchors_create": ([vp, vp, vp, vp, C.c_int, C.c_int, C.POINTER(vp)], C.c_int),
diff --git a/faster-rcnn.torch_amd/csrc/amax.h b/faster-rcnn.torch_amd/csrc/amax.h
--- a/faster-rcnn.torch_amd/csrc/amax.h
+++ b/faster-rcnn.torch_amd/csrc/amax.h
@@ -19,6 +19,20 @@
   }
 }
 
+__device__ __forceinline__ void amax_store_block_at(float m, float* rec, int tid, int nthreads, int block, int nblocks) {
+  __shared__ float amax_part_at[16];
+#pragma unroll
+  for (int o = 32; o > 0; o >>= 1) m = fmaxf(m, __shfl_xor(m, o));
+  if ((tid & 63) == 0) amax_part_at[tid >> 6] = m;
+  __syncthreads();
+  if (tid == 0) {
+    const int nw = (nthreads + 63) >> 6;
+    for (int i = 1; i < nw; ++i) m = fmaxf(m, amax_part_at[i]);
+    rec[1 + block] = m;
+    if (block == 0) rec[0] = __builtin_bit_cast(float, nblocks);
+  }
+}
+
 __device__ __forceinline__ float amax_load_block(const float* __restrict__ rec) {
   __shared__ float amax_all[16];
   const int n = __builtin_bit_cast(int, rec[0]);
diff --git a/faster-rcnn.torch_amd/csrc/cnet.hip b/faster-rcnn.torch_amd/csrc/cnet.hip
--- a/faster-rcnn.torch_amd/csrc/cnet.hip
+++ b/faster-rcnn.torch_amd/csrc/cnet.hip
@@ -1,3 +1,4 @@
+#include "amax.h"
 #include "kernels.h"
 
 namespace frcnn {
@@ -276,7 +277,8 @@
                                                                     const float* __restrict__ invstd, const float* __restrict__ gamma,
                                                                     const float* slope, const float* __restrict__ mask, float inv_keep,
                                                                     int R, int n, int training, float* __restrict__ gx, float* ggamma,
-                                                                    float* gbeta, float* gslope, float* part) {
+                                                                    float* gbeta, float* gslope, float* part,
+                                                                    float* __restrict__ rec) {
   __shared__ double sh[FB_RG * FB_CB];
   __shared__ float shs[16];
   const int tx = threadIdx.x, ty = threadIdx.y;
@@ -325,38 +327,44 @@
       if (part) part[blockIdx.x] = t; else unsafeAtomicAdd(gslope, t);
     }
   }
-  if (!ok) return;
-  if (ty == 0) {
-    ggamma[j] = (float)((double)ggamma[j] + sgx);
-    gbeta[j] = (float)((double)gbeta[j] + sg);
-  }
-  const double is = invstd[j], gm = gamma[j];
-  auto second = [&](size_t idx, double g, double xhv) {
-    const double v = training ? (g - sg / R - xhv * sgx / R) * gm * is : g * gm * is;
-    gx[idx] = (float)v;
-  };
-  if (keep) {
-#pragma unroll
-    for (int i = 0; i < FB_KEEP; ++i)
-      if (ty + i * FB_RG < R) second((size_t)(ty + i * FB_RG) * n + j, tv[i], xh[i]);
-  } else {
-    for (int r = ty; r < R; r += FB_RG) {
-      const size_t idx = (size_t)r * n + j;
-      second(idx, gx[idx], xhat[idx]);
-    }
-  }
+  float am = 0.f;
+  if (ok) {
+    if (ty == 0) {
+      ggamma[j] = (float)((double)ggamma[j] + sgx);
+      gbeta[j] = (float)((double)gbeta[j] + sg);
+    }
+    const double is = invstd[j], gm = gamma[j];
+    auto second = [&](size_t idx, double g, double xhv) {
+      const double v = training ? (g - sg / R - xhv * sgx / R) * gm * is : g * gm * is;
+      gx[idx] = (float)v;
+      am = fmaxf(am, fabsf((float)v));
+    };
+    if (keep) {
+#pragma unroll
+      for (int i = 0; i < FB_KEEP; ++i)
+        if (ty + i * FB_RG < R) second((size_t)(ty + i * FB_RG) * n + j, tv[i], xh[i]);
+    } else {
+      for (int r = ty; r < R; r += FB_RG) {
+        const size_t idx = (size_t)r * n + j;
+        second(idx, gx[idx], xhat[idx]);
+      }
+    }
+  }
+  if (rec) amax_store_block_at(am, rec, ty * FB_CB + tx, FB_CB * FB_RG, blockIdx.x, gridDim.x);
 }
 __global__ void slope_fold_kernel(const float* __restrict__ part, int n, float* gslope);
 int cnet_act_bn_backward(const float* gy, GemmFold src, const float* pre, const float* xhat, const float* invstd,
                          const float* gamma, const float* slope, const float* mask, float inv_keep, int R, int n, int training,
-                         float* gx, float* ggamma, float* gbeta, float* gslope, hipStream_t s) {
+                         float* gx, float* ggamma, float* gbeta, float* gslope, hipStream_t s, float* amax_out) {
   const int grid = cdiv(n, FB_CB);
   float* part = nullptr;
   if (deterministic()) FR_TRY(det_workspace(s, (size_t)grid, &part));
+  float* rec = grid <= AMAX_MAX_BLOCKS ? amax_out : nullptr;
   FR_LAUNCH(KC_ELEMWISE, 0, (double)R * n * 28.0, s, cnet_act_bn_backward_kernel, dim3(grid), dim3(FB_CB, FB_RG), 0, gy, src, pre, xhat,
-            invstd, gamma, slope, mask, inv_keep, R, n, training, gx, ggamma, gbeta, gslope, part);
+            invstd, gamma, slope, mask, inv_keep, R, n, training, gx, ggamma, gbeta, gslope, part, rec);
   if (part) FR_LAUNCH(KC_ELEMWISE, 0, grid * 4.0, s, slope_fold_kernel, dim3(1), dim3(1), 0, (const float*)part, grid, gslope);
   FR_LAUNCH_CHECK();
+  if (amax_out && !rec) FR_TRY(tensor_absmax(gx, (long)R * n, amax_out, s));
   return FRCNN_OK;
 }
 
diff --git a/faster-rcnn.torch_amd/csrc/kernels.h b/faster-rcnn.torch_amd/csrc/kernels.h
--- a/faster-rcnn.torch_amd/csrc/kernels.h
+++ b/faster-rcnn.torch_amd/csrc/kernels.h
@@ -169,9 +169,12 @@
 
 
 int roi_pool_forward(const float* fmap, int C, int H, int W, const int* wins, int R, int kh, int kw,
-                     float* out, int* idx, hipStream_t s);
+                     float* out, int* idx, hipStream_t s, float* amax_rec = nullptr, bool* recorded = nullptr);
 int roi_pool_backward(float* gmap, int C, int H, int W, const float* gout, const int* idx, int R,
                       int kh, int kw, hipStream_t s);
+bool roi_pool_backward_fold_eligible(int H, int W);
+int roi_pool_backward_fold(float* gmap, int C, int H, int W, float* gout, const GemmFold& src, const int* idx, int R, int kh, int kw,
+                           hipStream_t s);
 
 int roi_align_forward(const float* fmap, int C, int H, int W, const double* rect, const long long* pick, int R, double inv_sx,
                       double inv_sy, int kh, int kw, int g, float* out, hipStream_t s);
@@ -236,7 +239,8 @@
                      float inv_keep, float p, unsigned long long seed, float* post, hipStream_t s);
 int cnet_act_bn_backward(const float* gy, GemmFold src, const float* pre, const float* xhat, const float* invstd,
                          const float* gamma, const float* slope, const float* mask, float inv_keep, int R, int n, int training,
-                         float* gx, float* ggamma, float* gbeta, float* gslope, hipStream_t s);
+                         float* gx, float* ggamma, float* gbeta, float* gslope, hipStream_t s,
+                         float* amax_out = nullptr);
 bool cnet_heads_fused_eligible(int nf, int nc);
 int cnet_heads_forward(const float* x, int R, int nf, const float* Wb, const float* bb, const float* Wc, const float* bc, int nc,
                        float* bbox_out, float* logits, float* lsm, float* cls_out, hipStream_t s);
diff --git a/faster-rcnn.torch_amd/csrc/net.cpp b/faster-rcnn.torch_amd/csrc/net.cpp
--- a/faster-rcnn.torch_amd/csrc/net.cpp
+++ b/faster-rcnn.torch_amd/csrc/net.cpp
@@ -80,6 +80,7 @@
   DevBuf xp, xpT, gp, gpT;
   int x_form = 0;
   DevBuf am;
+  const float* am_x = nullptr;
   const float* am_w_of = nullptr;
   long am_w_gen = -1;
 };
@@ -177,6 +178,10 @@
   int train_heads = 1, train_cnet = 1;
   int R = 0, D = 0;
   const float* cnet_x = nullptr;
+  DevBuf roi_am;
+  int roi_am_next = 0;
+  const float* roi_stamp_x = nullptr;
+  int roi_stamp_R = 0, roi_stamp_D = 0;
   DevBuf feat_g, logits, lsm, glog, gtmp;
   std::vector<std::array<long long, 4>> table;
 };
@@ -1089,6 +1094,13 @@
       FR_CHECK(index >= 0 && index < (int)m->cls.size() && m->R > 0, "debug_buffer: classification layer %d (after frcnn_cnet_forward)", index);
       const ClsLayer& L = m->cls[index]; b = L.bn ? &L.pre : &L.lin; n = (size_t)m->R * L.n * 4;
     } break;
+    case 5: {
+      FR_CHECK(m->roi_stamp_x != nullptr, "debug_buffer: no pending record of frcnn_cnet_roi_pool_forward");
+      b = &m->roi_am; n = (size_t)AMAX_REC * 4;
+      FR_CHECK(b->p && b->bytes >= (size_t)2 * AMAX_REC * 4, "debug_buffer: buffer not allocated yet");
+      *ptr = m->roi_am.f() + (size_t)m->roi_am_next * AMAX_REC; *bytes = (long long)n;
+      return FRCNN_OK;
+    }
     default: FR_CHECK(false, "debug_buffer: unknown kind %d", kind);
   }
   FR_CHECK(b->p && b->bytes >= n, "debug_buffer: buffer not allocated yet");
@@ -1664,6 +1676,10 @@
   const char* e = getenv("FRCNN_CNET_FUSE");
   return !(e && atoi(e) == 0);
 }
+static bool cnet_stage_fuse() {
+  const char* e = getenv("FRCNN_CNET_STAGE_FUSE");
+  return !(e && atoi(e) == 0);
+}
 static bool gemm_f16_on() {
   static const bool env_on = !(getenv("FRCNN_GEMM_F16") && atoi(getenv("FRCNN_GEMM_F16")) == 0);
   return env_on && get_x3_f16();
@@ -1702,6 +1718,8 @@
   FR_TRY(cw_join(m, s));
   FR_TRY(ensure_cnet(m, R));
   m->R = R; m->cnet_x = x; m->training = training;
+  const bool stamped = x && m->roi_stamp_x == x && m->roi_stamp_R == R && !m->cls.empty() && m->roi_stamp_D == m->cls[0].in;
+  m->roi_stamp_x = nullptr;
   const float* w = weights;
   const float* cur = x;
   float* bnr = bn_running;
@@ -1718,10 +1736,16 @@
       L.am_w_of = nullptr;
     }
     if ((L.x_form & 1) && gemm_f16_on()) {
-      float* rx = L.am.f();
-      FR_TRY(tensor_absmax(cur, (long)R * L.in, rx, s));
+      const float* rx = L.am.f();
+      if (l == 0 && stamped) {
+        rx = m->roi_am.f() + (size_t)m->roi_am_next * AMAX_REC;
+        m->roi_am_next ^= 1;
+      } else {
+        FR_TRY(tensor_absmax(cur, (long)R * L.in, L.am.f(), s));
+      }
+      L.am_x = rx;
       FR_TRY(split_planes(cur, R, L.in, L.xp.p, nullptr, s, rx));
-      FR_TRY(linear_x_forward(L.xp.p, R, L.in, w + L.w_off, w + L.b_off, L.n, L.lin.f(), s, 0, defer, rx, rx + 2 * AMAX_REC));
+      FR_TRY(linear_x_forward(L.xp.p, R, L.in, w + L.w_off, w + L.b_off, L.n, L.lin.f(), s, 0, defer, rx, L.am.f() + 2 * AMAX_REC));
     } else if (L.x_form & 1) {
       FR_TRY(split_planes(cur, R, L.in, L.xp.p, nullptr, s));
       FR_TRY(linear_x_forward(L.xp.p, R, L.in, w + L.w_off, w + L.b_off, L.n, L.lin.f(), s, 0, defer));
@@ -1781,9 +1805,12 @@
   return FRCNN_OK;
 }
 
-int frcnn_cnet_backward(frcnn_model* m, const float* weights, const float* g_bbox, const float* g_cls, float* gx,
-                        float* grad, void* stream) {
+}
+
+static int cnet_backward_impl(frcnn_model* m, const float* weights, const float* g_bbox, const float* g_cls, float* gx, float* grad,
+                              void* stream, GemmFold* fold0) {
   hipStream_t s = S(stream);
+  if (fold0) *fold0 = GemmFold{};
   FR_CHECK(m->R > 0, "cnet_backward: call frcnn_cnet_forward first");
   const int R = m->R;
   const float* w = weights;
@@ -1843,11 +1870,13 @@
     ClsLayer& L = m->cls[l];
     const float* pre = L.bn ? L.pre.f() : L.lin.f();
     const bool drop = m->training && L.p_drop > 0.f;
+    float* g_rec = nullptr;
     if (top_act_done && l == (int)m->cls.size() - 1) {
     } else if (L.bn && cnet_fuse()) {
+      if (cnet_stage_fuse() && (L.x_form & 6) && gemm_f16_on()) g_rec = L.am.f() + AMAX_REC;
       FR_TRY(cnet_act_bn_backward(g, gfold, pre, L.xhat.f(), L.invstd.f(), w + L.bnw_off, w + L.a_off, drop ? L.mask.f() : nullptr,
                                   drop ? 1.0f / (1.0f - L.p_drop) : 1.f, R, L.n, m->training, L.g.f(), grad + L.bnw_off,
-                                  grad + L.bnb_off, grad + L.a_off, s));
+                                  grad + L.bnb_off, grad + L.a_off, s, g_rec));
     } else {
       FR_TRY(prelu_dropout_backward(g, pre, (long)R * L.n, w + L.a_off, drop ? L.mask.f() : nullptr,
                                     drop ? 1.0f / (1.0f - L.p_drop) : 1.f, L.g.f(), grad + L.a_off, s));
@@ -1857,13 +1886,14 @@
     }
     gfold = GemmFold{};
     GemmFold* gdefer = (cnet_fuse() && async && l > 0 && m->cls[l - 1].bn) ? &gfold : nullptr;
+    if (l == 0 && async) gdefer = fold0;
     FR_TRY(fork());
     const float* in = l == 0 ? m->cnet_x : m->cls[l - 1].post.f();
     float* gin = l == 0 ? gx : L.gin.f();
     const bool xw = (L.x_form & 4) != 0, xd = (L.x_form & 2) != 0 && gin;
     if (xd && gemm_f16_on() && L.am_w_of == w) {
       float* rg = L.am.f() + AMAX_REC;
-      FR_TRY(tensor_absmax(L.g.f(), (long)R * L.n, rg, s));
+      if (!g_rec) FR_TRY(tensor_absmax(L.g.f(), (long)R * L.n, rg, s));
       FR_TRY(split_planes(L.g.f(), R, L.n, L.gp.p, nullptr, s, rg));
       FR_TRY(linear_x_dgrad(L.gp.p, R, L.n, w + L.w_off, L.in, gin, OUT_STORE, s, 0, gdefer, rg, L.am.f() + 2 * AMAX_REC));
     } else if (xd) {
@@ -1874,10 +1904,11 @@
     }
     static const bool wgrad_f16 = !(getenv("FRCNN_GEMM_WGRAD_F16") && atoi(getenv("FRCNN_GEMM_WGRAD_F16")) == 0);
     if (xw && wgrad_f16 && gemm_f16_on() && L.am.bytes >= (size_t)5 * AMAX_REC * 4) {
-      float *rgT = L.am.f() + 3 * AMAX_REC, *rxT = L.am.f() + 4 * AMAX_REC;
-      FR_TRY(tensor_absmax(L.g.f(), (long)R * L.n, rgT, ws));
-      if ((L.x_form & 1) && L.am_w_of == w) rxT = L.am.f();
-      else FR_TRY(tensor_absmax(in, (long)R * L.in, rxT, ws));
+      const float *rgT = L.am.f() + 3 * AMAX_REC, *rxT = L.am.f() + 4 * AMAX_REC;
+      if (g_rec) rgT = g_rec;
+      else FR_TRY(tensor_absmax(L.g.f(), (long)R * L.n, L.am.f() + 3 * AMAX_REC, ws));
+      if ((L.x_form & 1) && L.am_w_of == w) rxT = L.am_x;
+      else FR_TRY(tensor_absmax(in, (long)R * L.in, L.am.f() + 4 * AMAX_REC, ws));
       FR_TRY(split_planes(L.g.f(), R, L.n, nullptr, L.gpT.p, ws, rgT));
       FR_TRY(split_planes(in, R, L.in, nullptr, L.xpT.p, ws, rxT));
       FR_TRY(linear_x_wgrad(L.gpT.p, L.xpT.p, R, L.n, L.in, grad + L.w_off, ws, wslot, rgT, rxT));
@@ -1899,4 +1930,33 @@
   return FRCNN_OK;
 }
 
-}
+extern "C" {
+
+int frcnn_cnet_backward(frcnn_model* m, const float* weights, const float* g_bbox, const float* g_cls, float* gx,
+                        float* grad, void* stream) {
+  return cnet_backward_impl(m, weights, g_bbox, g_cls, gx, grad, stream, nullptr);
+}
+
+int frcnn_cnet_roi_pool_forward(frcnn_model* m, const float* fmap, int C, int H, int W, const int* wins, int R, int kh, int kw,
+                                float* out, int* idx, void* stream) {
+  m->roi_stamp_x = nullptr;
+  if (!cnet_stage_fuse() || R <= 0) return roi_pool_forward(fmap, C, H, W, wins, R, kh, kw, out, idx, S(stream));
+  FR_TRY(m->roi_am.ensure((size_t)2 * AMAX_REC * 4));
+  bool recorded = false;
+  FR_TRY(roi_pool_forward(fmap, C, H, W, wins, R, kh, kw, out, idx, S(stream), m->roi_am.f() + (size_t)m->roi_am_next * AMAX_REC, &recorded));
+  if (recorded) { m->roi_stamp_x = out; m->roi_stamp_R = R; m->roi_stamp_D = C * kh * kw; }
+  return FRCNN_OK;
+}
+
+int frcnn_cnet_backward_roi_pool(frcnn_model* m, const float* weights, const float* g_bbox, const float* g_cls, float* gx, float* grad,
+                                 float* gmap, int C, int H, int W, const int* idx, int kh, int kw, void* stream) {
+  FR_CHECK(m->R > 0, "cnet_backward_roi_pool: call frcnn_cnet_forward first");
+  FR_CHECK((long)C * kh * kw == m->D, "cnet_backward_roi_pool: %d x %d x %d cells per row, the net's input has %d", C, kh, kw, m->D);
+  GemmFold fold;
+  const bool fuse = cnet_stage_fuse() && roi_pool_backward_fold_eligible(H, W);
+  FR_TRY(cnet_backward_impl(m, weights, g_bbox, g_cls, gx, grad, stream, fuse ? &fold : nullptr));
+  if (m->frozen_blocks >= (int)m->blocks.size()) return FRCNN_OK;
+  return roi_pool_backward_fold(gmap, C, H, W, gx, fold, idx, m->R, kh, kw, S(stream));
+}
+
+}
diff --git a/faster-rcnn.torch_amd/csrc/roi.hip b/faster-rcnn.torch_amd/csrc/roi.hip
--- a/faster-rcnn.torch_amd/csrc/roi.hip
+++ b/faster-rcnn.torch_amd/csrc/roi.hip
@@ -1,3 +1,4 @@
+#include "amax.h"
 #include "kernels.h"
 #include "roi_fix.h"
 
@@ -32,67 +33,81 @@
   }
 }
 
+template <bool REC>
 __global__ __launch_bounds__(256) void roi_pool_forward_cells_kernel(const float* __restrict__ fmap, int C, int H, int W,
                                                                      const int* __restrict__ wins, int kh, int kw,
-                                                                     float* __restrict__ out, int* __restrict__ idx) {
+                                                                     float* __restrict__ out, int* __restrict__ idx,
+                                                                     float* __restrict__ rec) {
   const int r = blockIdx.x, cells = kh * kw, groups = blockDim.x / cells;
   const int tid = threadIdx.x;
-  if (tid >= groups * cells) return;
-  const int cg = tid / cells, cell = tid - cg * cells;
-  const int i = cell / kw, j = cell - i * kw;
-  const int* wn = wins + 4 * r;
-  const int r0 = wn[0] - 1, c0 = wn[2] - 1;
-  const int h = wn[1] - wn[0] + 1, w = wn[3] - wn[2] + 1;
-  const int ys = (i * h) / kh, ye = ((i + 1) * h + kh - 1) / kh;
-  const int xs = (j * w) / kw, xe = ((j + 1) * w + kw - 1) / kw;
-  const int HW = H * W;
-  const int base = (r0 + ys) * W + c0 + xs, nx = xe - xs, ny = ye - ys;
-  if (HW >= 4) {
-    for (int c = blockIdx.y * groups + cg; c < C; c += gridDim.y * groups) {
-      const float* ip = fmap + (size_t)c * HW;
-      float best = -3.402823466e+38f;
-      int bi = -1;
-      for (int y = 0, o = base; y < ny; ++y, o += W)
-        for (int x = 0; x < nx; x += 4) {
-          const int q = min(o + x, HW - 4);
-          float v[4];
-          __builtin_memcpy(v, ip + q, 16);
+  float am = 0.f;
+  if (tid < groups * cells) {
+    const int cg = tid / cells, cell = tid - cg * cells;
+    const int i = cell / kw, j = cell - i * kw;
+    const int* wn = wins + 4 * r;
+    const int r0 = wn[0] - 1, c0 = wn[2] - 1;
+    const int h = wn[1] - wn[0] + 1, w = wn[3] - wn[2] + 1;
+    const int ys = (i * h) / kh, ye = ((i + 1) * h + kh - 1) / kh;
+    const int xs = (j * w) / kw, xe = ((j + 1) * w + kw - 1) / kw;
+    const int HW = H * W;
+    const int base = (r0 + ys) * W + c0 + xs, nx = xe - xs, ny = ye - ys;
+    if (HW >= 4) {
+      for (int c = blockIdx.y * groups + cg; c < C; c += gridDim.y * groups) {
+        const float* ip = fmap + (size_t)c * HW;
+        float best = -3.402823466e+38f;
+        int bi = -1;
+        for (int y = 0, o = base; y < ny; ++y, o += W)
+          for (int x = 0; x < nx; x += 4) {
+            const int q = min(o + x, HW - 4);
+            float v[4];
+            __builtin_memcpy(v, ip + q, 16);
 #pragma unroll
-          for (int e = 0; e < 4; ++e) {
-            const int at = q + e;
-            if (at >= o && at < o + nx && v[e] > best) { best = v[e]; bi = at; }
+            for (int e = 0; e < 4; ++e) {
+              const int at = q + e;
+              if (at >= o && at < o + nx && v[e] > best) { best = v[e]; bi = at; }
+            }
           }
-        }
-      const size_t t = ((size_t)r * C + c) * cells + cell;
-      out[t] = best;
-      if (idx) idx[t] = bi;
+        const size_t t = ((size_t)r * C + c) * cells + cell;
+        out[t] = best;
+        if (idx) idx[t] = bi;
+        if (REC) am = fmaxf(am, fabsf(best));
+      }
+    } else {
+      for (int c = blockIdx.y * groups + cg; c < C; c += gridDim.y * groups) {
+        const float* ip = fmap + (size_t)c * HW;
+        float best = -3.402823466e+38f;
+        int bi = -1;
+        for (int y = 0, o = base; y < ny; ++y, o += W)
+          for (int x = 0; x < nx; ++x) {
+            const float v = ip[o + x];
+            if (v > best) { best = v; bi = o + x; }
+          }
+        const size_t t = ((size_t)r * C + c) * cells + cell;
+        out[t] = best;
+        if (idx) idx[t] = bi;
+        if (REC) am = fmaxf(am, fabsf(best));
+      }
     }
-    return;
-  }
-  for (int c = blockIdx.y * groups + cg; c < C; c += gridDim.y * groups) {
-    const float* ip = fmap + (size_t)c * HW;
-    float best = -3.402823466e+38f;
-    int bi = -1;
-    for (int y = 0, o = base; y < ny; ++y, o += W)
-      for (int x = 0; x < nx; ++x) {
-        const float v = ip[o + x];
-        if (v > best) { best = v; bi = o + x; }
-      }
-    const size_t t = ((size_t)r * C + c) * cells + cell;
-    out[t] = best;
-    if (idx) idx[t] = bi;
-  }
+  }
+  if (REC) amax_store_block_at(am, rec, tid, blockDim.x, blockIdx.y * gridDim.x + blockIdx.x, gridDim.x * gridDim.y);
 }
 
 int roi_pool_forward(const float* fmap, int C, int H, int W, const int* wins, int R, int kh, int kw,
-                     float* out, int* idx, hipStream_t s) {
+                     float* out, int* idx, hipStream_t s, float* amax_rec, bool* recorded) {
+  if (recorded) *recorded = false;
   if (R <= 0) return FRCNN_OK;
   long total = (long)R * C * kh * kw;
   if (kh * kw <= 256) {
     const int groups = 256 / (kh * kw);
     const int slices = std::max(1, std::min(cdiv(C, groups), (int)cdivl(4096, R)));
-    FR_LAUNCH(KC_ROI, 0, total * 8.0, s, roi_pool_forward_cells_kernel, dim3(R, slices), dim3(256), 0, fmap, C, H, W,
-              wins, kh, kw, out, idx);
+    if (amax_rec && (long)R * slices <= AMAX_MAX_BLOCKS) {
+      FR_LAUNCH(KC_ROI, 0, total * 8.0, s, roi_pool_forward_cells_kernel<true>, dim3(R, slices), dim3(256), 0, fmap, C, H, W,
+                wins, kh, kw, out, idx, amax_rec);
+      if (recorded) *recorded = true;
+    } else {
+      FR_LAUNCH(KC_ROI, 0, total * 8.0, s, roi_pool_forward_cells_kernel<false>, dim3(R, slices), dim3(256), 0, fmap, C, H, W,
+                wins, kh, kw, out, idx, (float*)nullptr);
+    }
     FR_LAUNCH_CHECK();
     return FRCNN_OK;
   }
@@ -116,6 +131,31 @@
     const long t = (long)r * D + (long)c * cell + j;
     const int bi = idx[t];
     const float g = gout[t];
+    if (bi >= 0 && g != 0.f) atomicAdd(&plane[bi], g);
+  }
+  __syncthreads();
+  float* gp = gmap + (size_t)c * HW;
+  for (int i = threadIdx.x; i < HW; i += blockDim.x) {
+    const float v = plane[i];
+    if (v != 0.f) gp[i] += v;
+  }
+}
+
+__global__ void roi_pool_backward_lds_fold_kernel(float* __restrict__ gmap, int C, int HW, const float* __restrict__ slab, int nSplit,
+                                                  const int* __restrict__ idx, int R, int cell) {
+  extern __shared__ float plane[];
+  const int c = blockIdx.x;
+  for (int i = threadIdx.x; i < HW; i += blockDim.x) plane[i] = 0.f;
+  __syncthreads();
+  const long D = (long)C * cell;
+  const size_t slab_floats = (size_t)R * D;
+  const int total = R * cell;
+  for (int e = threadIdx.x; e < total; e += blockDim.x) {
+    const int r = e / cell, j = e - r * cell;
+    const long t = (long)r * D + (long)c * cell + j;
+    const int bi = idx[t];
+    float g = 0.f;
+    for (int sI = 0; sI < nSplit; ++sI) g += slab[(size_t)sI * slab_floats + t];
     if (bi >= 0 && g != 0.f) atomicAdd(&plane[bi], g);
   }
   __syncthreads();
@@ -217,4 +257,21 @@
   return FRCNN_OK;
 }
 
-}
+bool roi_pool_backward_fold_eligible(int H, int W) { return !deterministic() && (size_t)H * W * 4 <= 64 * 1024; }
+
+int roi_pool_backward_fold(float* gmap, int C, int H, int W, float* gout, const GemmFold& src, const int* idx, int R, int kh, int kw,
+                           hipStream_t s) {
+  if (R <= 0) return FRCNN_OK;
+  if (src.nSplit == 0) return roi_pool_backward(gmap, C, H, W, gout, idx, R, kh, kw, s);
+  if (src.bias || !roi_pool_backward_fold_eligible(H, W)) {
+    FR_TRY(gemm_reduce_slabs(src.slab, src.nSplit, R, C * kh * kw, src.bias, gout, (long)C * kh * kw, false, s));
+    return roi_pool_backward(gmap, C, H, W, gout, idx, R, kh, kw, s);
+  }
+  const long total = (long)R * C * kh * kw;
+  FR_LAUNCH(KC_ROI, 0, total * 4.0 * (src.nSplit + 1), s, roi_pool_backward_lds_fold_kernel, dim3(C), dim3(1024), (size_t)H * W * 4, gmap,
+            C, H * W, src.slab, src.nSplit, idx, R, kh * kw);
+  FR_LAUNCH_CHECK();
+  return FRCNN_OK;
+}
+
+}
diff --git a/faster-rcnn.torch_amd/model_utilities.py b/faster-rcnn.torch_amd/model_utilities.py
--- a/faster-rcnn.torch_amd/model_utilities.py
+++ b/faster-rcnn.torch_amd/model_utilities.py
@@ -244,6 +244,20 @@
         self._pending = (self._input, grad_outputs[0], grad_outputs[1])
         return gx
 
+    def roi_pool_forward(self, fmap, C_, H, W, wins_ptr, R, kh, kw, out, idx):
+        _lib.call("frcnn_cnet_roi_pool_forward", self.native.h, ptr(fmap), C_, H, W, wins_ptr, R, kh, kw, ptr(out), ptr(idx),
+                  stream_ptr())
+        return out
+
+    def backward_roi_pool(self, cinput, grad_outputs, gmap, C_, H, W, idx, kh, kw):
+        nat = self.native
+        R, D = self._input.shape
+        gx = self._buf("gx", (R, D))
+        _lib.call("frcnn_cnet_backward_roi_pool", nat.h, ptr(nat.weights), ptr(grad_outputs[0]), ptr(grad_outputs[1]), ptr(gx),
+                  ptr(nat.gradient), ptr(gmap), C_, H, W, ptr(idx), kh, kw, stream_ptr())
+        self._pending = (self._input, grad_outputs[0], grad_outputs[1])
+        return gx
+
     def join_backward(self):
         _lib.call("frcnn_cnet_backward_join", self.native.h, stream_ptr())
         self._pending = None
diff --git a/faster-rcnn.torch_amd/objective.py b/faster-rcnn.torch_amd/objective.py
--- a/faster-rcnn.torch_amd/objective.py
+++ b/faster-rcnn.torch_amd/objective.py
@@ -448,8 +448,7 @@
                               kh, kw, sampling, ptr(cinput), s)
                 else:
                     pidx = scratch.get("pidx", (E, D), np.int32)
-                    _lib.call("frcnn_roi_pool_forward", ptr(fm), fmC, fmH, fmW, C.c_void_p(d_wins), E, kh, kw,
-                              ptr(cinput), ptr(pidx), s)
+                    cnet.roi_pool_forward(fm, fmC, fmH, fmW, C.c_void_p(d_wins), E, kh, kw, cinput, pidx)
                 coutputs = cnet.forward(cinput)
                 crout, ccout = coutputs
                 crdelta = scratch.get("crdelta", (E, 4))
@@ -457,13 +456,13 @@
                 pnet.anchor_loss_wait()
                 _lib.call("frcnn_cnet_losses", ptr(crout), ptr(crtarget), ptr(ccout), ptr(cctarget), E, npos, ncls,
                           ptr(crdelta), ptr(ccdelta), C.c_void_p(acc_dev.ptr + 4 * 8), s)
-                post_roi_delta = cnet.backward(cinput, [crdelta, ccdelta])
-                if not trunk_frozen and align:
-                    _lib.call("frcnn_roi_align_backward", ptr(delta_outputs[4]), fmC, fmH, fmW, ptr(post_roi_delta),
-                              C.c_void_p(d_wins), None, E, inv_sx, inv_sy, kh, kw, sampling, s)
-                elif not trunk_frozen:
-                    _lib.call("frcnn_roi_pool_backward", ptr(delta_outputs[4]), fmC, fmH, fmW, ptr(post_roi_delta),
-                              ptr(pidx), E, kh, kw, s)
+                if align:
+                    post_roi_delta = cnet.backward(cinput, [crdelta, ccdelta])
+                    if not trunk_frozen:
+                        _lib.call("frcnn_roi_align_backward", ptr(delta_outputs[4]), fmC, fmH, fmW, ptr(post_roi_delta),
+                                  C.c_void_p(d_wins), None, E, inv_sx, inv_sy, kh, kw, sampling, s)
+                else:
+                    cnet.backward_roi_pool(cinput, [crdelta, ccdelta], delta_outputs[4], fmC, fmH, fmW, pidx, kh, kw)
             if E == 0:
                 for l in range(4):
                     _lib.call("frcnn_pnet_set_sparse_deltas", native.h, l + 1, None, 0)
diff --git a/include/frcnn_hip.h b/include/frcnn_hip.h
--- a/include/frcnn_hip.h
+++ b/include/frcnn_hip.h
@@ -232,6 +232,11 @@
 int frcnn_cnet_backward_join(frcnn_model *, void *stream);
 int frcnn_cnet_backward(frcnn_model *, const float *weights, const float *g_bbox,
                         const float *g_cls, float *gx, float *grad, void *stream);
+int frcnn_cnet_roi_pool_forward(frcnn_model *, const float *fmap, int C, int H, int W, const int *wins, int R,
+                                int kh, int kw, float *out, int *idx, void *stream);
+int frcnn_cnet_backward_roi_pool(frcnn_model *, const float *weights, const float *g_bbox, const float *g_cls,
+                                 float *gx, float *grad, float *gmap, int C, int H, int W, const int *idx,
+                                 int kh, int kw, void *stream);
 int frcnn_cnet_losses(float *crout, const float *crtarget, const float *ccout,
                       const float *cctarget, int R, int npos, int ncls, float *crdelta,
                       float *ccdelta, double *loss2, void *stream);
```

Result: no change. 518.2 (median of 6 runs) (+0.2%).
